# WD-Leong/CV-Lite-Object-Detection

Measured on AMD Instinct MI355X. Metric: training images/sec (whole node), FCOS-VOC 512x512 bs=16/GPU, higher is better.
Workload: dtype bf16; 1 GPU; FCOS ResNet-50-FPN train step (targets + fwd + loss + bwd + clip/SGD), 512x512, bs=16 per GPU; model=FCOS-ResNet50-FPN, global_batch=16, image_size=512, parallelism=dp1

## Files before the change

cv-lite-object-detection_amd/csrc/conv_common.h:

```cpp
#pragma once
#include "cvl_common.h"
#include "bn_acc.h"
#include <type_traits>
#include <vector>

typedef short s16x8 __attribute__((ext_vector_type(8)));
typedef short s16x4 __attribute__((ext_vector_type(4)));
typedef __bf16 bf16x8 __attribute__((ext_vector_type(8)));
typedef float f32x4 __attribute__((ext_vector_type(4)));

constexpr int kMaxSeg = CVL_CONV_MAX_SEG;

__device__ __forceinline__ short relu_bf16_bits(short v) { return v < 0 ? (short)0 : v; }

extern thread_local int g_cvl_conv_last_kernel;
extern thread_local int g_cvl_conv_last_ktile;

__device__ __forceinline__ int xcd_remap(int b, int nwg) {
  const int q = nwg / 8, r = nwg % 8, x = b % 8;
  return (x < r ? x * (q + 1) : r * (q + 1) + (x - r) * q) + b / 8;
}

template <int N>
__device__ __forceinline__ void wait_vm() {
  __builtin_amdgcn_s_waitcnt((N & 15) | ((N >> 4) << 14) | (7 << 4) | (15 << 8));
}

__device__ __forceinline__ s16x4 ds_tr16(unsigned addr) {
  s16x4 v;
  asm volatile("ds_read_b64_tr_b16 %0, %1" : "=v"(v) : "v"(addr));
  return v;
}
__device__ __forceinline__ void lgkm_wait() { asm volatile("s_waitcnt lgkmcnt(0)" ::: "memory"); }
__device__ __forceinline__ void tr_pin(s16x4& v) { asm volatile("" : "+v"(v)); }
__device__ __forceinline__ s16x8 tr_join(s16x4 l, s16x4 h) {
  return s16x8{l[0], l[1], l[2], l[3], h[0], h[1], h[2], h[3]};
}

__device__ __forceinline__ unsigned lds_addr(const void* p) {
  return (unsigned)(size_t)(const __attribute__((address_space(3))) void*)p;
}

struct ConvSeg {
  int Hr, Wr, Hs, Ws;
  long src_base, src_img, dst_base, dst_img;
  int m_start;
  int rows;
  const cvl_bf16* w;
  const float* bias;
};

struct ConvArgs {
  const cvl_bf16* src;
  void* dst;
  acc_u64* stats;
  int acc_slots;
  int nseg, B;
  ConvSeg seg[kMaxSeg];
  int Cin, KH, KW, stride, pad_t, pad_l;
  int K, Npad, n_store, ld_dst, dst_coff, dst_f32, relu_out, relu_in;
  float beta;
  int m_tiles, m_total;
  float* slab;
  int splits, ksteps_per_split;
  int dbg;
  int dst_up, dst_w;
  const cvl_bf16* bz;
  const float* bmr;
  const float* bga;
  const float* bbe;
  acc_u64* bsum;
  float bhi;
  const cvl_bf16* by;
  const uint8_t* bbits;
  unsigned long long* probe;
  const cvl_bf16* ymask;
};

uint64_t* cvl_probe_current(bool take);
void cvl_probe_enter_call();
void cvl_probe_leave_call();

__device__ __forceinline__ void probe_enter(unsigned long long* p) {
  if (blockIdx.x == 0 && threadIdx.x == 0) __hip_atomic_store(p, wall_clock64(), __ATOMIC_RELAXED, __HIP_MEMORY_SCOPE_AGENT);
}
__device__ __forceinline__ void probe_leave(unsigned long long* p) {
  __syncthreads();
  if (threadIdx.x == 0) {
    if (atomicAdd(p + 3, 1ull) == (unsigned long long)gridDim.x - 1) {
      const unsigned long long t = wall_clock64();
      const unsigned long long t0 = __hip_atomic_load(p, __ATOMIC_RELAXED, __HIP_MEMORY_SCOPE_AGENT);
      atomicAdd(p + 1, t - t0);
      atomicAdd(p + 2, 1ull);
      __hip_atomic_store(p + 3, 0ull, __ATOMIC_RELAXED, __HIP_MEMORY_SCOPE_AGENT);
    }
  }
}

int cvl_bn_acc_prepare(uint64_t* acc, long nstat, hipStream_t s);

int cvl_wgrad_reduce(const float* slab, float* dst0, float* dst1, long n4, int splits, int groups, float beta,
                     hipStream_t s);
int cvl_wgrad_defer_guard(const float* dst, hipStream_t s);
int cvl_wgrad_reduce_lanes(long elems4, int splits);

struct BnSumArgs {
  const cvl_bf16* z;
  const float* mr;
  const float* gamma;
  const float* beta;
  acc_u64* sums;
  float hi;
  const cvl_bf16* y;
  const uint8_t* bits;
};

enum { CVL_BSUM_NONE = 0, CVL_BSUM_Z = 1, CVL_BSUM_Y = 2, CVL_BSUM_BITS = 3 };
struct ConvCallOpts {
  bool bn_stats;
  int bsum;
  bool ymask;
  size_t workspace_bytes;
  bool res_relu;
};

enum { CVL_PRE_NONE = 0, CVL_PRE_ZERO_GAPS = 1, CVL_PRE_S2DG3_PACK = 2 };

struct ConvPlan {
  int kernel;
  int bn, bk;
  bool dgrad;
  bool sw;
  bool wres;
  bool prio, acc, stamps;
  int stages;
  int bsum;
  bool ymask;
  bool res_relu;
  int splits, ksteps_per_split;
  int grid;
  size_t workspace_bytes;
  int pre;
  size_t pack_bytes;
  int dbg;
  cvl_conv_desc desc;
  ConvArgs geo;
};

int conv_plan(const cvl_conv_desc* d, const ConvCallOpts& o, ConvPlan* p);
size_t conv_plan_workspace_bound(const cvl_conv_desc* d);
static inline void conv_plan_set_splits(ConvPlan* p, int nk, int want) {
  p->ksteps_per_split = (nk + want - 1) / want;
  p->splits = (nk + p->ksteps_per_split - 1) / p->ksteps_per_split;
}
static inline int conv_plan_ktile(const ConvPlan& p) { return p.kernel == CVL_CK_X32 || p.kernel == CVL_CK_P ? p.bk : 0; }

int launch_base(const ConvPlan& p, const ConvArgs& a, hipStream_t s);
int launch_l(const ConvPlan& p, const ConvArgs& a, hipStream_t s);
int launch_x(const ConvPlan& p, const ConvArgs& a, hipStream_t s);
int launch_h(const ConvPlan& p, const ConvArgs& a, hipStream_t s);
int launch_p(const ConvPlan& p, const ConvArgs& a, hipStream_t s);

bool cvl_conv_h_fits(const cvl_conv_desc* d, const ConvArgs& a, int* halo_px);
constexpr int kConvHWresCb = 2;
constexpr int kConvHStampWgs = 4096;
constexpr unsigned kConvBufRecords = 0x7fffffffu;

template <class F>
static inline void with_bool(bool b, F&& f) {
  if (b) f(std::true_type{});
  else f(std::false_type{});
}

constexpr int kWgSegM = 128;
constexpr int kWgXMaxGroups = 2;
constexpr int kWgXMaxProb = 16, kWgHMaxProb = 12;

struct WgLaunch {
  int kernel;
  int seg0, nseg, ngroups;
  int tile;
  int rows;
  bool pf;
  int tiles, co_tiles;
  int chunk, nsplit;
  int steps;
  int g_m0[kWgXMaxGroups], g_m1[kWgXMaxGroups];
  int cbase[kMaxSeg + 1];
  size_t slab_bytes;
};

struct WgradPlan {
  int nlaunch;
  WgLaunch l[kMaxSeg];
  size_t workspace_bytes;
};
int wgrad_plan(const cvl_conv_desc* d, int ngroups, WgradPlan* p);

static inline cvl_conv_desc wgrad_launch_desc(const cvl_conv_desc* d, const WgLaunch& l) {
  cvl_conv_desc s = *d;
  s.nseg = l.nseg;
  for (int i = 0; i < l.nseg; ++i) s.seg[i] = d->seg[l.seg0 + i];
  return s;
}

struct WgBatchLaunch {
  int kernel, tile;
  int n, idx[kWgXMaxProb];
  int chunk;
  int nsplit[kWgXMaxProb];
  size_t slab_off[kWgXMaxProb];
  size_t ws_off, ws_bytes;
  WgradPlan single;
};
struct WgradBatchPlan {
  std::vector<WgBatchLaunch> l;
  size_t workspace_bytes;
};
int wgrad_batch_plan(const cvl_conv_desc* const* d, int n, WgradBatchPlan* p);

bool wg_sn_fits(const cvl_conv_desc* d, int ngroups);
bool wg_h_fits(const cvl_conv_desc* d);
bool wg_x_fits(const cvl_conv_desc* d, int ngroups, const ConvArgs& a);
bool wg_x_batch_fits(const cvl_conv_desc* d, ConvArgs* a);
bool wg_l_fits(const cvl_conv_desc* d, const ConvArgs& a);

int launch_wg_sn(const WgLaunch& l, const cvl_conv_desc& d, const void* x, const void* dy, float* const* dw, float beta,
                 void* ws, hipStream_t s);
int launch_wg_h(const WgLaunch& l, const cvl_conv_desc& d, const void* x, const void* dy, float* const* dw, float beta,
                void* ws, hipStream_t s);
int launch_wg_x(const WgLaunch& l, const cvl_conv_desc& d, const void* x, const void* dy, float* const* dw, float beta,
                void* ws, hipStream_t s);
int launch_wg_l(const WgLaunch& l, const cvl_conv_desc& d, const void* x, const void* dy, float* const* dw, float beta,
                void* ws, hipStream_t s);
int launch_wg_s(const WgLaunch& l, const cvl_conv_desc& d, const void* x, const void* dy, float* const* dw, float beta,
                void* ws, hipStream_t s);
int launch_wg_x_batch(const WgBatchLaunch& b, const cvl_conv_desc* const* d, const void* const* x, const void* const* dy,
                      float* const* dw, float beta, char* ws, hipStream_t s);
int launch_wg_h_batch(const WgBatchLaunch& b, const cvl_conv_desc* const* d, const void* const* x, const void* const* dy,
                      float* const* dw, float beta, char* ws, hipStream_t s);
int wgrad_run(const WgradPlan& p, const cvl_conv_desc* d, const void* x, const void* dy, float* const* dw, float beta,
              void* ws, hipStream_t s);

size_t cvl_conv_wgrad_f32_workspace(const cvl_conv_desc* d, int ngroups);
int cvl_conv_wgrad_f32(const cvl_conv_desc* d, int ngroups, const void* x, const void* dy, float* const* dw,
                       float beta, void* workspace, size_t workspace_bytes, hipStream_t s);

__device__ __forceinline__ long conv_dst_row(const ConvArgs& a, const ConvSeg& S, int img, int q) {
  long r = q;
  if (a.dst_up != 1) {
    const int y = q / S.Wr, x = q - (q / S.Wr) * S.Wr;
    r = (long)y * a.dst_up * a.dst_w + (long)x * a.dst_up;
  }
  return S.dst_base + (long)img * S.dst_img + r;
}

static inline int cvl_conv_prepare(const cvl_conv_desc* d, int bm, ConvArgs* a) {
  CVL_CHECK_ARG(d);
  CVL_CHECK_ARG(d->nseg >= 1 && d->nseg <= kMaxSeg && d->B >= 1);
  CVL_CHECK_ARG(d->Cin > 0 && d->KH > 0 && d->KW > 0 && d->stride > 0);
  CVL_CHECK_ARG(d->mode == CVL_CONV_FWD || d->mode == CVL_CONV_DGRAD);
  CVL_CHECK_ARG(d->Npad > 0 && d->n_store > 0 && d->n_store <= d->Npad);
  CVL_CHECK_ARG(d->ld_dst >= d->dst_coff + d->n_store);
  a->slab = nullptr;
  a->splits = 1;
  a->ksteps_per_split = 0;
  a->dst_up = 1;
  a->dst_w = 0;
  a->dbg = 0;
  a->bz = nullptr; a->bmr = nullptr; a->bga = nullptr; a->bbe = nullptr; a->bsum = nullptr; a->bhi = 0.f;
  a->by = nullptr;
  a->bbits = nullptr;
  a->probe = nullptr;
  a->ymask = nullptr;
  a->acc_slots = cvl_bn_acc_slots();
  a->nseg = d->nseg;
  a->B = d->B;
  a->Cin = d->Cin; a->KH = d->KH; a->KW = d->KW; a->stride = d->stride;
  a->pad_t = d->pad_t; a->pad_l = d->pad_l;
  a->K = d->KH * d->KW * d->Cin;
  a->Npad = d->Npad; a->n_store = d->n_store; a->ld_dst = d->ld_dst; a->dst_coff = d->dst_coff;
  a->dst_f32 = d->dst_f32; a->relu_out = d->relu_out; a->relu_in = d->relu_in; a->beta = d->beta;
  int m = 0;
  for (int i = 0; i < kMaxSeg; ++i) {
    ConvSeg& s = a->seg[i];
    if (i >= d->nseg) {
      s = a->seg[0];
      s.m_start = 0x7fffffff;
      continue;
    }
    const cvl_conv_seg& q = d->seg[i];
    CVL_CHECK_ARG(q.Hr > 0 && q.Wr > 0 && q.Hs > 0 && q.Ws > 0 && q.w);
    s.Hr = q.Hr; s.Wr = q.Wr; s.Hs = q.Hs; s.Ws = q.Ws;
    s.src_base = q.src_base; s.src_img = q.src_img; s.dst_base = q.dst_base; s.dst_img = q.dst_img;
    s.w = reinterpret_cast<const cvl_bf16*>(q.w);
    s.bias = q.bias;
    s.m_start = m;
    s.rows = d->B * q.Hr * q.Wr;
    m += ((s.rows + bm - 1) / bm) * bm;
  }
  a->m_total = m;
  a->m_tiles = m / bm;
  return CVL_OK;
}
```

cv-lite-object-detection_amd/csrc/conv_dispatch.hip:

```cpp
#include "conv_common.h"

namespace {

constexpr int BM_BASE = 128, NT_BASE = 256;
constexpr int BM = 256;
constexpr int H_BN = 64, H_BK = 32;

int device_cus() {
  static const int n = cvl_device_cus();
  return n;
}

int pick_bn(int npad) { return npad % 128 == 0 ? 128 : (npad % 64 == 0 ? 64 : 32); }

int base_split_want(const ConvArgs& a) {
  if (a.nseg != 1) return 1;
  const int BN_ = pick_bn(a.Npad), BK_ = a.Cin % 64 == 0 ? 64 : 32;
  const int tiles = a.m_tiles * (a.Npad / BN_);
  const int nk = a.K / BK_;
  const int max_tiles = cvl_tune_int("CVL_KSPLIT_MAX_TILES", 192);
  const int target = cvl_tune_int("CVL_KSPLIT_TARGET", 384);
  const int min_nk = cvl_dispatch_int("ksplit_min_nk", 4);
  if (tiles >= max_tiles || nk < min_nk) return 1;
  int s = (target + tiles - 1) / tiles;
  const int per = cvl_tune_int("CVL_KSPLIT_MIN_PER", 2);
  if (s > nk / per) s = nk / per;
  return s < 1 ? 1 : s;
}

int h_split_want(const ConvArgs& a) {
  const int tiles = a.m_tiles * (a.Npad / H_BN);
  const int target = cvl_tune_int("CVL_CONV_H_SPLIT_TARGET", 256);
  if (tiles >= target) return 1;
  int splits = (target + tiles - 1) / tiles;
  if (splits > (a.Cin / H_BK) / 2) splits = (a.Cin / H_BK) / 2;
  return splits < 1 ? 1 : splits;
}

size_t slab_bytes(const ConvArgs& a, int splits) { return (size_t)splits * a.m_total * a.Npad * sizeof(float); }

bool s2dgrad_transform(const cvl_conv_desc* d, cvl_conv_desc* out, int* up, int* upw) {
  if (d->mode != CVL_CONV_DGRAD || d->KH != 1 || d->KW != 1 || d->stride < 2 || d->nseg != 1 ||
      d->pad_t != 0 || d->pad_l != 0 || d->relu_in || cvl_tune_flag("CVL_CONV_NO_S2DG"))
    return false;
  const cvl_conv_seg& q = d->seg[0];
  if ((q.Hs - 1) * d->stride >= q.Hr || (q.Ws - 1) * d->stride >= q.Wr) return false;
  *out = *d;
  out->mode = CVL_CONV_FWD;
  out->stride = 1;
  out->seg[0].Hr = q.Hs;
  out->seg[0].Wr = q.Ws;
  *up = d->stride;
  *upw = q.Wr;
  return true;
}

bool s2dgrad3_ok(const cvl_conv_desc* d) {
  if (!d || d->mode != CVL_CONV_DGRAD || d->KH != 3 || d->KW != 3 || d->stride != 2 || d->pad_t || d->pad_l ||
      d->nseg != 1 || d->relu_in || d->prec != CVL_PREC_BF16 || d->Cin % 32 || d->Npad % 32 ||
      cvl_dispatch_flag("no_s2dg3"))
    return false;
  const cvl_conv_seg& q = d->seg[0];
  return q.Hr == 2 * q.Hs && q.Wr == 2 * q.Ws && q.w &&
         (long)d->B * q.Hr * q.Wr >= cvl_dispatch_int("s2dg3_min_rows", 4096);
}

size_t s2dgrad3_pack_bytes(const cvl_conv_desc* d) {
  return ((size_t)4 * d->Npad * 4 * d->Cin * sizeof(cvl_bf16) + 255) / 256 * 256;
}

cvl_conv_desc s2dgrad3_desc(const cvl_conv_desc* d, const cvl_bf16* sub) {
  cvl_conv_desc dd = *d;
  const cvl_conv_seg q = d->seg[0];
  dd.mode = CVL_CONV_FWD;
  dd.KH = dd.KW = 2;
  dd.stride = 1;
  dd.pad_t = dd.pad_l = 1;
  dd.nseg = 4;
  for (int cls = 0; cls < 4; ++cls) {
    cvl_conv_seg& g = dd.seg[cls];
    g = q;
    g.Hr = q.Hs;
    g.Wr = q.Ws;
    g.w = sub + (size_t)cls * d->Npad * 4 * d->Cin;
    g.bias = nullptr;
    g.dst_base = q.dst_base + (long)(cls >> 1) * q.Wr + (cls & 1);
  }
  return dd;
}
const cvl_bf16* const kPackPlaceholder = reinterpret_cast<const cvl_bf16*>(16);

bool dst_chunks8(const cvl_conv_desc* d) { return d->n_store % 8 == 0 && d->ld_dst % 8 == 0 && d->dst_coff % 8 == 0; }

bool tiles_in_images(const ConvArgs& a, bool dense) {
  for (int i = 0; i < a.nseg; ++i) {
    const long hw = (long)a.seg[i].Hr * a.seg[i].Wr;
    if (hw % BM || (dense && a.seg[i].dst_img != hw)) return false;
  }
  return true;
}

bool buffer_bounds_ok(const ConvArgs& a) {
  for (int i = 0; i < a.nseg; ++i) {
    const ConvSeg& q = a.seg[i];
    const long src_bytes = (q.src_base + (long)a.B * q.src_img) * a.Cin * 2;
    if (src_bytes >= (long)kConvBufRecords - 65536) return false;
  }
  return (long)a.Npad * a.K * 2 < (long)kConvBufRecords;
}

bool x32_fits(const cvl_conv_desc* d, const ConvArgs& a) {
  const bool dg = d->mode == CVL_CONV_DGRAD;
  if (a.Npad % 256 || a.Cin % 32 || a.K / 32 < 1 || d->KH * d->KW > 32 || a.relu_in || (dg && d->stride != 1) ||
      a.dst_up != 1)
    return false;
  return buffer_bounds_ok(a);
}

bool plan_x(const cvl_conv_desc* d, const ConvArgs& a, const ConvCallOpts& o, ConvPlan* p) {
  if (cvl_dispatch_flag("no_x") || !x32_fits(d, a)) return false;
  p->kernel = CVL_CK_X32;
  p->bn = 256;
  p->bk = 32;
  p->grid = a.m_tiles * (a.Npad / 256);
  p->dbg = cvl_tune_int("CVL_X_ABLATE", 0);
  p->sw = !a.dst_f32 && !o.bn_stats && a.beta == 0.f && dst_chunks8(d) && !cvl_dispatch_flag("x_no_sw");
  p->ymask = p->sw && o.ymask && !a.relu_out && !cvl_dispatch_flag("no_relu_mask_fuse");
  return true;
}

bool p_fits(const cvl_conv_desc* d, const ConvArgs& a, const ConvCallOpts& o) {
  if (d->KH != 1 || d->KW != 1 || d->pad_t || d->pad_l || a.relu_in || a.nseg != 1 || a.K % 32) return false;
  const bool by = o.bsum == CVL_BSUM_Y || o.bsum == CVL_BSUM_BITS;
  if (o.bsum == CVL_BSUM_BITS && (a.ld_dst % 8 || a.dst_coff % 8)) return false;
  if (o.bsum && ((d->mode != CVL_CONV_DGRAD && a.dst_up == 1) || a.dst_f32 || (a.beta != 0.f) != by ||
                 (a.dst_up != 1 && !by) || o.bn_stats || (a.seg[0].Hr * a.seg[0].Wr) % BM ||
                 (a.dst_up == 1 && a.seg[0].dst_img != (long)a.seg[0].Hr * a.seg[0].Wr) || a.Npad % 64))
    return false;
  if (d->mode == CVL_CONV_DGRAD && d->stride != 1) return false;
  const ConvSeg& q = a.seg[0];
  if (d->stride == 1 && (q.Hs != q.Hr || q.Ws != q.Wr)) return false;
  if (a.dst_f32 ? (a.n_store % 4 || a.ld_dst % 4 || a.dst_coff % 4) : !dst_chunks8(d)) return false;
  if (o.bn_stats && (a.dst_f32 || (q.Hr * q.Wr) % BM)) return false;
  return buffer_bounds_ok(a);
}

bool plan_p(const cvl_conv_desc* d, const ConvArgs& a, const ConvCallOpts& o, ConvPlan* p) {
  if (cvl_dispatch_flag("no_p") || !p_fits(d, a, o)) return false;
  if (o.bsum && cvl_tune_flag("CVL_CONV_P_NO_BSUM")) return false;
  const bool wide = a.K <= 256 || (a.Npad >= 2 * a.K && cvl_dispatch_int("p_wide128", 1));
  const int bn = wide && a.Npad % 128 == 0 ? 128 : (a.Npad % 64 == 0 ? 64 : 0);
  const int fbn = cvl_dispatch_int("p_bn", 0);
  const int use = o.bsum ? 64 : (fbn && a.Npad % fbn == 0 ? fbn : bn);
  if (!use) return false;
  const int ntiles = a.m_tiles * (a.Npad / use);
  const int ntn = a.Npad / use;
  const int wgs = cvl_dispatch_int("p_wgs", 256);
  int grid = cvl_tune_int("CVL_CONV_P_WGS", wgs > 256 ? 256 : (wgs < 1 ? 1 : wgs));
  if (grid >= ntiles) grid = ntiles;
  else grid -= grid % ntn;
  if (grid < 1) return false;
  p->kernel = CVL_CK_P;
  p->bn = use;
  p->bk = a.K % 64 == 0 && use != 256 && cvl_dispatch_int("p_k64", 1) ? 64 : 32;
  p->grid = grid;
  p->dbg = cvl_tune_int("CVL_P_ABLATE", 0);
  p->bsum = o.bsum;
  p->acc = a.beta != 0.f && !cvl_tune_flag("CVL_P_NO_ACC");
  p->res_relu = o.res_relu && p->acc && use != 256 && !cvl_dispatch_flag("no_res_relu_fuse");
  return true;
}

bool plan_h(const cvl_conv_desc* d, const ConvArgs& a, const ConvCallOpts& o, size_t ws_bytes, ConvPlan* p) {
  int halo_px = 0;
  if (cvl_dispatch_flag("no_h") || !cvl_conv_h_fits(d, a, &halo_px)) return false;
  const bool stg3 = !cvl_dispatch_flag("h_no_3stage") && halo_px <= 512;
  const bool bs = o.bsum != CVL_BSUM_NONE;
  p->kernel = CVL_CK_H64;
  p->bk = H_BK;
  p->bsum = o.bsum;
  if (a.Npad == 32) {
    if (o.bn_stats || bs) return false;
    p->bn = 32;
    p->stages = stg3 ? 3 : 2;
    p->grid = a.m_tiles < device_cus() ? a.m_tiles : device_cus();
    return true;
  }
  const int tiles = a.m_tiles * (a.Npad / H_BN);
  const bool sw_ok = !d->dst_f32 && d->beta == 0.f && dst_chunks8(d) && !(o.bn_stats && bs) && tiles_in_images(a, bs);
  if (!cvl_dispatch_flag("h_no_n32") && a.Npad % H_BN == 0 && 2 * tiles <= device_cus() && sw_ok) {
    p->bn = 32;
    p->sw = true;
    p->stages = stg3 ? 3 : 2;
    p->grid = 2 * tiles;
    return true;
  }
  const int ncb = a.Cin / H_BK;
  int splits = 1;
  if (a.nseg == 1 && !bs && ws_bytes && d->n_store % 8 == 0 && d->dst_coff % 8 == 0 &&
      (d->dst_f32 || d->ld_dst % 8 == 0) && d->n_store / 8 <= 256) {
    splits = h_split_want(a);
    if (slab_bytes(a, splits) > ws_bytes) splits = 1;
  }
  if (splits > 1) conv_plan_set_splits(p, ncb, splits);
  const int per_cu = cvl_tune_int("CVL_CONV_H_WG_PER_CU", 1);
  p->grid = p->splits > 1 ? tiles : (tiles < device_cus() * per_cu ? tiles : device_cus() * per_cu);
  p->bn = H_BN;
  p->stages = 2;
  p->wres = p->splits <= 1 && a.Npad == H_BN && ncb <= kConvHWresCb && a.nseg == 1 && !cvl_dispatch_flag("h_no_wres");
  p->sw = p->splits <= 1 && sw_ok && !cvl_dispatch_flag("h_no_sw");
  p->stamps = cvl_tune_flag("CVL_H_STAMPS") && p->splits <= 1 && p->grid <= kConvHStampWgs;
  return true;
}

bool large_fits(const cvl_conv_desc* d, const ConvCallOpts& o) {
  if (d->Cin % 32 != 0 || d->relu_in) return false;
  return d->dst_f32 ? (d->n_store % 4 == 0 && !o.bn_stats) : dst_chunks8(d);
}

bool plan_large(const cvl_conv_desc* d, const ConvArgs& a, const ConvCallOpts& o, ConvPlan* p) {
  if (cvl_dispatch_flag("no_l")) return false;
  const bool bs = o.bsum != CVL_BSUM_NONE, by = o.bsum == CVL_BSUM_Y || o.bsum == CVL_BSUM_BITS;
  const bool scat = by && a.dst_up != 1 && d->KH == 1 && d->KW == 1 && d->mode == CVL_CONV_FWD;
  if (bs && !scat &&
      (d->mode != CVL_CONV_DGRAD || d->dst_f32 || (d->beta != 0.f && !by) || a.dst_up != 1 || o.bn_stats))
    return false;
  if (scat && (d->dst_f32 || o.bn_stats)) return false;
  if (by && (d->KH != 1 || d->KW != 1)) return false;
  if (d->Npad == 32 && d->KH == 3 && d->KW == 3 && d->mode == CVL_CONV_FWD && d->dst_f32 && !o.bn_stats &&
      !bs && a.dst_up == 1 && d->Cin % 32 == 0 && !d->relu_in && !cvl_dispatch_flag("no_h32"))
    return plan_h(d, a, o, 0, p);
  if (!large_fits(d, o)) return false;
  if (d->dst_f32 && (cvl_tune_flag("CVL_CONV_L_F32_N8") || cvl_tune_flag("CVL_CONV_L_NO_F32"))) return false;
  const bool l_cin = d->Cin % 64 == 0;
  const bool w256 = d->Npad % 256 == 0 && !cvl_dispatch_flag("no_256") &&
                    (d->mode == CVL_CONV_FWD || !cvl_tune_flag("CVL_CONV_NO_DGRAD_256"));
  const int bn = w256 ? 256 : (d->Npad % 128 == 0 ? 128 : (d->Npad % 64 == 0 ? 64 : 0));
  if (!bn) return false;
  if (l_cin && d->KH * d->KW * d->Cin < cvl_tune_int("CVL_CONV_L_MIN_K", 0) && !bs) return false;
  if (d->KH == 1 && d->KW == 1) {
    if (plan_p(d, a, o, p)) return true;
    if (by) return false;
  }
  const long min_tiles = cvl_dispatch_int("l_min_tiles", 128);
  int use_bn = bn;
  if (use_bn == 256 && (long)a.m_tiles * (a.Npad / 256) < cvl_dispatch_int("l256_min_tiles", 256)) use_bn = 128;
  const int w256_min_k = cvl_dispatch_int("w256_min_k", 512);
  if (use_bn == 256 && a.K < w256_min_k) use_bn = 128;
  const int fill = cvl_tune_int("CVL_CONV_L64_FILL", 256);
  const bool fill_pre = !cvl_tune_flag("CVL_CONV_L64_NO_FILL_PRE");
  const bool to64 = fill && use_bn == 128 && (long)a.m_tiles * (a.Npad / 128) < fill && a.Npad % 64 == 0 &&
                    !(bs && cvl_tune_flag("CVL_BSUM_NO_FILL"));
  if (!l_cin && d->Cin == 32 && bn == 256 && !bs && !o.bn_stats && cvl_dispatch_int("x_cin32", 1) &&
      plan_x(d, a, o, p))
    return true;
  const bool h_width = use_bn == 64 || to64 || !l_cin || cvl_tune_flag("CVL_CONV_H_ANY_N");
  if (h_width && use_bn != 256 && (!bs || ((a.seg[0].Hr * a.seg[0].Wr) % BM == 0 && !o.bn_stats)) &&
      (!bs || tiles_in_images(a, true)) && plan_h(d, a, o, o.workspace_bytes, p))
    return true;
  if (!l_cin) return false;
  if (fill_pre && to64) use_bn = 64;
  if ((long)a.m_tiles * (a.Npad / use_bn) < min_tiles) return false;
  if (to64) use_bn = 64;
  if (o.bn_stats)
    for (int i = 0; i < a.nseg; ++i)
      if ((a.seg[i].Hr * a.seg[i].Wr) % 4) return false;
  if (bs && (use_bn == 256 || !tiles_in_images(a, true))) return false;
  if (use_bn == 256 && plan_x(d, a, o, p)) return true;
  p->kernel = use_bn == 256 ? CVL_CK_L256 : (use_bn == 128 ? CVL_CK_L128 : CVL_CK_L64);
  p->bn = use_bn;
  p->bk = 64;
  p->grid = a.m_tiles * (a.Npad / use_bn);
  p->bsum = o.bsum;
  p->prio = !cvl_tune_flag("CVL_CONV_NO_PRIO");
  p->sw = !a.dst_f32 && a.beta == 0.f && !bs && a.dst_up == 1 && dst_chunks8(d) && !cvl_dispatch_flag("l_no_sw") &&
          (!o.bn_stats || tiles_in_images(a, false));
  return true;
}

void plan_base(const cvl_conv_desc* d, const ConvArgs& a, const ConvCallOpts& o, ConvPlan* p) {
  p->bn = pick_bn(a.Npad);
  p->bk = p->bn <= 64 && a.Cin % 128 == 0 && cvl_dispatch_int("base_bk128", 1) ? 128 : (a.Cin % 64 == 0 ? 64 : 32);
  const int sp = base_split_want(a);
  const bool split = sp > 1 && (d->n_store / 8 <= NT_BASE) && o.workspace_bytes >= slab_bytes(a, sp) &&
                     d->n_store % 8 == 0 && d->dst_coff % 8 == 0 && (d->dst_f32 || d->ld_dst % 8 == 0);
  if (split) conv_plan_set_splits(p, a.K / p->bk, sp);
  p->kernel = split ? CVL_CK_BASE_SPLITK : CVL_CK_BASE;
  p->grid = a.m_tiles * (a.Npad / p->bn);
}

bool bsum_offer_ok(const cvl_conv_desc* d, int form) {
  if (cvl_tune_flag("CVL_NO_BNSUM_FUSE") || d->prec != CVL_PREC_BF16 || d->mode != CVL_CONV_DGRAD || d->dst_f32 ||
      d->Cin % 32 || d->Npad % 32 || !dst_chunks8(d))
    return false;
  const long hw = (long)d->seg[0].Hr * d->seg[0].Wr;
  if (form == CVL_BSUM_Z)
    return d->beta == 0.f && hw >= cvl_tune_int("CVL_BNSUM_MIN_HW", 0);
  return !cvl_tune_flag("CVL_NO_BNSUM_RES") && d->beta != 0.f && d->KH == 1 && d->KW == 1 &&
         (d->stride == 1 || !cvl_dispatch_flag("no_bnsum_res_s2")) &&
         hw >= cvl_dispatch_int("bnsum_res_min_hw", 256);
}

}

int conv_plan(const cvl_conv_desc* d, const ConvCallOpts& o, ConvPlan* p) {
  CVL_CHECK_ARG(d && p && d->prec == CVL_PREC_BF16);
  *p = ConvPlan{};
  p->kernel = CVL_CK_NONE;
  p->splits = 1;
  size_t ws_bytes = o.workspace_bytes;
  int up = 1, upw = 0;
  if (o.bsum) {
    if (!d->nseg || !bsum_offer_ok(d, o.bsum)) return CVL_OK;
    const bool tr = s2dgrad_transform(d, &p->desc, &up, &upw);
    if (o.bsum == CVL_BSUM_Z ? tr : (d->stride != 1 && !tr)) return CVL_OK;
    if (!tr) p->desc = *d;
  } else if (s2dgrad3_ok(d) && ws_bytes >= s2dgrad3_pack_bytes(d)) {
    CVL_CHECK_ARG(!o.bn_stats);
    CVL_CHECK_ARG(d->dst_f32 || dst_chunks8(d));
    p->pre = CVL_PRE_S2DG3_PACK;
    p->pack_bytes = s2dgrad3_pack_bytes(d);
    p->desc = s2dgrad3_desc(d, kPackPlaceholder);
    up = 2;
    upw = d->seg[0].Wr;
    ws_bytes -= p->pack_bytes;
  } else if (s2dgrad_transform(d, &p->desc, &up, &upw)) {
    CVL_CHECK_ARG(!o.bn_stats);
    CVL_CHECK_ARG(d->dst_f32 || dst_chunks8(d));
    if (d->beta == 0.f) {
      const cvl_conv_seg& q = d->seg[0];
      const long line = (long)q.Wr * (d->dst_f32 ? d->n_store : d->n_store / 8);
      CVL_CHECK_ARG(line < (1l << 31) && (long)d->B * q.Hr < (1l << 31));
      p->pre = CVL_PRE_ZERO_GAPS;
    }
  } else {
    p->desc = *d;
  }
  d = &p->desc;
  p->dgrad = d->mode == CVL_CONV_DGRAD;
  ConvCallOpts oo = o;
  oo.workspace_bytes = ws_bytes;
  ConvArgs base;
  const int st = cvl_conv_prepare(d, BM_BASE, &base);
  if (st) return o.bsum ? CVL_OK : st;
  if (!o.bsum) {
    CVL_CHECK_ARG(d->Cin % 32 == 0 && d->Npad % 32 == 0);
    if (!d->dst_f32) CVL_CHECK_ARG(dst_chunks8(d));
    if (o.bn_stats) {
      for (int i = 0; i < base.nseg; ++i) {
        const int hw = base.seg[i].Hr * base.seg[i].Wr;
        CVL_CHECK_ARG(hw % BM_BASE == 0 || hw % 4 == 0);
      }
    }
  }
  if (cvl_conv_prepare(d, BM, &p->geo) == CVL_OK) {
    p->geo.dst_up = up;
    p->geo.dst_w = upw;
    ConvPlan q = *p;
    if (plan_large(d, p->geo, oo, &q)) *p = q;
  }
  if (p->kernel == CVL_CK_NONE) {
    if (o.bsum) return CVL_OK;
    p->geo = base;
    p->geo.dst_up = up;
    p->geo.dst_w = upw;
    plan_base(d, p->geo, oo, p);
  }
  p->workspace_bytes = p->pack_bytes + (p->splits > 1 ? slab_bytes(p->geo, p->splits) : 0);
  return CVL_OK;
}

size_t conv_plan_workspace_bound(const cvl_conv_desc* d) {
  if (s2dgrad3_ok(d)) {
    const cvl_conv_desc dd = s2dgrad3_desc(d, kPackPlaceholder);
    return s2dgrad3_pack_bytes(d) + conv_plan_workspace_bound(&dd);
  }
  cvl_conv_desc dd;
  int up = 1, upw = 0;
  if (s2dgrad_transform(d, &dd, &up, &upw)) d = &dd;
  ConvArgs a;
  if (cvl_conv_prepare(d, BM_BASE, &a)) return 0;
  const int sp = base_split_want(a);
  size_t n = sp > 1 ? slab_bytes(a, sp) : 16;
  ConvArgs a256;
  int halo_px = 0;
  if (cvl_conv_prepare(d, BM, &a256) == CVL_OK && a256.nseg == 1 && a256.Npad % H_BN == 0 &&
      cvl_conv_h_fits(d, a256, &halo_px)) {
    const int hs = h_split_want(a256);
    if (hs > 1 && slab_bytes(a256, hs) > n) n = slab_bytes(a256, hs);
  }
  return n;
}

extern "C" int cvl_conv_igemm_plan(const cvl_conv_desc* d, int with_bn_stats, size_t workspace_bytes, int32_t* kernel,
                                   int32_t* ktile) {
  CVL_CHECK_ARG(d && kernel && ktile);
  *kernel = CVL_CK_NONE;
  *ktile = 0;
  if (d->prec == CVL_PREC_F32) return CVL_OK;
  ConvPlan p;
  const int st = conv_plan(d, ConvCallOpts{with_bn_stats != 0, CVL_BSUM_NONE, false, workspace_bytes}, &p);
  if (st) return st;
  *kernel = p.kernel;
  *ktile = conv_plan_ktile(p);
  return CVL_OK;
}
```

cv-lite-object-detection_amd/csrc/conv_igemm.hip:

```cpp
#include "conv_common.h"

namespace {

constexpr int BM = 128;
constexpr int NT = 256;

template <int BK>
__device__ __forceinline__ int swz(int r) {
  return BK == 128 ? (r & 15) : (BK == 64 ? ((r >> 1) & 7) : ((r >> 2) & 3));
}

__device__ __forceinline__ s16x8 relu_bf16x8(s16x8 v) {
#pragma unroll
  for (int i = 0; i < 8; ++i) v[i] = v[i] < 0 ? (short)0 : v[i];
  return v;
}



template <int BN, int BK, bool DGRAD>
__global__ void __launch_bounds__(NT) conv_igemm_kernel(ConvArgs a) {
  constexpr int WM = BM / 2, WN = BN / 2;
  constexpr int TM = WM / 16, TN = WN / 16;
  constexpr int CPR = BK / 8;
  constexpr int RPP = NT / CPR;
  constexpr int AP = BM / RPP;
  constexpr int BROWS = BN < RPP ? BN : RPP;
  constexpr int BP = BN / BROWS;
  constexpr int LDS_AB = (BM + BN) * BK;
  constexpr int LDS_C = BM * (BN + 8);
  constexpr int LDS_EL = LDS_AB > LDS_C ? LDS_AB : LDS_C;
  __shared__ __attribute__((aligned(16))) cvl_bf16 lds[LDS_EL];
  cvl_bf16* As = lds;
  cvl_bf16* Bs = lds + BM * BK;

  const int tid = threadIdx.x;
  const int m_tile = blockIdx.x, n_tile = blockIdx.y;
  const int m0 = m_tile * BM, n0 = n_tile * BN;
  int sg = 0;
#pragma unroll
  for (int i = 1; i < kMaxSeg; ++i)
    if (i < a.nseg && m0 >= a.seg[i].m_start) sg = i;
  const ConvSeg& S = a.seg[sg];
  const int HWr = S.Hr * S.Wr;
  const int mloc0 = m0 - S.m_start;
  if (mloc0 >= S.rows) return;

  const int ch = tid % CPR, rr = tid / CPR;
  int a_img[AP], a_y[AP], a_x[AP];
  bool a_ok[AP];
#pragma unroll
  for (int p = 0; p < AP; ++p) {
    const int ml = mloc0 + p * RPP + rr;
    a_ok[p] = ml < S.rows;
    const int img = ml / HWr, q = ml - img * HWr;
    const int oy = q / S.Wr, ox = q - (q / S.Wr) * S.Wr;
    a_img[p] = img;
    if (DGRAD) { a_y[p] = oy + a.pad_t; a_x[p] = ox + a.pad_l; }
    else { a_y[p] = oy * a.stride - a.pad_t; a_x[p] = ox * a.stride - a.pad_l; }
  }
  const cvl_bf16* __restrict__ wsrc = S.w;
  const cvl_bf16* __restrict__ src = a.src;
  const int Cin = a.Cin;

  s16x8 ra[AP], rb[BP];
  auto load_tile = [&](int kt) {
    const int k0 = kt * BK;
    const int tap = k0 / Cin;
    const int c0 = k0 - tap * Cin + ch * 8;
    const int r = tap / a.KW, s = tap - (tap / a.KW) * a.KW;
#pragma unroll
    for (int p = 0; p < AP; ++p) {
      int iy, ix;
      bool ok = a_ok[p];
      if (DGRAD) {
        const int ty = a_y[p] - r, tx = a_x[p] - s;
        ok = ok && ty >= 0 && tx >= 0 && (ty % a.stride) == 0 && (tx % a.stride) == 0;
        iy = ty / a.stride; ix = tx / a.stride;
      } else {
        iy = a_y[p] + r; ix = a_x[p] + s;
      }
      ok = ok && iy >= 0 && ix >= 0 && iy < S.Hs && ix < S.Ws;
      if (ok) {
        const long row = S.src_base + (long)a_img[p] * S.src_img + (long)iy * S.Ws + ix;
        ra[p] = *reinterpret_cast<const s16x8*>(src + row * Cin + c0);
        if (a.relu_in) ra[p] = relu_bf16x8(ra[p]);
      } else {
        ra[p] = s16x8{0, 0, 0, 0, 0, 0, 0, 0};
      }
    }
#pragma unroll
    for (int p = 0; p < BP; ++p) {
      const int n = n0 + p * BROWS + tid / CPR;
      if (tid / CPR < BROWS)
        rb[p] = *reinterpret_cast<const s16x8*>(wsrc + (long)n * a.K + k0 + ch * 8);
    }
  };
  auto store_tile = [&]() {
#pragma unroll
    for (int p = 0; p < AP; ++p) {
      const int r = p * RPP + rr;
      *reinterpret_cast<s16x8*>(As + r * BK + ((ch ^ swz<BK>(r)) * 8)) = ra[p];
    }
#pragma unroll
    for (int p = 0; p < BP; ++p) {
      const int r = p * BROWS + tid / CPR;
      if (tid / CPR < BROWS) *reinterpret_cast<s16x8*>(Bs + r * BK + ((ch ^ swz<BK>(r)) * 8)) = rb[p];
    }
  };

  const int wave = tid >> 6, lane = tid & 63;
  const int wm = wave >> 1, wn = wave & 1;
  const int lr = lane & 15, lg = lane >> 4;
  f32x4 acc[TM][TN];
#pragma unroll
  for (int i = 0; i < TM; ++i)
#pragma unroll
    for (int j = 0; j < TN; ++j) acc[i][j] = f32x4{0.f, 0.f, 0.f, 0.f};

  int kt0 = 0, kt1 = a.K / BK;
  if (a.splits > 1) {
    kt0 = blockIdx.z * a.ksteps_per_split;
    kt1 = min(kt1, kt0 + a.ksteps_per_split);
  }
  const int nk = kt1;
  load_tile(kt0);
  for (int kt = kt0; kt < nk; ++kt) {
    const cvl_bf16* Ac = As;
    const cvl_bf16* Bc = Bs;
    __syncthreads();
    store_tile();
    __syncthreads();
    if (kt + 1 < nk) load_tile(kt + 1);
#pragma unroll
    for (int ks = 0; ks < BK / 32; ++ks) {
      const int chunk = ks * 4 + lg;
      s16x8 fa[TM], fb[TN];
#pragma unroll
      for (int i = 0; i < TM; ++i) {
        const int r = wm * WM + i * 16 + lr;
        fa[i] = *reinterpret_cast<const s16x8*>(Ac + r * BK + ((chunk ^ swz<BK>(r)) * 8));
      }
#pragma unroll
      for (int j = 0; j < TN; ++j) {
        const int r = wn * WN + j * 16 + lr;
        fb[j] = *reinterpret_cast<const s16x8*>(Bc + r * BK + ((chunk ^ swz<BK>(r)) * 8));
      }
#pragma unroll
      for (int i = 0; i < TM; ++i)
#pragma unroll
        for (int j = 0; j < TN; ++j)
          acc[i][j] = __builtin_amdgcn_mfma_f32_16x16x32_bf16(
              __builtin_bit_cast(bf16x8, fa[i]), __builtin_bit_cast(bf16x8, fb[j]), acc[i][j], 0, 0, 0);
    }
  }

  if (a.splits > 1) {
    float* slab = a.slab + (size_t)blockIdx.z * a.m_total * a.Npad;
#pragma unroll
    for (int i = 0; i < TM; ++i)
#pragma unroll
      for (int j = 0; j < TN; ++j)
#pragma unroll
        for (int e = 0; e < 4; ++e) {
          const int r = m0 + wm * WM + i * 16 + lg * 4 + e;
          const int c = n0 + wn * WN + j * 16 + lr;
          slab[(size_t)r * a.Npad + c] = acc[i][j][e];
        }
    return;
  }
  const float* bias = S.bias;
  float bcol[TN];
#pragma unroll
  for (int j = 0; j < TN; ++j) {
    const int n = n0 + wn * WN + j * 16 + lr;
    bcol[j] = (bias && n < a.n_store) ? bias[n] : 0.f;
  }
  const bool round_bf16 = !a.dst_f32;
#pragma unroll
  for (int i = 0; i < TM; ++i)
#pragma unroll
    for (int j = 0; j < TN; ++j)
#pragma unroll
      for (int e = 0; e < 4; ++e) {
        float v = acc[i][j][e] + bcol[j];
        if (a.relu_out) v = v > 0.f ? v : 0.f;
        if (round_bf16) v = bf16_to_f32(f32_to_bf16(v));
        acc[i][j][e] = v;
      }

  if (a.stats && (HWr % BM) != 0) {
#pragma unroll
    for (int i = 0; i < TM; ++i) {
      const int ml0 = mloc0 + wm * WM + i * 16 + lg * 4;
      if (ml0 >= S.rows) continue;
      const int img = ml0 / HWr;
#pragma unroll
      for (int j = 0; j < TN; ++j) {
        const int n = n0 + wn * WN + j * 16 + lr;
        if (n >= a.n_store) continue;
        float s1 = 0.f, s2 = 0.f;
#pragma unroll
        for (int e = 0; e < 4; ++e) { const float v = acc[i][j][e]; s1 += v; s2 += v * v; }
        acc_u64* st = a.stats + acc_idx((long)img * a.n_store + n, 0, a.acc_slots);
        acc_add(st, s1, a.acc_slots);
        acc_add(st + a.acc_slots, s2, a.acc_slots);
      }
    }
  } else if (a.stats) {
    const int img = mloc0 / HWr;
#pragma unroll
    for (int j = 0; j < TN; ++j) {
      float s1 = 0.f, s2 = 0.f;
#pragma unroll
      for (int i = 0; i < TM; ++i)
#pragma unroll
        for (int e = 0; e < 4; ++e) {
          const int ml = mloc0 + wm * WM + i * 16 + lg * 4 + e;
          const float v = ml < S.rows ? acc[i][j][e] : 0.f;
          s1 += v; s2 += v * v;
        }
      s1 += __shfl_xor(s1, 16, 64); s1 += __shfl_xor(s1, 32, 64);
      s2 += __shfl_xor(s2, 16, 64); s2 += __shfl_xor(s2, 32, 64);
      const int n = n0 + wn * WN + j * 16 + lr;
      if (lg == 0 && n < a.n_store) {
        acc_u64* st = a.stats + acc_idx((long)img * a.n_store + n, 0, a.acc_slots);
        acc_add(st, s1, a.acc_slots);
        acc_add(st + a.acc_slots, s2, a.acc_slots);
      }
    }
  }

  if (a.dst_f32) {
    float* dst = reinterpret_cast<float*>(a.dst);
#pragma unroll
    for (int i = 0; i < TM; ++i)
#pragma unroll
      for (int e = 0; e < 4; ++e) {
        const int ml = mloc0 + wm * WM + i * 16 + lg * 4 + e;
        if (ml >= S.rows) continue;
        const int img = ml / HWr, q = ml - img * HWr;
        const long drow = conv_dst_row(a, S, img, q);
#pragma unroll
        for (int j = 0; j < TN; ++j) {
          const int n = n0 + wn * WN + j * 16 + lr;
          if (n >= a.n_store) continue;
          float* pd = dst + drow * a.ld_dst + a.dst_coff + n;
          *pd = a.beta != 0.f ? acc[i][j][e] + a.beta * *pd : acc[i][j][e];
        }
      }
    return;
  }

  __syncthreads();
  constexpr int CP = BN + 8;
  cvl_bf16* Cs = lds;
#pragma unroll
  for (int i = 0; i < TM; ++i)
#pragma unroll
    for (int j = 0; j < TN; ++j)
#pragma unroll
      for (int e = 0; e < 4; ++e) {
        const int r = wm * WM + i * 16 + lg * 4 + e;
        const int c = wn * WN + j * 16 + lr;
        Cs[r * CP + c] = f32_to_bf16(acc[i][j][e]);
      }
  __syncthreads();
  constexpr int CCH = BN / 8;
  cvl_bf16* dst = reinterpret_cast<cvl_bf16*>(a.dst);
  for (int idx = tid; idx < BM * CCH; idx += NT) {
    const int r = idx / CCH, c8 = (idx - (idx / CCH) * CCH) * 8;
    const int ml = mloc0 + r;
    if (ml >= S.rows || n0 + c8 >= a.n_store) continue;
    const int img = ml / HWr, q = ml - img * HWr;
    const long drow = conv_dst_row(a, S, img, q);
    s16x8 v = *reinterpret_cast<const s16x8*>(Cs + r * CP + c8);
    s16x8* pd = reinterpret_cast<s16x8*>(dst + drow * a.ld_dst + a.dst_coff + n0 + c8);
    if (a.beta != 0.f) {
      const s16x8 o = *pd;
#pragma unroll
      for (int u = 0; u < 8; ++u)
        v[u] = (short)f32_to_bf16(bf16_to_f32((cvl_bf16)v[u]) + a.beta * bf16_to_f32((cvl_bf16)o[u]));
    }
    *pd = v;
  }
}

constexpr int FIN_RL = NT / 8;
__global__ void __launch_bounds__(NT) conv_splitk_finish(ConvArgs a, int rows_per_blk) {
  const ConvSeg& S = a.seg[0];
  const int HW = S.Hr * S.Wr;
  const int img = blockIdx.y;
  const int cgi = threadIdx.x & 7, rl = threadIdx.x >> 3;
  const int c0 = blockIdx.z * 64 + cgi * 8;
  const bool cok = c0 < a.n_store;
  const int q0 = blockIdx.x * rows_per_blk;
  const int q1 = min(q0 + rows_per_blk, HW);
  __shared__ float red[FIN_RL][8][17];
  float s1[8], s2[8], bb[8];
#pragma unroll
  for (int u = 0; u < 8; ++u) { s1[u] = 0.f; s2[u] = 0.f; bb[u] = (S.bias && cok) ? S.bias[c0 + u] : 0.f; }
  if (cok) {
    for (int q = q0 + rl; q < q1; q += FIN_RL) {
      const long ml = (long)img * HW + q;
      float v[8];
#pragma unroll
      for (int u = 0; u < 8; ++u) v[u] = bb[u];
      const f32x4* p = reinterpret_cast<const f32x4*>(a.slab + (size_t)ml * a.Npad + c0);
      const size_t zs = (size_t)a.m_total * a.Npad / 4;
      int z = 0;
      for (; z + 4 <= a.splits; z += 4) {
        f32x4 x[4][2];
#pragma unroll
        for (int t = 0; t < 4; ++t) { x[t][0] = p[(z + t) * zs]; x[t][1] = p[(z + t) * zs + 1]; }
#pragma unroll
        for (int t = 0; t < 4; ++t) {
          v[0] += x[t][0][0]; v[1] += x[t][0][1]; v[2] += x[t][0][2]; v[3] += x[t][0][3];
          v[4] += x[t][1][0]; v[5] += x[t][1][1]; v[6] += x[t][1][2]; v[7] += x[t][1][3];
        }
      }
      for (; z < a.splits; ++z) {
        const f32x4 x0 = p[z * zs], x1 = p[z * zs + 1];
        v[0] += x0[0]; v[1] += x0[1]; v[2] += x0[2]; v[3] += x0[3];
        v[4] += x1[0]; v[5] += x1[1]; v[6] += x1[2]; v[7] += x1[3];
      }
      const long drow = conv_dst_row(a, S, img, q);
      if (a.dst_f32) {
        float* pd = reinterpret_cast<float*>(a.dst) + drow * a.ld_dst + a.dst_coff + c0;
#pragma unroll
        for (int u = 0; u < 8; ++u) {
          float o = v[u];
          if (a.relu_out) o = o > 0.f ? o : 0.f;
          s1[u] += o; s2[u] += o * o;
          if (a.beta != 0.f) o += a.beta * pd[u];
          pd[u] = o;
        }
      } else {
        s16x8* pd = reinterpret_cast<s16x8*>(reinterpret_cast<cvl_bf16*>(a.dst) + drow * a.ld_dst + a.dst_coff + c0);
        s16x8 old;
        if (a.beta != 0.f) old = *pd;
        s16x8 o;
#pragma unroll
        for (int u = 0; u < 8; ++u) {
          float x = v[u];
          if (a.relu_out) x = x > 0.f ? x : 0.f;
          x = bf16_to_f32(f32_to_bf16(x));
          s1[u] += x; s2[u] += x * x;
          if (a.beta != 0.f) x += a.beta * bf16_to_f32((cvl_bf16)old[u]);
          o[u] = (short)f32_to_bf16(x);
        }
        *pd = o;
      }
    }
  }
  if (a.stats) {
#pragma unroll
    for (int u = 0; u < 8; ++u) { red[rl][cgi][u] = s1[u]; red[rl][cgi][8 + u] = s2[u]; }
    __syncthreads();
    if (threadIdx.x < 64) {
      const int cg2 = threadIdx.x >> 3, u = threadIdx.x & 7;
      const int c = blockIdx.z * 64 + cg2 * 8 + u;
      if (c < a.n_store) {
        double t1 = 0.0, t2 = 0.0;
        for (int k = 0; k < FIN_RL; ++k) { t1 += red[k][cg2][u]; t2 += red[k][cg2][8 + u]; }
        acc_u64* st = a.stats + acc_idx((long)img * a.n_store + c, 0, a.acc_slots);
        acc_add_f64(st, t1, a.acc_slots);
        acc_add_f64(st + a.acc_slots, t2, a.acc_slots);
      }
    }
  }
}

static int splitk_finish_launch(const ConvArgs& a, hipStream_t s) {
  const ConvSeg& S = a.seg[0];
  const int HW = S.Hr * S.Wr;
  const int nch = (a.n_store + 63) / 64;
  int parts = 512 / (a.B * nch);
  if (parts > HW / 16) parts = HW / 16;
  if (parts < 1) parts = 1;
  const int rpb = (HW + parts - 1) / parts;
  hipLaunchKernelGGL(conv_splitk_finish, dim3((HW + rpb - 1) / rpb, a.B, nch), dim3(NT), 0, s, a, rpb);
  return cvl_launch_status();
}

template <int BN, int BK>
void launch_bn_bk(const ConvPlan& p, const ConvArgs& a, hipStream_t s) {
  dim3 grid(a.m_tiles, a.Npad / BN, a.splits);
  with_bool(p.dgrad, [&](auto DG) {
    hipLaunchKernelGGL((conv_igemm_kernel<BN, BK, decltype(DG)::value>), grid, dim3(NT), 0, s, a);
  });
}

template <int BN>
void launch_bn(const ConvPlan& p, const ConvArgs& a, hipStream_t s) {
  if (BN <= 64 && p.bk == 128) launch_bn_bk<BN, 128>(p, a, s);
  else if (p.bk == 64) launch_bn_bk<BN, 64>(p, a, s);
  else launch_bn_bk<BN, 32>(p, a, s);
}

}

__global__ void s2dgrad3_pack_kernel(const cvl_bf16* __restrict__ wd, cvl_bf16* __restrict__ sub, int Npad, int Cin) {
  const int c8n = Cin / 8;
  const long total = 16L * Npad * c8n;
  for (long i = blockIdx.x * (long)NT + threadIdx.x; i < total; i += (long)gridDim.x * NT) {
    const int c8 = (int)(i % c8n);
    const long r1 = i / c8n;
    const int t = (int)(r1 & 3);
    const long r2 = r1 >> 2;
    const int n = (int)(r2 % Npad), cls = (int)(r2 / Npad);
    const int py = cls >> 1, px = cls & 1, rp = t >> 1, sp = t & 1;
    const int r = py ? (rp ? 1 : -1) : (rp ? 0 : 2);
    const int sx = px ? (sp ? 1 : -1) : (sp ? 0 : 2);
    s16x8 v = s16x8{0, 0, 0, 0, 0, 0, 0, 0};
    if (r >= 0 && sx >= 0) v = *reinterpret_cast<const s16x8*>(wd + (long)n * 9 * Cin + (r * 3 + sx) * Cin + c8 * 8);
    *reinterpret_cast<s16x8*>(sub + i * 8) = v;
  }
}

__global__ void zero_gaps_kernel(void* dst, int is_f32, long dst_base, long dst_img, int ld, int coff, int n,
                                 int B, int H, int W, int s) {
  const int n8 = is_f32 ? n : n / 8;
  for (int line = blockIdx.y; line < B * H; line += gridDim.y) {
    const int img = line / H, y = line - img * H;
    const bool full = y % s != 0;
    const long base = dst_base + (long)img * dst_img + (long)y * W;
    for (int i = blockIdx.x * blockDim.x + threadIdx.x; i < W * n8; i += gridDim.x * blockDim.x) {
      const int x = i / n8, c = i - x * n8;
      if (!full && x % s == 0) continue;
      const long row = base + x;
      if (is_f32) reinterpret_cast<float*>(dst)[row * ld + coff + c] = 0.f;
      else *reinterpret_cast<s16x8*>(reinterpret_cast<cvl_bf16*>(dst) + row * ld + coff + c * 8) = s16x8{0, 0, 0, 0, 0, 0, 0, 0};
    }
  }
}

namespace {

int pre_pass(const ConvPlan& p, const cvl_conv_desc* d, void* dst, void* workspace, hipStream_t s) {
  if (p.pre == CVL_PRE_S2DG3_PACK) {
    const long b = (16L * d->Npad * (d->Cin / 8) + NT - 1) / NT;
    hipLaunchKernelGGL(s2dgrad3_pack_kernel, dim3((int)(b > 4096 ? 4096 : (b < 1 ? 1 : b))), dim3(NT), 0, s,
                       reinterpret_cast<const cvl_bf16*>(d->seg[0].w), reinterpret_cast<cvl_bf16*>(workspace), d->Npad,
                       d->Cin);
  } else if (p.pre == CVL_PRE_ZERO_GAPS) {
    const cvl_conv_seg& q = d->seg[0];
    const long line = (long)q.Wr * (d->dst_f32 ? d->n_store : d->n_store / 8);
    const int bx = (int)((line + NT - 1) / NT);
    const int by = d->B * q.Hr < 65535 ? d->B * q.Hr : 65535;
    hipLaunchKernelGGL(zero_gaps_kernel, dim3(bx < 1 ? 1 : bx, by), dim3(NT), 0, s, dst, d->dst_f32, q.dst_base,
                       q.dst_img, d->ld_dst, d->dst_coff, d->n_store, d->B, q.Hr, q.Wr, d->stride);
  } else {
    return CVL_OK;
  }
  return cvl_launch_status();
}

struct ConvIo {
  const void* src;
  void* dst;
  acc_u64* stats;
  const BnSumArgs* bsum;
  const void* ymask;
  void* workspace;
};

void fill_args(const ConvPlan& p, const ConvIo& io, ConvArgs* a) {
  *a = p.geo;
  a->src = reinterpret_cast<const cvl_bf16*>(io.src);
  a->dst = io.dst;
  a->stats = io.stats;
  if (p.bsum) {
    const BnSumArgs& b = *io.bsum;
    a->bz = b.z; a->bmr = b.mr; a->bga = b.gamma; a->bbe = b.beta; a->bsum = b.sums; a->bhi = b.hi;
    a->by = b.y;
    a->bbits = b.bits;
  }
  if (p.ymask) a->ymask = reinterpret_cast<const cvl_bf16*>(io.ymask);
  if (p.kernel == CVL_CK_X32) a->probe = reinterpret_cast<unsigned long long*>(cvl_probe_current(true));
  a->dbg = p.dbg;
  a->splits = p.splits;
  a->ksteps_per_split = p.ksteps_per_split;
  char* ws = reinterpret_cast<char*>(io.workspace);
  if (p.splits > 1) a->slab = reinterpret_cast<float*>(ws + p.pack_bytes);
  if (p.pre == CVL_PRE_S2DG3_PACK)
    for (int i = 0; i < kMaxSeg; ++i)
      a->seg[i].w = reinterpret_cast<const cvl_bf16*>(ws) + (size_t)(i < a->nseg ? i : 0) * a->Npad * a->K;
}

}

thread_local int g_cvl_conv_last_kernel = CVL_CK_NONE;
thread_local int g_cvl_conv_last_ktile = 0;

extern "C" int cvl_conv_igemm_last_kernel(void) { return g_cvl_conv_last_kernel; }
extern "C" int cvl_conv_igemm_last_ktile(void) { return g_cvl_conv_last_ktile; }

int launch_base(const ConvPlan& p, const ConvArgs& a, hipStream_t s) {
  if (p.bn == 128) launch_bn<128>(p, a, s);
  else if (p.bn == 64) launch_bn<64>(p, a, s);
  else launch_bn<32>(p, a, s);
  return cvl_launch_status();
}

namespace {
int conv_run(const ConvPlan& p, const cvl_conv_desc* d, const ConvIo& io, hipStream_t s) {
  int st = pre_pass(p, d, io.dst, io.workspace, s);
  if (st) return st;
  ConvArgs a;
  fill_args(p, io, &a);
  switch (p.kernel) {
    case CVL_CK_P: st = launch_p(p, a, s); break;
    case CVL_CK_X32: st = launch_x(p, a, s); break;
    case CVL_CK_H64: st = launch_h(p, a, s); break;
    case CVL_CK_L64: case CVL_CK_L128: case CVL_CK_L256: st = launch_l(p, a, s); break;
    default: st = launch_base(p, a, s); break;
  }
  g_cvl_conv_last_kernel = p.kernel;
  g_cvl_conv_last_ktile = conv_plan_ktile(p);
  if (st || p.splits <= 1) return st;
  return splitk_finish_launch(a, s);
}
}

extern "C" const char* cvl_conv_kernel_name(int code) {
  switch (code) {
    case CVL_CK_BASE: return "conv_igemm_kernel (128-row)";
    case CVL_CK_BASE_SPLITK: return "conv_igemm_kernel (128-row, split-K)";
    case CVL_CK_L64: return "conv_igemm_l_kernel<64> (256x64)";
    case CVL_CK_L128: return "conv_igemm_l_kernel<128> (256x128)";
    case CVL_CK_L256: return "conv_igemm_l_kernel<256> (256x256)";
    case CVL_CK_X256: return "conv_igemm_x_kernel (256x256, 4 phases per 64-deep K-tile)";
    case CVL_CK_X32: return "conv_igemm_x32_kernel (256x256, 5-slot ring of 32-deep K-tiles)";
    case CVL_CK_X32H: return "conv_igemm_x32h_kernel (256x256, 3x3 halo tile in LDS, 6-slot weight ring)";
    case CVL_CK_WG_SN: return "conv_wgrad_sn_kernel (Npad 32, taps on the dY side, chunk slabs)";
    case CVL_CK_WG_S: return "conv_wgrad_kernel (128-wide k tile)";
    case CVL_CK_WG_L128: return "conv_wgrad_l_kernel<128> (128x256)";
    case CVL_CK_WG_L256: return "conv_wgrad_l_kernel<256> (256x256)";
    case CVL_CK_WG_X: return "conv_wgrad_x_kernel (256x256, 5-slot ring of 32-row steps, grouped)";
    case CVL_CK_WG_H: return "conv_wgrad_h_kernel (64 ci x 64 co x 9 taps, 128-row halo steps)";
    case CVL_CK_H64: return "conv_igemm_h_kernel (256x64, 3x3 halo + 9-tap weight stage per channel block)";
    case CVL_CK_P: return "conv_igemm_p_kernel (persistent 1x1, K-tile stream across tiles)";
    default: return "none";
  }
}

int cvl_conv_f32(const cvl_conv_desc* d, const void* src, void* dst, acc_u64* bn_stats, hipStream_t s);
int cvl_relu_backward(const void* dy, const void* y, void* dx, long n, float beta, cvl_stream_t stream);

extern "C" size_t cvl_conv_igemm_workspace_size(const cvl_conv_desc* d) {
  if (!d) return 0;
  if (d->prec == CVL_PREC_F32) return 16;
  return conv_plan_workspace_bound(d);
}

extern "C" int cvl_conv_igemm(const cvl_conv_desc* d, const void* src, void* dst, uint64_t* bn_stats_acc,
                              void* workspace, size_t workspace_bytes, cvl_stream_t stream) {
  CVL_CHECK_ARG(d);
  acc_u64* bn_stats = reinterpret_cast<acc_u64*>(bn_stats_acc);
  if (d->prec == CVL_PREC_F32) return cvl_conv_f32(d, src, dst, bn_stats, (hipStream_t)stream);
  ConvPlan p;
  const int st = conv_plan(d, ConvCallOpts{bn_stats != nullptr, CVL_BSUM_NONE, false, workspace ? workspace_bytes : 0}, &p);
  if (st) return st;
  CVL_CHECK_ARG(src && dst);
  cvl_probe_enter_call();
  const int rst = conv_run(p, d, ConvIo{src, dst, bn_stats, nullptr, nullptr, workspace}, (hipStream_t)stream);
  cvl_probe_leave_call();
  return rst;
}

extern "C" int cvl_conv_igemm_relu_mask(const cvl_conv_desc* d, const void* src, void* dst, const void* y,
                                        void* workspace, size_t workspace_bytes, cvl_stream_t stream) {
  CVL_CHECK_ARG(d && src && dst && y && d->mode == CVL_CONV_DGRAD && d->prec == CVL_PREC_BF16 && !d->dst_f32 &&
                d->beta == 0.f && !d->relu_out);
  ConvPlan p;
  int st = conv_plan(d, ConvCallOpts{false, CVL_BSUM_NONE, true, workspace ? workspace_bytes : 0}, &p);
  if (st) return st;
  if (!p.ymask) CVL_CHECK_ARG(d->ld_dst == d->n_store && d->dst_coff == 0);
  cvl_probe_enter_call();
  st = conv_run(p, d, ConvIo{src, dst, nullptr, nullptr, y, workspace}, (hipStream_t)stream);
  cvl_probe_leave_call();
  if (st || p.ymask) return st;
  long rows = 0;
  for (int i = 0; i < d->nseg; ++i) {
    const long e = d->seg[i].dst_base + (long)d->B * (d->seg[i].dst_img ? d->seg[i].dst_img : (long)d->seg[i].Hr * d->seg[i].Wr);
    rows = e > rows ? e : rows;
  }
  return cvl_relu_backward(dst, y, dst, rows * d->n_store, 0.f, stream);
}

namespace {
int res_relu_plan(const cvl_conv_desc* d, size_t ws, ConvPlan* p) {
  CVL_CHECK_ARG(d && d->mode == CVL_CONV_FWD && d->prec == CVL_PREC_BF16 && !d->dst_f32 && d->beta == 1.f &&
                !d->relu_out);
  const int st = conv_plan(d, ConvCallOpts{false, CVL_BSUM_NONE, false, ws, true}, p);
  if (st) return st;
  if (!p->res_relu) CVL_CHECK_ARG(d->ld_dst == d->n_store && d->dst_coff == 0);
  return CVL_OK;
}
}

extern "C" int cvl_conv_igemm_res_relu(const cvl_conv_desc* d, const void* src, void* dst, void* workspace,
                                       size_t workspace_bytes, cvl_stream_t stream) {
  CVL_CHECK_ARG(src && dst);
  ConvPlan p;
  int st = res_relu_plan(d, workspace ? workspace_bytes : 0, &p);
  if (st) return st;
  cvl_probe_enter_call();
  st = conv_run(p, d, ConvIo{src, dst, nullptr, nullptr, nullptr, workspace}, (hipStream_t)stream);
  cvl_probe_leave_call();
  if (st || p.res_relu) return st;
  long lo = d->seg[0].dst_base, hi = 0;
  for (int i = 0; i < d->nseg; ++i) {
    const long b = d->seg[i].dst_base;
    const long e = b + (long)d->B * (d->seg[i].dst_img ? d->seg[i].dst_img : (long)d->seg[i].Hr * d->seg[i].Wr);
    lo = b < lo ? b : lo;
    hi = e > hi ? e : hi;
  }
  return cvl_relu_(reinterpret_cast<cvl_bf16*>(dst) + lo * d->n_store, (hi - lo) * d->n_store, stream);
}

extern "C" int cvl_conv_igemm_res_relu_plan(const cvl_conv_desc* d, size_t workspace_bytes, int32_t* kernel,
                                            int32_t* fused) {
  CVL_CHECK_ARG(kernel && fused);
  *kernel = CVL_CK_NONE;
  *fused = 0;
  ConvPlan p;
  const int st = res_relu_plan(d, workspace_bytes, &p);
  if (st) return st;
  *kernel = p.kernel;
  *fused = p.res_relu ? 1 : 0;
  return CVL_OK;
}

namespace {
int dgrad_bnsum_plan_form(const cvl_conv_desc* d, int offer, size_t ws, int32_t* form) {
  *form = CVL_BSUM_NONE;
  if (d->prec == CVL_PREC_F32) return CVL_OK;
  for (int f = offer; f != CVL_BSUM_NONE; f = f == CVL_BSUM_BITS ? CVL_BSUM_Y : CVL_BSUM_NONE) {
    ConvPlan p;
    const int st = conv_plan(d, ConvCallOpts{false, f, false, ws}, &p);
    if (st) return st;
    if (p.kernel != CVL_CK_NONE) { *form = f; break; }
  }
  return CVL_OK;
}

int dgrad_bnsum_call(const cvl_conv_desc* d, const void* src, void* dst, int form, const BnSumArgs& b, int32_t* fused,
                     void* workspace, size_t workspace_bytes, cvl_stream_t stream) {
  *fused = 0;
  if (d->prec == CVL_PREC_F32) return cvl_conv_f32(d, src, dst, nullptr, (hipStream_t)stream);
  const size_t ws = workspace ? workspace_bytes : 0;
  ConvPlan p;
  int st = conv_plan(d, ConvCallOpts{false, form, false, ws}, &p);
  if (st) return st;
  const bool fuse = p.kernel != CVL_CK_NONE && src && dst;
  if (!fuse && (st = conv_plan(d, ConvCallOpts{false, CVL_BSUM_NONE, false, ws}, &p))) return st;
  CVL_CHECK_ARG(src && dst);
  if (!fuse) cvl_probe_enter_call();
  st = conv_run(p, d, ConvIo{src, dst, nullptr, &b, nullptr, workspace}, (hipStream_t)stream);
  if (!fuse) cvl_probe_leave_call();
  *fused = fuse && st == CVL_OK ? 1 : 0;
  return st;
}
}

extern "C" int cvl_conv_igemm_dgrad_bnsum(const cvl_conv_desc* d, const void* src, void* dst, const void* z,
                                          const float* mean_rstd, const float* gamma, const float* beta, float act_hi,
                                          uint64_t* sums, int32_t* fused, void* workspace, size_t workspace_bytes,
                                          cvl_stream_t stream) {
  CVL_CHECK_ARG(d && fused && z && mean_rstd && gamma && beta && sums);
  const BnSumArgs b{reinterpret_cast<const cvl_bf16*>(z), mean_rstd, gamma, beta, reinterpret_cast<acc_u64*>(sums),
                    act_hi, nullptr, nullptr};
  return dgrad_bnsum_call(d, src, dst, CVL_BSUM_Z, b, fused, workspace, workspace_bytes, stream);
}

extern "C" int cvl_conv_igemm_dgrad_bnsum_res(const cvl_conv_desc* d, const void* src, void* dst, const void* y,
                                              const void* z, const float* mean_rstd, const float* gamma,
                                              const float* beta, uint64_t* sums, int32_t* fused, void* workspace,
                                              size_t workspace_bytes, cvl_stream_t stream) {
  CVL_CHECK_ARG(d && fused && y && z && mean_rstd && gamma && beta && sums);
  const BnSumArgs b{reinterpret_cast<const cvl_bf16*>(z), mean_rstd, gamma, beta, reinterpret_cast<acc_u64*>(sums),
                    INFINITY, reinterpret_cast<const cvl_bf16*>(y), nullptr};
  return dgrad_bnsum_call(d, src, dst, CVL_BSUM_Y, b, fused, workspace, workspace_bytes, stream);
}

extern "C" int cvl_conv_igemm_dgrad_bnsum_res_bits(const cvl_conv_desc* d, const void* src, void* dst, const void* y,
                                                   const uint8_t* relu_bits, const void* z, const float* mean_rstd,
                                                   const float* gamma, const float* beta, uint64_t* sums,
                                                   int32_t* fused, int32_t* form, void* workspace,
                                                   size_t workspace_bytes, cvl_stream_t stream) {
  CVL_CHECK_ARG(d && fused && y && relu_bits && z && mean_rstd && gamma && beta && sums);
  const BnSumArgs b{reinterpret_cast<const cvl_bf16*>(z), mean_rstd, gamma, beta, reinterpret_cast<acc_u64*>(sums),
                    INFINITY, reinterpret_cast<const cvl_bf16*>(y), relu_bits};
  int32_t tmp = 0, *pf = form ? form : &tmp;
  *pf = 0;
  int st = dgrad_bnsum_plan_form(d, CVL_BSUM_BITS, workspace ? workspace_bytes : 0, pf);
  if (st) return st;
  st = dgrad_bnsum_call(d, src, dst, *pf ? *pf : CVL_BSUM_Y, b, fused, workspace, workspace_bytes, stream);
  if (st || !*fused) *pf = 0;
  return st;
}

extern "C" int cvl_conv_igemm_plan_bnsum(const cvl_conv_desc* d, int offer, size_t workspace_bytes, int32_t* form,
                                         int32_t* kernel, int32_t* ktile) {
  CVL_CHECK_ARG(d && form && kernel && ktile && offer >= CVL_BSUM_Z && offer <= CVL_BSUM_BITS);
  *form = 0;
  *kernel = CVL_CK_NONE;
  *ktile = 0;
  if (d->prec == CVL_PREC_F32) return CVL_OK;
  int st = dgrad_bnsum_plan_form(d, offer, workspace_bytes, form);
  if (st) return st;
  ConvPlan p;
  if ((st = conv_plan(d, ConvCallOpts{false, *form, false, workspace_bytes}, &p))) return st;
  *kernel = p.kernel;
  *ktile = conv_plan_ktile(p);
  return CVL_OK;
}

extern "C" int cvl_conv_igemm_plan_grid(const cvl_conv_desc* d, int with_bn_stats, int bsum_offer, size_t workspace_bytes,
                                        int32_t* kernel, int32_t* ktile, int32_t* grid, int32_t* ntile) {
  CVL_CHECK_ARG(d && kernel && ktile && grid && ntile && bsum_offer >= CVL_BSUM_NONE && bsum_offer <= CVL_BSUM_BITS);
  *kernel = CVL_CK_NONE;
  *ktile = *grid = *ntile = 0;
  if (d->prec == CVL_PREC_F32) return CVL_OK;
  int32_t form = CVL_BSUM_NONE;
  int st = bsum_offer ? dgrad_bnsum_plan_form(d, bsum_offer, workspace_bytes, &form) : CVL_OK;
  if (st) return st;
  ConvPlan p;
  if ((st = conv_plan(d, ConvCallOpts{with_bn_stats != 0 && !form, form, false, workspace_bytes}, &p))) return st;
  *kernel = p.kernel;
  *ktile = conv_plan_ktile(p);
  *grid = p.grid;
  *ntile = p.bn;
  return CVL_OK;
}
```

cv-lite-object-detection_amd/csrc/conv_igemm_h.hip:

```cpp
#include "conv_common.h"
#include "conv_epilogue.h"

namespace {

constexpr int BM = 256, BN = 64, NT = 512, BK = 32;
constexpr int WGM = 4, WM = 64, TM = 4;
constexpr int HPX = 640;
constexpr int HPW = HPX / 16 / 8;
constexpr int HALO_EL = HPX * BK;
constexpr int WRES_CB = 2;
constexpr unsigned kRecords = 0x7fffffffu;
constexpr unsigned kOOB = 0x80000000u;

__device__ __forceinline__ int swz4(int r) { return (r >> 1) & 3; }

typedef __bf16 bf16x2 __attribute__((ext_vector_type(2)));
typedef float f32x2 __attribute__((ext_vector_type(2)));
typedef unsigned u32x4 __attribute__((ext_vector_type(4)));

__device__ __forceinline__ void dma16(__amdgpu_buffer_rsrc_t r, const cvl_bf16* lds_dst, unsigned voff) {
  __builtin_amdgcn_raw_ptr_buffer_load_lds(r, (__attribute__((address_space(3))) void*)lds_dst, 16, (int)voff, 0,
                                           0, 0);
}

struct HGeo {
  int whole, mx, my, th, pitch, rows;
};
__host__ __device__ inline HGeo h_geo(int H, int W) {
  HGeo g;
  const int HW = H * W;
  g.whole = HW < BM;
  if (g.whole) {
    const int n = BM / HW;
    int lg = 0;
    while ((1 << (lg + 1)) <= n) ++lg;
    g.mx = 1 << ((lg + 1) / 2);
    g.my = n / g.mx;
    g.th = H;
  } else {
    g.mx = g.my = 1;
    g.th = BM / W;
  }
  g.pitch = (g.mx * (W + 1) + 1 + 7) & ~7;
  g.rows = g.my * (g.th + 1) + 1;
  return g;
}

struct HaloPieces {
  int rel[HPW];
  int yrow[HPW];
  unsigned valid;
};

__device__ __forceinline__ HaloPieces halo_pieces(const HGeo& G, int H, int W, int wave, int lane) {
  HaloPieces P;
  P.valid = 0;
  const int hpx = G.rows * G.pitch;
#pragma unroll
  for (int j = 0; j < HPW; ++j) {
    const int hp = 16 * (wave + 8 * j) + (lane >> 2);
    const int hy = hp / G.pitch, hx = hp - hy * G.pitch;
    bool ok;
    if (!G.whole) {
      const int gx = hx - 1;
      ok = gx >= 0 && gx < W;
      P.rel[j] = (hy - 1) * W + gx;
      P.yrow[j] = hy - 1;
    } else {
      const int ix = (hx - 1) / (W + 1), iy = (hy - 1) / (H + 1);
      const int gx = hx - 1 - ix * (W + 1), gy = hy - 1 - iy * (H + 1);
      ok = hx >= 1 && hy >= 1 && gx < W && gy < H && ix < G.mx && iy < G.my;
      P.rel[j] = gy * W + gx;
      P.yrow[j] = iy * G.mx + ix;
    }
    if (ok && hp < hpx) P.valid |= 1u << j;
  }
  return P;
}

#ifdef CVL_MEASURE
constexpr int kHStampWgs = 4096;
#else
constexpr int kHStampWgs = 1;
#endif
__device__ unsigned long long g_h_stamps[kHStampWgs * 8];

template <bool DGRAD, bool BSUM, bool WRES = false, bool ST = false, bool SW = false, int BNT = 64, int NSTG = 2>
__global__ void __launch_bounds__(NT) conv_igemm_h_kernel(ConvArgs a) {
  constexpr int BN = BNT, TN = BN / 32, WN = BN / 2;
  static_assert(NSTG == 2 || (NSTG == 3 && BNT == 32 && !WRES), "three stages: 32-wide tiles only");
  constexpr int HPXk = NSTG == 3 ? 512 : HPX;
  constexpr int HPWk = HPXk / 16 / 8;
  constexpr int HALO_ELk = HPXk * BK;
  constexpr int WPC = 9 * BN * BK * 2 / 1024;
  constexpr int WJ = WPC / 8, WR = WPC % 8;
  constexpr int PPT = BN / 16;
  constexpr int WT_EL = 9 * BN * BK;
  constexpr int STAGE_EL = HALO_ELk + WT_EL;
  constexpr int LDS_C = BM * (BN + 8) + WGM * BN * 2 * 2;
  constexpr int LDS_EL = NSTG * STAGE_EL > LDS_C ? NSTG * STAGE_EL : LDS_C;
  constexpr int LDS_WRES_EL = 2 * HALO_EL + WRES_CB * WT_EL;
  static_assert(HALO_ELk >= LDS_C && HPWk + WJ <= 9 && BN % 32 == 0, "H64 stage layout");
  constexpr int MAIN_EL = WRES ? LDS_WRES_EL : LDS_EL;
  __shared__ __attribute__((aligned(16))) cvl_bf16 lds[MAIN_EL + (SW ? WGM * BN * 2 * 2 : 0)];
  float* const red = reinterpret_cast<float*>(lds + MAIN_EL);
  constexpr int SST = WRES ? HALO_EL : STAGE_EL;
  const int pw_blk = HPWk + WJ + ((WR && (int)(threadIdx.x >> 6) < WR) ? 1 : 0);
  cvl_bf16* const wres = lds + 2 * HALO_EL;
  const int tid = threadIdx.x;
  const int wave = __builtin_amdgcn_readfirstlane(tid >> 6), lane = tid & 63;
  unsigned long long* const stamp = (ST && tid == 0 && blockIdx.x < kHStampWgs && blockIdx.z == 0)
                                        ? g_h_stamps + blockIdx.x * 8 : nullptr;
  unsigned long long t_tap = 0, t_wait = 0, t_epi = 0, n_tile = 0, c0 = 0, w0 = 0, w1 = 0;
  unsigned long long te[4] = {0, 0, 0, 0};
  if (ST && stamp) w0 = wall_clock64();
  const int ntn = a.Npad / BN;
  const int ntiles = a.m_tiles * ntn;
  const int G_ = gridDim.x;
  const int wl = xcd_remap(blockIdx.x, G_);
  const int t_lo = (int)((long)wl * ntiles / G_), t_hi = (int)((long)(wl + 1) * ntiles / G_);

  const int Cin = a.Cin, Kdim = a.K;
  const int ncb_all = Cin / BK;
  int cb0 = 0, cb1 = ncb_all;
  if (a.splits > 1) {
    cb0 = blockIdx.z * a.ksteps_per_split;
    cb1 = min(ncb_all, cb0 + a.ksteps_per_split);
  }
  auto tile_seg = [&](int L, int* sg, int* mloc0, int* n0) {
    const int m0 = (L / ntn) * BM;
    *n0 = (L % ntn) * BN;
    int q = 0;
#pragma unroll
    for (int i = 1; i < kMaxSeg; ++i)
      if (i < a.nseg && m0 >= a.seg[i].m_start) q = i;
    *sg = q;
    *mloc0 = m0 - a.seg[q].m_start;
    return *mloc0 < a.seg[q].rows;
  };
  auto next_tile = [&](int L) {
    int sg, ml, n0;
    while (L < t_hi && !tile_seg(L, &sg, &ml, &n0)) ++L;
    return L;
  };

  const int hch = lane & 3;
  int i_L = next_tile(t_lo), i_cb = cb0, i_sg = -1;
  unsigned hoff[HPW], woff[WJ + (WR ? 1 : 0)];
  HaloPieces HP;
  HP.valid = 0;
  auto cursor_tile = [&]() {
    int sg, mloc0, n0;
    tile_seg(i_L, &sg, &mloc0, &n0);
    const ConvSeg& S = a.seg[sg];
    const int W = S.Wr, H = S.Hr, HWr = H * W;
    const HGeo G = h_geo(H, W);
    if (sg != i_sg) {
      HP = halo_pieces(G, H, W, wave, lane);
      i_sg = sg;
    }
    const int img0 = mloc0 / HWr;
    const int y0 = G.whole ? 0 : (mloc0 - img0 * HWr) / W;
    const long base = S.src_base + (long)img0 * S.src_img + (long)y0 * W;
#pragma unroll
    for (int j = 0; j < HPW; ++j) {
      const int hp = 16 * (wave + 8 * j) + (lane >> 2);
      bool ok = (HP.valid >> j) & 1u;
      long pix;
      if (!G.whole) {
        ok = ok && (unsigned)(y0 + HP.yrow[j]) < (unsigned)H && img0 < a.B;
        pix = base + HP.rel[j];
      } else {
        const int img = img0 + HP.yrow[j];
        ok = ok && img < a.B;
        pix = S.src_base + (long)img * S.src_img + HP.rel[j];
      }
      hoff[j] = ok ? (unsigned)(pix * Cin * 2) + (unsigned)((hch ^ swz4(hp)) * 16) : kOOB;
    }
#pragma unroll
    for (int j = 0; j < WJ + (WR ? 1 : 0); ++j) {
      const int w = (wave + 8 * j) % WPC, tap = w / PPT;
      const int row = (w % PPT) * 16 + (lane >> 2);
      woff[j] = (unsigned)(((n0 + row) * Kdim + tap * Cin) * 2) + (unsigned)((hch ^ swz4(row)) * 16);
    }
  };
  if (i_L >= t_hi) return;
  cursor_tile();
  const __amdgpu_buffer_rsrc_t rsA = __builtin_amdgcn_make_buffer_rsrc((void*)a.src, (short)0, (int)kRecords, 0x00020000);
  __amdgpu_buffer_rsrc_t rsB = __builtin_amdgcn_make_buffer_rsrc((void*)a.seg[i_sg].w, (short)0, (int)kRecords, 0x00020000);
  auto advance = [&]() {
    if (++i_cb < cb1) return;
    i_cb = cb0;
    i_L = next_tile(i_L + 1);
    if (i_L < t_hi) {
      cursor_tile();
      rsB = __builtin_amdgcn_make_buffer_rsrc((void*)a.seg[i_sg].w, (short)0, (int)kRecords, 0x00020000);
    }
  };

  const int wm = wave >> 1, wn = wave & 1;
  const int lr = lane & 15, lg = lane >> 4;
  unsigned bfr[TN];
#pragma unroll
  for (int j = 0; j < TN; ++j) {
    const int rr = wn * WN + j * 16 + lr;
    bfr[j] = (unsigned)(rr * BK * 2 + ((lg ^ swz4(rr)) * 16));
  }

  constexpr int CPL = TN == 2 ? 8 : 4;
  const int lgo = TN == 2 ? ((lg & 1) ? 16 : 0) + ((lg & 2) ? 8 : 0) : 4 * lg;
  float ss1[SW ? TN : 1][4], ss2[SW ? TN : 1][4];
  float bs1[8], bs2[8], pm[8], prs[8], pga[8], pbe[8];
  int k_img = -1, k_n0 = 0;
  if constexpr (SW) {
#pragma unroll
    for (int j = 0; j < TN; ++j)
#pragma unroll
      for (int e = 0; e < 4; ++e) { ss1[j][e] = 0.f; ss2[j][e] = 0.f; }
#pragma unroll
    for (int u = 0; u < 8; ++u) { bs1[u] = 0.f; bs2[u] = 0.f; }
  }
  auto row16_sum = [](float v) {
    v += __int_as_float(__builtin_amdgcn_mov_dpp(__float_as_int(v), 0xB1, 0xF, 0xF, false));
    v += __int_as_float(__builtin_amdgcn_mov_dpp(__float_as_int(v), 0x4E, 0xF, 0xF, false));
    v += __int_as_float(__builtin_amdgcn_mov_dpp(__float_as_int(v), 0x141, 0xF, 0xF, false));
    v += __int_as_float(__builtin_amdgcn_mov_dpp(__float_as_int(v), 0x140, 0xF, 0xF, false));
    return v;
  };
  auto sw_flush = [&]() {
    if constexpr (SW) {
      if (k_img < 0) return;
      if (BSUM) {
#pragma unroll
        for (int u = 0; u < CPL; ++u) {
          const float t1 = row16_sum(bs1[u]), t2 = row16_sum(bs2[u]);
          bs1[u] = 0.f;
          bs2[u] = 0.f;
          if (lr == 0) {
            const int c = wn * WN + lgo + u;
            red[(wm * BN + c) * 2] = t1;
            red[(wm * BN + c) * 2 + 1] = t2;
          }
        }
      } else {
#pragma unroll
        for (int j = 0; j < TN; ++j)
#pragma unroll
          for (int e = 0; e < 4; ++e) {
            const float t1 = row16_sum(ss1[j][e]), t2 = row16_sum(ss2[j][e]);
            ss1[j][e] = 0.f;
            ss2[j][e] = 0.f;
            if (lr == 0) {
              const int c = wn * WN + j * 16 + 4 * lg + e;
              red[(wm * BN + c) * 2] = t1;
              red[(wm * BN + c) * 2 + 1] = t2;
            }
          }
      }
      __syncthreads();
      if (tid < BN && k_n0 + tid < a.n_store) {
        float t1 = 0.f, t2 = 0.f;
#pragma unroll
        for (int w = 0; w < WGM; ++w) { t1 += red[(w * BN + tid) * 2]; t2 += red[(w * BN + tid) * 2 + 1]; }
        acc_u64* st = (BSUM ? a.bsum : a.stats) + acc_idx((long)k_img * a.n_store + k_n0 + tid, 0, a.acc_slots);
        acc_add(st, t1, a.acc_slots);
        acc_add(st + a.acc_slots, t2, a.acc_slots);
      }
      __syncthreads();
    }
  };

  {
    cvl_bf16* st = lds;
    const unsigned cbo = (unsigned)(i_cb * BK * 2);
#pragma unroll
    for (int j = 0; j < HPWk; ++j) dma16(rsA, st + (wave + 8 * j) * 16 * BK, hoff[j] + cbo);
    if (WRES) {
#pragma unroll
      for (int j = 0; j < WJ; ++j) dma16(rsB, wres + (wave + 8 * j) * 16 * BK, woff[j]);
      if (WR && wave < WR) dma16(rsB, wres + (wave + 8 * WJ) * 16 * BK, woff[WJ]);
    } else {
#pragma unroll
      for (int j = 0; j < WJ; ++j) dma16(rsB, st + HALO_ELk + (wave + 8 * j) * 16 * BK, woff[j] + cbo);
      if (WR && wave < WR) dma16(rsB, st + HALO_ELk + (wave + 8 * WJ) * 16 * BK, woff[WJ] + cbo);
    }
    advance();
    if constexpr (NSTG == 3) {
      const bool m1 = i_L < t_hi;
      cvl_bf16* s1 = lds + SST;
      const unsigned cb1o = (unsigned)(i_cb * BK * 2);
#pragma unroll
      for (int j = 0; j < HPWk; ++j) dma16(rsA, s1 + (wave + 8 * j) * 16 * BK, m1 ? hoff[j] + cb1o : kOOB);
#pragma unroll
      for (int j = 0; j < WJ; ++j) dma16(rsB, s1 + HALO_ELk + (wave + 8 * j) * 16 * BK, m1 ? woff[j] + cb1o : kOOB);
      if (WR && wave < WR) dma16(rsB, s1 + HALO_ELk + (wave + 8 * WJ) * 16 * BK, m1 ? woff[WJ] + cb1o : kOOB);
      if (m1) advance();
    }
  }
  if constexpr (NSTG == 3) {
    if (pw_blk == HPWk + WJ + 1) wait_vm<HPWk + WJ + 1>();
    else wait_vm<HPWk + WJ>();
  } else {
    wait_vm<0>();
  }
  __builtin_amdgcn_s_barrier();
  asm volatile("" ::: "memory");
  if (ST && stamp) w1 = wall_clock64();
  if (WRES) {
    for (int cbw = 1; cbw < ncb_all; ++cbw) {
      const unsigned wo = (unsigned)(cbw * BK * 2);
#pragma unroll
      for (int j = 0; j < WJ; ++j) dma16(rsB, wres + cbw * WT_EL + (wave + 8 * j) * 16 * BK, woff[j] + wo);
      if (WR && wave < WR) dma16(rsB, wres + cbw * WT_EL + (wave + 8 * WJ) * 16 * BK, woff[WJ] + wo);
    }
  }

  int gb = 0;
  int c_cb = 0;
  int c_sg = -1;
  unsigned afr[TM][3];
  int HWr = 1, prow = 0;
  for (int L = next_tile(t_lo); L < t_hi; L = next_tile(L + 1)) {
    int sg, mloc0, n0;
    tile_seg(L, &sg, &mloc0, &n0);
    const ConvSeg& S = a.seg[sg];
    if (sg != c_sg) {
      c_sg = sg;
      const int W = S.Wr, H = S.Hr;
      HWr = H * W;
      const HGeo G = h_geo(H, W);
      prow = G.pitch * BK * 2;
#pragma unroll
      for (int i = 0; i < TM; ++i) {
        const int r = wm * WM + i * 16 + lr;
        const int ii = r / HWr, q = r - ii * HWr;
        const int yy = q / W, xx = q - yy * W;
        const int hy = 1 + (G.whole ? (ii / G.mx) * (H + 1) : 0) + yy;
        const int hx = 1 + (G.whole ? (ii % G.mx) * (W + 1) : 0) + xx;
        const int pc = hy * G.pitch + hx;
#pragma unroll
        for (int d = 0; d < 3; ++d) {
          const int pp = pc + d - 1;
          afr[i][d] = (unsigned)(pp * BK * 2 + ((lg ^ swz4(pp)) * 16));
        }
      }
    }
    s16x8 zpre[BnSumPre<BN, NT>::N];
    BnSumPar bpar;
    float bcol[TN];
    float bq[SW ? TN : 1][4];
    s16x8 zq[SW && BSUM ? TM : 1];
    if constexpr (SW) {
      const int img = mloc0 / HWr;
      if ((a.stats || BSUM) && (img != k_img || n0 != k_n0)) {
        sw_flush();
        k_img = img;
        k_n0 = n0;
        if (BSUM) {
#pragma unroll
          for (int u = 0; u < CPL; ++u) {
            const int c = min(n0 + wn * WN + lgo + u, a.n_store - 1);
            const long bc = (long)img * a.n_store + c;
            pm[u] = a.bmr[bc * 2];
            prs[u] = a.bmr[bc * 2 + 1];
            pga[u] = a.bga[c];
            pbe[u] = a.bbe[c];
          }
        }
      }
#pragma unroll
      for (int j = 0; j < TN; ++j)
#pragma unroll
        for (int e = 0; e < 4; ++e) {
          const int n = n0 + wn * WN + j * 16 + 4 * lg + e;
          bq[j][e] = (S.bias && n < a.n_store) ? S.bias[n] : 0.f;
        }
      if (BSUM) {
#pragma unroll
        for (int i = 0; i < TM; ++i) {
          const long row = S.dst_base + mloc0 + wm * WM + i * 16 + lr;
          const cvl_bf16* zp = a.bz + row * a.ld_dst + a.dst_coff + n0 + wn * WN + lgo;
          if constexpr (TN == 2) {
            zq[i] = *reinterpret_cast<const s16x8*>(zp);
          } else {
            const s16x4 z4 = *reinterpret_cast<const s16x4*>(zp);
            zq[i] = s16x8{z4[0], z4[1], z4[2], z4[3], 0, 0, 0, 0};
          }
        }
      }
    } else {
      if constexpr (BSUM) bnsum_prefetch<BN, NT>(a, S, tid, n0, mloc0, zpre, bpar);
      epi_bias<BN, WGM, TN>(a, S, n0, wn, lane, bcol);
    }
    f32x4 acc[TM][TN];
#pragma unroll
    for (int i = 0; i < TM; ++i)
#pragma unroll
      for (int j = 0; j < TN; ++j) acc[i][j] = f32x4{0.f, 0.f, 0.f, 0.f};

    s16x8 fa[2][TM], fb[2][TN];
    auto read_tap = [&](int buf, const char* Hc, int t) {
      const int r = t / 3, sx = t - 3 * (t / 3);
      const int d = DGRAD ? 2 - sx : sx;
      const char* Hr = Hc + (DGRAD ? 1 - r : r - 1) * prow;
      const char* Wt = WRES ? reinterpret_cast<const char*>(wres + c_cb * WT_EL) + t * BN * BK * 2
                            : Hc + HALO_ELk * 2 + t * BN * BK * 2;
#pragma unroll
      for (int i = 0; i < TM; ++i) fa[buf][i] = *reinterpret_cast<const s16x8*>(Hr + afr[i][d]);
#pragma unroll
      for (int j = 0; j < TN; ++j) fb[buf][j] = *reinterpret_cast<const s16x8*>(Wt + bfr[j]);
    };
    auto mma_tap = [&](int buf) {
#pragma unroll
      for (int i = 0; i < TM; ++i)
#pragma unroll
        for (int j = 0; j < TN; ++j)
          acc[i][j] = SW ? __builtin_amdgcn_mfma_f32_16x16x32_bf16(__builtin_bit_cast(bf16x8, fb[buf][j]),
                                                                    __builtin_bit_cast(bf16x8, fa[buf][i]), acc[i][j], 0, 0, 0)
                         : __builtin_amdgcn_mfma_f32_16x16x32_bf16(__builtin_bit_cast(bf16x8, fa[buf][i]),
                                                                    __builtin_bit_cast(bf16x8, fb[buf][j]), acc[i][j], 0, 0, 0);
    };
    for (int cb = cb0; cb < cb1; ++cb) {
      const char* Hc = reinterpret_cast<const char*>(lds + (gb % NSTG) * SST);
      c_cb = cb;
      const bool more = i_L < t_hi;
      cvl_bf16* nh = lds + ((gb + NSTG - 1) % NSTG) * SST;
      const unsigned cbo = (unsigned)(i_cb * BK * 2);
      if (ST && stamp) c0 = __builtin_amdgcn_s_memtime();
      read_tap(0, Hc, 0);
#pragma unroll
      for (int t = 0; t < 9; ++t) {
        const bool iss = NSTG == 3 || more;
        if (iss && t < HPWk) dma16(rsA, nh + (wave + 8 * t) * 16 * BK, more ? hoff[t] + cbo : kOOB);
        if (!WRES && iss && t >= HPWk && t < HPWk + WJ)
          dma16(rsB, nh + HALO_ELk + (wave + 8 * (t - HPWk)) * 16 * BK, more ? woff[t - HPWk] + cbo : kOOB);
        if (!WRES && WR && t == 8 && iss && wave < WR) dma16(rsB, nh + HALO_ELk + (wave + 8 * WJ) * 16 * BK, more ? woff[WJ] + cbo : kOOB);
        if (t < 8) read_tap((t + 1) & 1, Hc, t + 1);
        mma_tap(t & 1);
      }
      if (more) advance();
      unsigned long long c1 = 0;
      if (ST && stamp) {
        c1 = __builtin_amdgcn_s_memtime();
        t_tap += c1 - c0;
      }
      if constexpr (NSTG == 3) {
        if (pw_blk == HPWk + WJ + 1) wait_vm<HPWk + WJ + 1>();
        else wait_vm<HPWk + WJ>();
      } else {
        wait_vm<0>();
      }
      __builtin_amdgcn_s_barrier();
      asm volatile("" ::: "memory");
      if (ST && stamp) t_wait += __builtin_amdgcn_s_memtime() - c1;
      ++gb;
    }
    if (a.splits > 1) {
      const int m0 = mloc0 + S.m_start;
      float* slab = a.slab + (size_t)blockIdx.z * a.m_total * a.Npad;
#pragma unroll
      for (int i = 0; i < TM; ++i)
#pragma unroll
        for (int j = 0; j < TN; ++j)
#pragma unroll
          for (int e = 0; e < 4; ++e) {
            const int rr = m0 + wm * WM + i * 16 + lg * 4 + e;
            const int c = n0 + wn * WN + j * 16 + lr;
            slab[(size_t)rr * a.Npad + c] = acc[i][j][e];
          }
      continue;
    }
    if constexpr (SW) {
      if (ST && stamp) c0 = __builtin_amdgcn_s_memtime();
      const bool dense = S.dst_img == (long)HWr;
      const int n = n0 + wn * WN + lgo;
#pragma unroll
      for (int i = 0; i < TM; ++i) {
        const int ml = mloc0 + wm * WM + i * 16 + lr;
        long drow;
        if (dense) {
          drow = S.dst_base + ml;
        } else {
          const int img = ml / HWr, q = ml - img * HWr;
          drow = conv_dst_row(a, S, img, q);
        }
        unsigned pk[2][2];
#pragma unroll
        for (int jj = 0; jj < TN; ++jj)
#pragma unroll
          for (int h = 0; h < 2; ++h) {
            float v0 = acc[i][jj][2 * h] + bq[jj][2 * h];
            float v1 = acc[i][jj][2 * h + 1] + bq[jj][2 * h + 1];
            if (a.relu_out) { v0 = fmaxf(v0, 0.f); v1 = fmaxf(v1, 0.f); }
            const unsigned u = __builtin_bit_cast(unsigned, __builtin_convertvector((f32x2){v0, v1}, bf16x2));
            pk[jj][h] = u;
            if (!BSUM && a.stats) {
              const float r0 = __uint_as_float(u << 16), r1 = __uint_as_float(u & 0xffff0000u);
              ss1[jj][2 * h] += r0;
              ss2[jj][2 * h] = __builtin_fmaf(r0, r0, ss2[jj][2 * h]);
              ss1[jj][2 * h + 1] += r1;
              ss2[jj][2 * h + 1] = __builtin_fmaf(r1, r1, ss2[jj][2 * h + 1]);
            }
          }
        if constexpr (TN == 2) {
#pragma unroll
          for (int h = 0; h < 2; ++h) {
            const auto sw = __builtin_amdgcn_permlane16_swap(pk[0][h], pk[1][h], false, false);
            pk[0][h] = sw[0];
            pk[1][h] = sw[1];
          }
        } else {
          pk[1][0] = pk[1][1] = 0u;
        }
        if (n >= a.n_store) continue;
        const s16x8 o = __builtin_bit_cast(s16x8, (u32x4){pk[0][0], pk[0][1], pk[1][0], pk[1][1]});
        if (BSUM) {
#pragma unroll
          for (int u = 0; u < CPL; ++u) {
            const float zf = bf16_to_f32((cvl_bf16)zq[i][u]);
            const float xh = (zf - pm[u]) * prs[u];
            const float af = __builtin_fmaf(pga[u], xh, pbe[u]);
            const float g = (af > 0.f && af < a.bhi) ? bf16_to_f32((cvl_bf16)o[u]) : 0.f;
            bs1[u] += g;
            bs2[u] = __builtin_fmaf(g, xh, bs2[u]);
          }
        }
        cvl_bf16* op = reinterpret_cast<cvl_bf16*>(a.dst) + drow * a.ld_dst + a.dst_coff + n;
        if constexpr (TN == 2) {
          *reinterpret_cast<s16x8*>(op) = o;
        } else {
          *reinterpret_cast<s16x4*>(op) = s16x4{o[0], o[1], o[2], o[3]};
        }
      }
      if (ST && stamp) {
        t_epi += __builtin_amdgcn_s_memtime() - c0;
        ++n_tile;
      }
      continue;
    }
    if (ST && stamp) {
      c0 = __builtin_amdgcn_s_memtime();
    }
    conv_l_epilogue<BN, WGM, TM, TN, NT, BSUM>(a, S, acc, lds + ((gb + NSTG - 1) % NSTG) * SST, tid, wm, wn, n0, mloc0,
                                                HWr, zpre, bpar, bcol, (ST && stamp) ? te : nullptr);
    __builtin_amdgcn_s_barrier();
    asm volatile("" ::: "memory");
    if (ST && stamp) {
      t_epi += __builtin_amdgcn_s_memtime() - c0;
      ++n_tile;
    }
  }
  sw_flush();
  wait_vm<0>();
  if (ST && stamp) {
    stamp[0] = w0;
    stamp[1] = w1;
    stamp[2] = (te[0] & 0xffff) | ((te[1] & 0xffff) << 16) | ((te[2] & 0xffff) << 32) | ((te[3] & 0xffff) << 48);
    stamp[3] = wall_clock64();
    stamp[4] = t_tap;
    stamp[5] = t_wait;
    stamp[6] = t_epi;
    stamp[7] = n_tile;
  }
}

static_assert(WRES_CB == kConvHWresCb && HPX >= 512, "conv_dispatch.hip plans with these");

template <bool DG, bool BS, bool ST>
void h_launch64(const ConvPlan& p, const ConvArgs& a, hipStream_t s) {
  const dim3 grid(p.grid, 1, p.splits);
  with_bool(p.wres, [&](auto WR) {
    with_bool(p.sw, [&](auto SW) {
      hipLaunchKernelGGL((conv_igemm_h_kernel<DG, BS, decltype(WR)::value, ST, decltype(SW)::value>), grid, dim3(NT), 0,
                         s, a);
    });
  });
}

template <bool DG, bool BS, bool SW>
void h_launch32(const ConvPlan& p, const ConvArgs& a, hipStream_t s) {
  if (p.stages == 3) hipLaunchKernelGGL((conv_igemm_h_kernel<DG, BS, false, false, SW, 32, 3>), dim3(p.grid), dim3(NT), 0, s, a);
  else hipLaunchKernelGGL((conv_igemm_h_kernel<DG, BS, false, false, SW, 32>), dim3(p.grid), dim3(NT), 0, s, a);
}

template <bool ST>
void h_launch(const ConvPlan& p, const ConvArgs& a, hipStream_t s) {
  if (p.bn == 32 && !p.sw) h_launch32<false, false, false>(p, a, s);
  else if (p.bn == 32 && p.dgrad && p.bsum) h_launch32<true, true, true>(p, a, s);
  else if (p.bn == 32 && p.dgrad) h_launch32<true, false, true>(p, a, s);
  else if (p.bn == 32) h_launch32<false, false, true>(p, a, s);
  else if (p.dgrad && p.bsum) h_launch64<true, true, ST>(p, a, s);
  else if (p.dgrad) h_launch64<true, false, ST>(p, a, s);
  else h_launch64<false, false, ST>(p, a, s);
}

}

#ifdef CVL_MEASURE
int g_h_stamp_grid = 0;

extern "C" int cvl_debug_h_stamps(uint64_t* host, int max_wgs) {
  if (max_wgs < 0) return g_h_stamp_grid = 0;
  const int n = g_h_stamp_grid < max_wgs ? g_h_stamp_grid : max_wgs;
  if (n <= 0 || !host) return g_h_stamp_grid;
  if (hipDeviceSynchronize() != hipSuccess) return CVL_EHIP;
  if (hipMemcpyFromSymbol(host, HIP_SYMBOL(g_h_stamps), (size_t)n * 64, 0, hipMemcpyDeviceToHost) != hipSuccess)
    return CVL_EHIP;
  return g_h_stamp_grid;
}
#endif

bool cvl_conv_h_fits(const cvl_conv_desc* d, const ConvArgs& a, int* halo_px) {
  *halo_px = 0;
  if (d->KH != 3 || d->KW != 3 || d->stride != 1 || d->pad_t != 1 || d->pad_l != 1 || a.Cin % BK ||
      (a.Npad % BN && a.Npad != 32) || a.relu_in || a.dst_up != 1)
    return false;
  if (a.Npad == 32 && (d->mode != CVL_CONV_FWD || !d->dst_f32)) return false;
  for (int i = 0; i < a.nseg; ++i) {
    const ConvSeg& q = a.seg[i];
    if (q.Hr != q.Hs || q.Wr != q.Ws) return false;
    const int W = q.Wr, HW = q.Hr * q.Wr;
    if (HW >= BM ? (BM % W || HW % BM) : (BM % HW)) return false;
    const HGeo g = h_geo(q.Hr, W);
    if (g.mx * g.my * (g.whole ? HW : BM) != BM || g.rows * g.pitch > HPX) return false;
    if (g.rows * g.pitch > *halo_px) *halo_px = g.rows * g.pitch;
    const long src_bytes = (q.src_base + (long)a.B * q.src_img) * a.Cin * 2;
    if (src_bytes >= (long)kRecords - 65536) return false;
  }
  return (long)a.Npad * a.K * 2 < (long)kRecords;
}

int launch_h(const ConvPlan& p, const ConvArgs& a, hipStream_t s) {
#ifdef CVL_MEASURE
  if (p.stamps) {
    g_h_stamp_grid = p.grid;
    h_launch<true>(p, a, s);
  } else
#endif
  {
    h_launch<false>(p, a, s);
  }
  return cvl_launch_status();
}
```

cv-lite-object-detection_amd/csrc/conv_igemm_x.hip:

```cpp
#include "conv_common.h"
#include "conv_epilogue.h"

namespace {

constexpr int BM = 256, BN = 256, NT = 512;
constexpr int WGM = 2, WM = 128, WN = 64, TM = 8, TN = 4;
constexpr int LDS_C = BM * (BN + 8);
constexpr unsigned kRecords = 0x7fffffffu;
constexpr unsigned kOOB = 0x80000000u;

__device__ __forceinline__ void dma16(__amdgpu_buffer_rsrc_t r, const cvl_bf16* lds_dst, unsigned voff) {
  __builtin_amdgcn_raw_ptr_buffer_load_lds(r, (__attribute__((address_space(3))) void*)lds_dst, 16, (int)voff, 0,
                                           0, 0);
}

constexpr int BK32 = 32;
constexpr int SLOT = 2 * 256 * BK32;
constexpr int NSLOT = 5;
constexpr int LDS32_EL = NSLOT * SLOT > LDS_C ? NSLOT * SLOT : LDS_C;

__device__ __forceinline__ int swz4(int r) { return (r >> 1) & 3; }

typedef __bf16 bf16x2 __attribute__((ext_vector_type(2)));
typedef float f32x2 __attribute__((ext_vector_type(2)));
typedef unsigned u32x4 __attribute__((ext_vector_type(4)));

template <bool DGRAD, bool DBG, bool SW>
__device__ __forceinline__ void x32_body(const ConvArgs& a) {
  const int dbg = DBG ? a.dbg : 0;
  __shared__ __attribute__((aligned(16))) cvl_bf16 lds[LDS32_EL];
  unsigned long long* stamp = (DBG && (dbg & 256) && threadIdx.x == 0)
                                  ? reinterpret_cast<unsigned long long*>(a.dst) + (size_t)blockIdx.x * 4 : nullptr;
  if (stamp) stamp[0] = wall_clock64();

  const int tid = threadIdx.x;
  const int wave = __builtin_amdgcn_readfirstlane(tid >> 6), lane = tid & 63;
  const int ntn = a.Npad / BN;
  const int L = xcd_remap(blockIdx.x, gridDim.x);
  const int m_tile = L / ntn, n_tile = L % ntn;
  const int m0 = m_tile * BM, n0 = n_tile * BN;
  int sg = 0;
#pragma unroll
  for (int i = 1; i < kMaxSeg; ++i)
    if (i < a.nseg && m0 >= a.seg[i].m_start) sg = i;
  const ConvSeg& S = a.seg[sg];
  const int HWr = S.Hr * S.Wr;
  const int mloc0 = m0 - S.m_start;
  if (mloc0 >= S.rows) return;

  const int Cin = a.Cin, KW = a.KW, T = a.KH * a.KW, Ws = S.Ws, Hs = S.Hs;
  const int Kdim = a.K;
  const int nk = Kdim / BK32;
  const int x16 = wave * 16 + (lane >> 2), ch = lane & 3;
  const unsigned chs = (unsigned)((ch ^ swz4(x16)) * 16);
  unsigned aoff[2], amask[2];
#pragma unroll
  for (int p = 0; p < 2; ++p) {
    const int ml = mloc0 + p * 128 + x16;
    const int img = ml / HWr, q = ml - img * HWr;
    const int oy = q / S.Wr, ox = q - (q / S.Wr) * S.Wr;
    const int y0 = DGRAD ? oy + a.pad_t : oy * a.stride - a.pad_t;
    const int x0 = DGRAD ? ox + a.pad_l : ox * a.stride - a.pad_l;
    const long pix = S.src_base + (long)img * S.src_img + (long)y0 * Ws + x0;
    aoff[p] = (unsigned)(pix * Cin * 2) + chs;
    unsigned cm = 0, m = 0;
    for (int s = 0; s < KW; ++s) {
      const int ix = DGRAD ? x0 - s : x0 + s;
      if (ix >= 0 && ix < Ws) cm |= 1u << s;
    }
    for (int r = 0; r < a.KH; ++r) {
      const int iy = DGRAD ? y0 - r : y0 + r;
      if (iy >= 0 && iy < Hs) m |= cm << (r * KW);
    }
    amask[p] = ml < S.rows ? m : 0u;
  }
  const unsigned boff0 = (unsigned)((n0 + x16) * Kdim * 2) + chs;
  const __amdgpu_buffer_rsrc_t rsA = __builtin_amdgcn_make_buffer_rsrc((void*)a.src, (short)0, (int)kRecords, 0x00020000);
  const __amdgpu_buffer_rsrc_t rsB = __builtin_amdgcn_make_buffer_rsrc((void*)S.w, (short)0, (int)kRecords, 0x00020000);

  const int dsgn = DGRAD ? -1 : 1;
  int kc = 0, ctap = 0, cr = 0, cs = 0, ccb = 0, cslot = 0;
  unsigned cak = 0, cbk = 0;
  auto issue_piece = [&](int q) {
    if (dbg & 32) return;
    const bool live = kc < nk;
    cvl_bf16* Ab = lds + cslot * SLOT;
    cvl_bf16* Bb = Ab + 256 * BK32;
    if (q < 2) {
      const bool v = live && ((amask[q] >> ctap) & 1u) && !(dbg & 1);
      dma16(rsA, Ab + (q * 128 + wave * 16) * BK32, v ? aoff[q] + cak : kOOB);
    } else {
      const int p = q - 2;
      dma16(rsB, Bb + (p * 128 + wave * 16) * BK32,
            live && !(dbg & 2) ? boff0 + (unsigned)(p * 128 * Kdim * 2) + cbk : kOOB);
    }
  };
  auto advance = [&]() {
    ++kc;
    cslot = cslot == NSLOT - 1 ? 0 : cslot + 1;
    ++ctap;
    if (++cs == KW) { cs = 0; ++cr; }
    if (ctap == T) { ctap = 0; cr = 0; cs = 0; ++ccb; }
    cak = (unsigned)(dsgn * (cr * Ws + cs) * Cin * 2 + ccb * 64);
    cbk = (unsigned)((ctap * Cin + ccb * 32) * 2);
  };
  auto issue = [&]() {
#pragma unroll
    for (int q = 0; q < 4; ++q) issue_piece(q);
    advance();
  };

  const int wm = wave >> 2, wn = wave & 3;
  const int lr = lane & 15, lg = lane >> 4;
  float bq[SW ? TN : 1][4];
  if constexpr (SW) {
#pragma unroll
    for (int j = 0; j < TN; ++j)
#pragma unroll
      for (int e = 0; e < 4; ++e) {
        const int n = n0 + wn * WN + j * 16 + 4 * lg + e;
        bq[j][e] = (S.bias && n < a.n_store) ? S.bias[n] : 0.f;
      }
  }
  f32x4 acc[TM][TN];
#pragma unroll
  for (int i = 0; i < TM; ++i)
#pragma unroll
    for (int j = 0; j < TN; ++j) acc[i][j] = f32x4{0.f, 0.f, 0.f, 0.f};
  auto bar = [&]() {
    if (!(dbg & 512)) __builtin_amdgcn_s_barrier();
    asm volatile("" ::: "memory");
  };

  issue();
  issue();
  issue();
  wait_vm<8>();
  __builtin_amdgcn_s_barrier();
  asm volatile("" ::: "memory");
  if (wm == 1) bar();
  unsigned long long clk0 = 0;
  if (stamp) { stamp[1] = wall_clock64(); clk0 = __builtin_amdgcn_s_memtime(); }

  int rslot = 0;
  for (int kt = 0; kt < nk; ++kt) {
    if (!(dbg & 16)) wait_vm<4>();
    issue();
    const cvl_bf16* Ac = lds + rslot * SLOT;
    const cvl_bf16* Bc = Ac + 256 * BK32;
    s16x8 fa[TM], fb[TN];
    if (dbg & 64) {
#pragma unroll
      for (int i = 0; i < TM; ++i) fa[i] = s16x8{(short)lr, 0, 0, 0, 0, 0, 0, (short)kt};
#pragma unroll
      for (int j = 0; j < TN; ++j) fb[j] = s16x8{(short)j, 0, 0, 0, 0, 0, 0, (short)lg};
    } else {
#pragma unroll
      for (int i = 0; i < TM; ++i) {
        const int r = wm * WM + i * 16 + lr;
        fa[i] = *reinterpret_cast<const s16x8*>(Ac + r * BK32 + ((lg ^ swz4(r)) * 8));
      }
#pragma unroll
      for (int j = 0; j < TN; ++j) {
        const int r = wn * WN + j * 16 + lr;
        fb[j] = *reinterpret_cast<const s16x8*>(Bc + r * BK32 + ((lg ^ swz4(r)) * 8));
      }
    }
    bar();
    asm volatile("s_waitcnt lgkmcnt(0)" ::: "memory");
    __builtin_amdgcn_sched_barrier(0);
    __builtin_amdgcn_s_setprio(1);
    if (dbg & 4) {
      asm volatile("" ::"v"(fa[0]), "v"(fb[0]), "v"(fa[TM - 1]), "v"(fb[TN - 1]));
    } else {
#pragma unroll
      for (int i = 0; i < TM; ++i) {
#pragma unroll
        for (int j = 0; j < TN; ++j)
          acc[i][j] = SW ? __builtin_amdgcn_mfma_f32_16x16x32_bf16(__builtin_bit_cast(bf16x8, fb[j]),
                                                                    __builtin_bit_cast(bf16x8, fa[i]), acc[i][j], 0, 0, 0)
                         : __builtin_amdgcn_mfma_f32_16x16x32_bf16(__builtin_bit_cast(bf16x8, fa[i]),
                                                                    __builtin_bit_cast(bf16x8, fb[j]), acc[i][j], 0, 0, 0);
      }
    }
    __builtin_amdgcn_s_setprio(0);
    __builtin_amdgcn_sched_barrier(0);
    bar();
    rslot = rslot == NSLOT - 1 ? 0 : rslot + 1;
  }
  if (wm == 0) bar();
  wait_vm<0>();
  if (stamp) { stamp[2] = wall_clock64(); stamp[3] = __builtin_amdgcn_s_memtime() - clk0; }
  if (dbg & 8) {
    if (acc[0][0][0] == 12345.f) reinterpret_cast<float*>(a.dst)[1] = 1.f;
    return;
  }
  if constexpr (SW) {
    const int lgo = ((lg & 1) ? 16 : 0) + ((lg & 2) ? 8 : 0);
    const bool dense = S.dst_img == (long)HWr;
#pragma unroll
    for (int i = 0; i < TM; ++i) {
      const int ml = mloc0 + wm * WM + i * 16 + lr;
      if (ml >= S.rows) continue;
      long drow;
      if (dense) {
        drow = S.dst_base + ml;
      } else {
        const int img = ml / HWr, q = ml - img * HWr;
        drow = conv_dst_row(a, S, img, q);
      }
      s16x8 ym[TN / 2];
      if (a.ymask) {
#pragma unroll
        for (int jp = 0; jp < TN / 2; ++jp) {
          const int n = min(n0 + wn * WN + jp * 32 + lgo, a.n_store - 8);
          ym[jp] = *reinterpret_cast<const s16x8*>(a.ymask + drow * a.ld_dst + a.dst_coff + n);
        }
      }
#pragma unroll
      for (int jp = 0; jp < TN / 2; ++jp) {
        unsigned pk[2][2];
#pragma unroll
        for (int jj = 0; jj < 2; ++jj)
#pragma unroll
          for (int h = 0; h < 2; ++h) {
            float v0 = acc[i][2 * jp + jj][2 * h] + bq[2 * jp + jj][2 * h];
            float v1 = acc[i][2 * jp + jj][2 * h + 1] + bq[2 * jp + jj][2 * h + 1];
            if (a.relu_out) { v0 = fmaxf(v0, 0.f); v1 = fmaxf(v1, 0.f); }
            pk[jj][h] = __builtin_bit_cast(unsigned, __builtin_convertvector((f32x2){v0, v1}, bf16x2));
          }
#pragma unroll
        for (int h = 0; h < 2; ++h) {
          const auto sw = __builtin_amdgcn_permlane16_swap(pk[0][h], pk[1][h], false, false);
          pk[0][h] = sw[0];
          pk[1][h] = sw[1];
        }
        const int n = n0 + wn * WN + jp * 32 + lgo;
        if (n >= a.n_store) continue;
        s16x8 o = __builtin_bit_cast(s16x8, (u32x4){pk[0][0], pk[0][1], pk[1][0], pk[1][1]});
        if (a.ymask) {
#pragma unroll
          for (int u = 0; u < 8; ++u) o[u] = bf16_to_f32((cvl_bf16)ym[jp][u]) > 0.f ? o[u] : (short)0;
        }
        *reinterpret_cast<s16x8*>(reinterpret_cast<cvl_bf16*>(a.dst) + drow * a.ld_dst + a.dst_coff + n) = o;
      }
    }
    return;
  }
  const s16x8 znone[1] = {s16x8{0, 0, 0, 0, 0, 0, 0, 0}};
  conv_l_epilogue<BN, WGM, TM, TN, NT>(a, S, acc, lds, tid, wm, wn, n0, mloc0, HWr, znone, BnSumPar{});
}

template <bool DGRAD, bool DBG = false, bool SW = false>
__global__ void __launch_bounds__(NT) conv_igemm_x32_kernel(ConvArgs a) {
  if (a.probe) probe_enter(a.probe);
  x32_body<DGRAD, DBG, SW>(a);
  if (a.probe) probe_leave(a.probe);
}

}

int launch_x(const ConvPlan& p, const ConvArgs& a, hipStream_t s) {
  const dim3 grid(p.grid);
  with_bool(p.dgrad, [&](auto DG) {
    with_bool(p.sw, [&](auto SW) {
#ifdef CVL_MEASURE
      if (p.dbg)
        hipLaunchKernelGGL((conv_igemm_x32_kernel<decltype(DG)::value, true, decltype(SW)::value>), grid, dim3(NT), 0, s, a);
      else
#endif
        hipLaunchKernelGGL((conv_igemm_x32_kernel<decltype(DG)::value, false, decltype(SW)::value>), grid, dim3(NT), 0, s, a);
    });
  });
  return cvl_launch_status();
}
```

cv-lite-object-detection_amd/cvlite/_lib.py:

```python
import ctypes
import os

import torch

_HERE = os.path.dirname(os.path.abspath(__file__))
LIB_PATH = os.environ.get("CVL_LIB") or os.path.join(_HERE, "libcvlite_hip.so")


def dispatch(key, default=0):
    for tok in os.environ.get("CVL_DISPATCH", "").split(","):
        k, _, v = tok.strip().partition("=")
        if k == key:
            return int(v) if v else 1
    return default

c_int, c_float, c_size_t, c_void_p = ctypes.c_int, ctypes.c_float, ctypes.c_size_t, ctypes.c_void_p
P = c_void_p

SIGNATURES = {
    "cvl_version": (c_int, []),
    "cvl_fcos_assign": (c_int, [P, P, P, c_int, c_int, c_int, c_int, c_int, P, P, P, P, P]),
    "cvl_fcos_loss_workspace_size": (c_size_t, [c_int, c_int]),
    "cvl_fcos_loss": (c_int, [P, c_int, P, c_int, P, c_int, c_int, c_int, c_int, c_float, P,
                              P, c_int, c_int, P, c_int, c_int, P, c_size_t, P]),
    "cvl_fcos_loss_ex": (c_int, [P, c_int, P, c_int, P, c_int, c_int, c_int, c_int, c_float, c_float, c_float,
                                 c_float, P, P, c_int, c_int, P, c_int, c_int, P, c_size_t, P]),
    "cvl_fcos_paper_assign": (c_int, [P, P, P, c_int, c_int, c_int, c_int, c_int, P, P, c_float, P, P, P]),
    "cvl_fcos_target_norm_workspace_size": (c_size_t, [c_int, c_int]),
    "cvl_fcos_target_norm": (c_int, [P, c_int, c_int, c_int, P, P, c_size_t, P]),
    "cvl_fcos_paper_loss": (c_int, [P, c_int, P, c_int, P, P, c_int, c_int, c_int, c_float, c_float, c_float, P,
                                    P, c_int, c_int, P, c_int, c_int, P, c_size_t, P]),
    "cvl_fcos_atss_workspace_size": (c_size_t, [c_int, c_int]),
    "cvl_fcos_atss_assign": (c_int, [P, P, P, c_int, c_int, c_int, c_int, c_int, P, c_int, c_float, P, P, P, P, P,
                                     P, c_size_t, P]),
    "cvl_retina_atss_workspace_size": (c_size_t, [c_int, c_int, c_int]),
    "cvl_retina_atss_assign": (c_int, [P, P, P, c_int, c_int, c_int, c_int, P, c_int, P, c_int, P, P, P, P, P, P,
                                       c_size_t, P]),
    "cvl_retina_atss_loss_workspace_size": (c_size_t, [c_int, c_int, c_int]),
    "cvl_retina_atss_loss": (c_int, [P, c_int, P, c_int, P, P, P, c_int, c_int, c_int, c_int, c_float, c_float,
                                     c_float, P, P, c_int, c_int, P, c_int, c_int, P, c_size_t, P]),
    "cvl_fcos_gfl_norm_workspace_size": (c_size_t, [c_int, c_int]),
    "cvl_fcos_gfl_norm": (c_int, [P, c_int, P, c_int, c_int, c_int, P, P, c_size_t, P]),
    "cvl_fcos_gfl_loss_workspace_size": (c_size_t, [c_int, c_int]),
    "cvl_fcos_gfl_loss": (c_int, [P, c_int, P, c_int, P, P, c_int, c_int, c_int, c_int, c_float, c_float, c_float,
                                  c_float, P, P, c_int, c_int, P, c_int, c_int, P, c_size_t, P]),
    "cvl_fcos_gfl_decode": (c_int, [P, c_int, c_int, c_int, P, c_int, P]),
    "cvl_centernet_gauss_assign": (c_int, [P, P, P, c_int, c_int, c_int, c_int, c_int, c_int, c_float, P, P]),
    "cvl_centernet_gauss_norm": (c_int, [P, c_int, c_int, c_int, P, P]),
    "cvl_centernet_gauss_loss_workspace_size": (c_size_t, [c_int, c_int]),
    "cvl_centernet_gauss_loss": (c_int, [P, c_int, P, P, c_int, c_int, c_int, c_float, c_float, c_float, c_float,
                                         P, P, c_int, P, P]),
    "cvl_fcos_decode": (c_int, [P, c_int, c_int, c_int, ctypes.c_double, P, P]),
    "cvl_fcos_v1_decode": (c_int, [P, c_int, c_int, c_int, c_float, c_float, P, P]),
    "cvl_conv_igemm_workspace_size": (c_size_t, [P]),
    "cvl_conv_igemm": (c_int, [P, P, P, P, P, c_size_t, P]),
    "cvl_conv_igemm_relu_mask": (c_int, [P, P, P, P, P, c_size_t, P]),
    "cvl_conv_igemm_res_relu": (c_int, [P, P, P, P, c_size_t, P]),
    "cvl_conv_igemm_res_relu_plan": (c_int, [P, c_size_t, P, P]),
    "cvl_pack_conv_weights_scaled_multi": (c_int, [P, P, c_int, P]),
    "cvl_relu_": (c_int, [P, ctypes.c_long, P]),
    "cvl_conv_igemm_last_kernel": (c_int, []),
    "cvl_conv_igemm_last_ktile": (c_int, []),
    "cvl_conv_igemm_plan": (c_int, [P, c_int, c_size_t, P, P]),
    "cvl_conv_igemm_plan_grid": (c_int, [P, c_int, c_int, c_size_t, P, P, P, P]),
    "cvl_conv_kernel_name": (ctypes.c_char_p, [c_int]),
    "cvl_conv_igemm_plan_bnsum": (c_int, [P, c_int, c_size_t, P, P, P]),
    "cvl_conv_igemm_dgrad_bnsum_res_bits": (c_int, [P, P, P, P, P, P, P, P, P, P, P, P, P, ctypes.c_size_t, P]),
    "cvl_bn_finalize_apply_bits": (c_int, [P, P, P, P, P, P, P, P, P, P, c_int, c_int, c_int, c_int, c_float,
                                           c_float, P]),
    "cvl_bn_finalize_apply_bnres_bits": (c_int, [P, P, P, P, P, P, P, P, P, P, P, P, P, P, c_float, c_float, P, P,
                                                 c_int, c_int, c_int, c_int, c_float, c_float, P]),
    "cvl_bn_backward_bits": (c_int, [P, P, P, P, P, P, c_size_t, P, P, P, P, c_float, P, c_int, c_int, c_int, P]),
    "cvl_bn_backward_res_sums_bits": (c_int, [P, P, P, P, P, P, P, P, P, P, c_float, P, c_int, c_int, c_int, P]),
    "cvl_bn_backward_res_sums_sc_bits": (c_int, [P, P, P, P, P, P, P, P, P, P, c_float, P, P, P, P, c_size_t, P,
                                                 c_int, c_int, c_int, P]),
    "cvl_bn_backward_sc_bits": (c_int, [P, P, P, P, P, P, c_size_t, P, P, P, P, c_float, P, P, P, P, c_int, c_int,
                                        c_int, P]),
    "cvl_centernet_peak_decode_workspace_size": (ctypes.c_size_t, [c_int, c_int, c_int, c_int]),
    "cvl_centernet_peak_decode": (c_int, [P, c_int, c_int, c_int, c_int, c_int, c_float, c_float, c_int, P, P, P,
                                          ctypes.c_size_t, P]),
    "cvl_conv_igemm_dgrad_bnsum": (c_int, [P, P, P, P, P, P, P, c_float, P, P, P, ctypes.c_size_t, P]),
    "cvl_bn_backward_relu_sums": (c_int, [P, P, P, P, P, P, P, P, P, c_float, P, c_float, c_int, c_int, c_int, P]),
    "cvl_conv_igemm_dgrad_bnsum_res": (c_int, [P, P, P, P, P, P, P, P, P, P, P, ctypes.c_size_t, P]),
    "cvl_bn_backward_res_sums": (c_int, [P, P, P, P, P, P, P, P, P, P, c_float, P, c_int, c_int, c_int, P]),
    "cvl_bn_backward_res_sums_sc_workspace_size": (c_size_t, [c_int, c_int, c_int]),
    "cvl_bn_backward_res_sums_sc": (c_int, [P, P, P, P, P, P, P, P, P, P, c_float, P, P, P, P, c_size_t, P, c_int,
                                            c_int, c_int, P]),
    "cvl_bn_backward_sums": (c_int, [P, P, P, P, P, P, P, P, c_float, P, c_int, c_int, c_int, P]),
    "cvl_bn_backward_sc_workspace_size": (c_size_t, [c_int, c_int, c_int]),
    "cvl_bn_backward_sc": (c_int, [P, P, P, P, P, P, c_size_t, P, P, P, P, c_float, P, P, P, P, c_int, c_int, c_int, P]),
    "cvl_probe_arm": (c_int, [P]),
    "cvl_probe_clock_hz": (ctypes.c_double, []),
    "cvl_conv_wgrad_workspace_size": (c_size_t, [P]),
    "cvl_conv_wgrad": (c_int, [P, P, P, P, c_float, P, c_size_t, P]),
    "cvl_conv_wgrad_grouped_workspace_size": (c_size_t, [P, c_int]),
    "cvl_conv_wgrad_grouped": (c_int, [P, c_int, P, P, P, c_float, P, c_size_t, P]),
    "cvl_conv_wgrad_batch_workspace_size": (c_size_t, [P, c_int]),
    "cvl_conv_wgrad_batch": (c_int, [P, c_int, P, P, P, c_float, P, c_size_t, P]),
    "cvl_conv_wgrad_plan": (c_int, [P, c_int, P, P, P, P]),
    "cvl_conv_wgrad_batch_plan": (c_int, [P, c_int, P, P, P]),
    "cvl_pack_conv_weights": (c_int, [P, c_int, c_int, c_int, c_int, c_int, c_int, P, c_int, c_int, P, P]),
    "cvl_pack_conv_weights_multi": (c_int, [P, P, c_int, P]),
    "cvl_im2col": (c_int, [P, c_int, c_int, c_int, c_int, c_int, c_int, c_int, c_int, c_int, c_int,
                           c_int, c_int, P, P]),
    "cvl_bn_finalize": (c_int, [P, P, P, P, c_int, c_int, c_int, c_float, c_float, P]),
    "cvl_bn_acc_decode": (c_int, [P, P, ctypes.c_int64, P]),
    "cvl_bn_set_exact": (c_int, [c_int]),
    "cvl_bn_acc_slots": (c_int, []),
    "cvl_stem_conv7x7s2": (c_int, [P, c_int, c_int, c_int, P, P, P, P, P]),
    "cvl_stem_wgrad_workspace_size": (c_size_t, [c_int, c_int, c_int]),
    "cvl_stem_wgrad": (c_int, [P, c_int, c_int, c_int, P, P, c_float, P, c_size_t, P]),
    "cvl_bn_apply": (c_int, [P, P, P, P, P, P, c_int, c_int, c_int, c_int, P]),
    "cvl_bn_finalize_apply": (c_int, [P, P, P, P, P, P, P, P, P, c_int, c_int, c_int, c_int, c_float, c_float, P]),
    "cvl_bn_finalize_apply_bnres": (c_int, [P, P, P, P, P, P, P, P, P, P, P, P, P, P, c_float, c_float, P, c_int,
                                            c_int, c_int, c_int, c_float, c_float, P]),
    "cvl_bn_backward_workspace_size": (c_size_t, [c_int, c_int, c_int]),
    "cvl_bn_backward": (c_int, [P, P, P, P, P, P, c_size_t, P, P, P, P, c_float, P, c_int, c_int, c_int, P]),
    "cvl_bn_backward_relu": (c_int, [P, P, P, P, P, P, c_size_t, P, P, P, c_float, P, c_int, c_int, c_int, P]),
    "cvl_maxpool3x3s2": (c_int, [P, P, P, c_int, c_int, c_int, c_int, P]),
    "cvl_bn_relu_maxpool3x3s2": (c_int, [P, P, P, P, P, P, c_int, c_int, c_int, c_int, P]),
    "cvl_maxpool3x3s2_backward": (c_int, [P, P, P, c_int, c_int, c_int, c_int, P]),
    "cvl_maxpool3x3s2_backward_bn_relu_workspace_size": (c_size_t, [c_int, c_int, c_int, c_int]),
    "cvl_maxpool3x3s2_backward_bn_relu": (c_int, [P, P, P, P, P, P, P, c_size_t, P, P, P, P, c_float, P, c_int, c_int,
                                                  c_int, c_int, P]),
    "cvl_upsample2x_add": (c_int, [P, P, P, c_int, c_int, c_int, c_int, P]),
    "cvl_upsample2x_backward": (c_int, [P, P, c_int, c_int, c_int, c_int, c_float, P]),
    "cvl_relu_backward": (c_int, [P, P, P, ctypes.c_long, c_float, P]),
    "cvl_add": (c_int, [P, P, P, ctypes.c_long, P]),
    "cvl_bias_grad_workspace_size": (c_size_t, [c_int, c_int, c_int]),
    "cvl_bias_grad_multi_workspace_size": (c_size_t, [P, c_int]),
    "cvl_bias_grad_multi": (c_int, [P, c_int, P, c_size_t, P]),
    "cvl_bias_grad": (c_int, [P, c_int, c_int, c_int, ctypes.c_int64, ctypes.c_int64, c_int, c_int, P, c_size_t,
                              P, c_float, P]),
    "cvl_wgrad_defer": (c_int, [c_int, P]),
    "cvl_wgrad_flush": (c_int, [P]),
    "cvl_sgd_clip_update": (c_int, [P, P, P, ctypes.c_int64, P, c_float, c_float, c_float, P, P]),
    "cvl_lr_schedule": (c_int, [P, P, ctypes.c_double, ctypes.c_double, ctypes.c_double, c_int, P]),
    "cvl_lr_schedule_capped": (c_int, [P, P, ctypes.c_double, ctypes.c_double, ctypes.c_double, c_int, c_int, P]),
    "cvl_l2_params_reg": (c_int, [P, P, P, c_int, P, P, P]),
    "cvl_select_first_nonzero": (c_int, [P, c_int, c_int, P, P, P]),
    "cvl_gather_rows": (c_int, [P, ctypes.c_int64, P, c_int, P, P]),
    "cvl_retina_assign": (c_int, [P, P, P, c_int, c_int, c_int, c_int, P, c_int, P, c_float, P, P, P]),
    "cvl_centernet_assign": (c_int, [P, P, P, c_int, c_int, c_int, c_int, c_int, c_int, P, P]),
    "cvl_center_dist": (c_int, [P, P, c_int, ctypes.c_double, ctypes.c_double, ctypes.c_double, P, P]),
    "cvl_centernet_splat": (c_int, [P, P, P, c_int, c_int, c_int, c_int, c_int, c_int, c_float, P, P]),
    "cvl_det_loss_workspace_size": (c_size_t, [c_int, c_int]),
    "cvl_det_loss": (c_int, [P, c_int, P, c_int, P, c_int, c_int, c_int, c_float, c_float, P, P, P, P, P]),
    "cvl_retina_loss_workspace_size": (c_size_t, [c_int, c_int, c_int]),
    "cvl_retina_loss": (c_int, [P, c_int, P, c_int, P, c_int, P, c_int, c_int, P, c_float, P, P, c_int, P, c_int,
                                P, P]),
    "cvl_bn_stats_workspace_size": (c_size_t, [c_int, c_int, c_int]),
    "cvl_bn_stats": (c_int, [P, c_int, c_int, c_int, P, P, c_size_t, P]),
    "cvl_bn_finalize_grouped": (c_int, [P, P, P, P, c_int, c_int, c_int, c_int, c_float, c_float, P]),
    "cvl_bn_backward_grouped_workspace_size": (c_size_t, [c_int, c_int, c_int]),
    "cvl_bn_backward_grouped": (c_int, [P, P, P, P, P, P, c_size_t, P, c_float, P, P, c_int, c_int, c_int, c_int, P]),
    "cvl_maxpool2x2": (c_int, [P, P, P, c_int, c_int, c_int, c_int, P]),
    "cvl_maxpool2x2_backward": (c_int, [P, P, P, c_int, c_int, c_int, c_int, P]),
    "cvl_upsample_bilinear2x_add": (c_int, [P, P, P, c_int, c_int, c_int, c_int, P]),
    "cvl_upsample_bilinear2x_backward": (c_int, [P, P, c_int, c_int, c_int, c_int, c_float, P]),
    "cvl_upsample_bilinear2x_sum": (c_int, [P, P, P, c_int, c_int, c_int, c_int, P]),
    "cvl_bn_backward_relu6": (c_int, [P, P, P, P, P, P, c_size_t, P, P, P, c_float, P, c_int, c_int, c_int, P]),
    "cvl_depthwise_fwd": (c_int, [P, P, P, c_int, c_int, c_int, c_int, c_int, c_int, c_int, c_int, c_int, c_int, P]),
    "cvl_depthwise_dgrad": (c_int, [P, P, P, c_int, c_int, c_int, c_int, c_int, c_int, c_int, c_int, c_int, c_int,
                                    c_float, P]),
    "cvl_depthwise_wgrad_workspace_size": (c_size_t, [c_int, c_int, c_int, c_int, c_int]),
    "cvl_depthwise_wgrad": (c_int, [P, P, P, c_float, c_int, c_int, c_int, c_int, c_int, c_int, c_int, c_int, c_int,
                                    c_int, P, c_size_t, P]),
    "cvl_gconv3x3_packed_bytes": (c_size_t, [c_int]),
    "cvl_gconv3x3_pack": (c_int, [P, c_int, c_int, P, P, P]),
    "cvl_gconv3x3_fwd": (c_int, [P, P, P, P, c_int, c_int, c_int, c_int, c_int, c_int, c_int, c_int, P]),
    "cvl_gconv3x3_dgrad": (c_int, [P, P, P, c_int, c_int, c_int, c_int, c_int, c_int, c_int, c_int, c_float, P]),
    "cvl_gconv3x3_wgrad_workspace_size": (c_size_t, [c_int, c_int, c_int, c_int, c_int, c_int]),
    "cvl_gconv3x3_wgrad": (c_int, [P, P, P, c_float, c_int, c_int, c_int, c_int, c_int, c_int, c_int, c_int, P,
                                   c_size_t, P]),
    "cvl_gconv3x3_plan": (c_int, [c_int, c_int, c_int, c_int, c_int, c_int, c_int, P, P, P, P, P, P]),
    "cvl_bn_data_stats_workspace_size": (c_size_t, [c_int]),
    "cvl_bn_data_stats": (c_int, [P, c_int, c_int, c_int, c_float, c_float, P, P, P, P, c_size_t, P]),
    "cvl_bn_data_apply": (c_int, [P, P, P, P, c_int, c_int, c_int, P]),
    "cvl_reshape_concat": (c_int, [P, c_int, c_int, c_int, P, c_int, P]),
    "cvl_reshape_concat_backward": (c_int, [P, c_int, c_int, c_int, P, c_int, P]),
    "cvl_bias_scalar_fold_periodic": (c_int, [P, P, P, c_int, c_int, c_int, P]),
    "cvl_bias_scalar_unfold_periodic": (c_int, [P, P, P, c_int, c_int, c_int, P]),
    "cvl_hourglass_v2_assign": (c_int, [P, P, c_int, c_int, c_int, c_int, c_int, P, P]),
    "cvl_centernet_s8_assign": (c_int, [P, P, P, c_int, c_int, c_int, c_int, c_int, P, c_int, c_int, P, P]),
    "cvl_centernet_s8_loss_workspace_size": (c_size_t, [c_int, c_int, c_int]),
    "cvl_centernet_s8_loss": (c_int, [P, c_int, P, c_int, P, c_int, c_int, c_int, c_int, c_float, c_float, P, P, c_int,
                                      P, c_int, P, P]),
    "cvl_hourglass_v2_loss_workspace_size": (c_size_t, [c_int, c_int]),
    "cvl_hourglass_v2_loss": (c_int, [P, c_int, P, c_int, c_int, c_int, c_int, c_float, c_float, P, P, c_int, P, P]),
    "cvl_sep_fold_multi": (c_int, [P, P, c_int, P]),
    "cvl_sep_unfold_multi": (c_int, [P, P, c_int, P]),
    "cvl_bias_scalar_fold": (c_int, [P, P, P, c_int, c_int, P]),
    "cvl_bias_scalar_unfold": (c_int, [P, P, P, c_int, c_int, P]),
    "cvl_centernet_loss": (c_int, [P, c_int, P, c_int, c_int, c_int, c_float, c_float, P, P, c_int, P, P]),
    "cvl_adam_clip_update": (c_int, [P, P, P, P, ctypes.c_int64, P, P, c_float, c_float, c_float, c_float, c_float,
                                     P, P]),
    "cvl_centernet_decode": (c_int, [P, c_int, c_int, c_int, c_int, ctypes.c_double, c_float, ctypes.c_double,
                                     ctypes.c_double, ctypes.c_double, ctypes.c_double, P, P, P]),
    "cvl_centernet_scale_decode": (c_int, [P, c_int, c_int, c_int, c_int, c_int, c_int, c_int, c_int, P, c_float,
                                           c_float, ctypes.c_double, ctypes.c_double, ctypes.c_double,
                                           ctypes.c_double, P, P, P]),
    "cvl_nms_workspace_size": (c_size_t, [c_int, c_int]),
    "cvl_nms": (c_int, [P, c_int, P, c_int, ctypes.c_double, P, P, P, P]),
    "cvl_soft_nms_workspace_size": (c_size_t, [c_int, c_int]),
    "cvl_soft_nms": (c_int, [P, c_int, P, c_int, ctypes.c_double, P, P, P, P, P]),
    "cvl_retina_corners": (c_int, [P, c_int, c_int, c_int, c_float, c_float, c_int, P, P]),
    "cvl_retina_decode_workspace_size": (c_size_t, [c_int, P, c_int]),
    "cvl_retina_decode": (c_int, [P, c_int, P, c_int, c_int, P, P, P, c_int, c_int, c_float, P, P, P, c_size_t,
                                  P]),
    "cvl_retina_nms_workspace_size": (c_size_t, [c_int, c_int]),
    "cvl_retina_nms": (c_int, [P, c_int, P, c_int, c_int, c_float, P, P, P, P]),
    "cvl_fcos_center_assign": (c_int, [P, P, P, c_int, c_int, c_int, c_int, c_int, P, P, c_int, P, P, P]),
    "cvl_fcos_center_v1_assign": (c_int, [P, P, P, c_int, c_int, c_int, c_int, c_int, P, P, P, P, P]),
    "cvl_resize_pad_normalize": (c_int, [P, c_int, c_int, c_int, c_int, c_int, c_int, c_int, c_int, c_int, P, P]),
    "cvl_image_augment_workspace_size": (c_size_t, [c_int, c_int]),
    "cvl_image_augment": (c_int, [P, P, P, P, P, P, c_int, c_int, c_int, c_int, P, c_size_t, P]),
    "cvl_fcos_detect_workspace_size": (c_size_t, [c_int, c_int, c_int, c_int]),
    "cvl_fcos_detect": (c_int, [P, c_int, P, c_int, c_int, P, P, c_int, c_int, c_float, c_float, c_int, c_int, P, P,
                                P, P, P, c_size_t, P]),
    "cvl_eval_match": (c_int, [P, P, P, P, P, P, P, P, P, c_int, c_int, c_int, c_int, P, c_int, c_int, c_int, P, P, P,
                               P, P, ctypes.c_int64, P, P]),
    "cvl_eval_ap": (c_int, [P, P, P, P, ctypes.c_int64, c_int, c_int, c_int, P, P, P]),
    "cvl_eval_match_areas": (c_int, [P, P, P, P, P, P, P, P, P, c_int, c_int, c_int, c_int, P, c_int, c_int, c_int,
                                     P, c_int, P, P, P, P, P, P, P, P, ctypes.c_int64, P, P]),
    "cvl_eval_ap_views": (c_int, [P, P, P, P, P, ctypes.c_int64, c_int, c_int, c_int, P, c_int, P, P, P]),
    "cvl_jpeg_info": (c_int, [P, c_size_t, P]),
    "cvl_jpeg_entropy_decode": (c_int, [P, c_size_t, P, c_size_t, P]),
    "cvl_jpeg_batch_sizes": (c_int, [P, c_int, P, P]),
    "cvl_jpeg_decode_batch": (c_int, [P, P, c_int, P, P, c_size_t, P, c_size_t, P, P]),
    "cvl_bn_apply_f32": (c_int, [P, P, P, P, P, P, c_int, c_int, c_int, c_int, P]),
    "cvl_bn_finalize_apply_f32": (c_int, [P, P, P, P, P, P, P, P, P, c_int, c_int, c_int, c_int, c_float, c_float,
                                          P]),
    "cvl_bn_backward_f32_workspace_size": (c_size_t, [c_int, c_int]),
    "cvl_bn_backward_f32": (c_int, [P, P, P, P, P, P, P, c_size_t, P, P, P, P, c_float, P, c_float, c_int, c_int,
                                    c_int, P]),
    "cvl_maxpool3x3s2_f32": (c_int, [P, P, P, c_int, c_int, c_int, c_int, P]),
    "cvl_maxpool3x3s2_backward_f32": (c_int, [P, P, P, c_int, c_int, c_int, c_int, P]),
    "cvl_upsample2x_add_f32": (c_int, [P, P, P, c_int, c_int, c_int, c_int, P]),
    "cvl_upsample2x_backward_f32": (c_int, [P, P, c_int, c_int, c_int, c_int, c_float, P]),
    "cvl_relu_backward_f32": (c_int, [P, P, P, ctypes.c_long, c_float, P]),
    "cvl_add_f32": (c_int, [P, P, P, ctypes.c_long, P]),
    "cvl_bias_grad_multi_f32": (c_int, [P, c_int, P]),
    "cvl_retina_loss_f32": (c_int, [P, c_int, P, c_int, P, c_int, P, c_int, c_int, P, c_float, P, P, c_int, P, c_int,
                                    P, P]),
}


class CvlError(RuntimeError):
    pass


_lib = None


NEWER = {"cvl_conv_igemm_last_ktile", "cvl_conv_igemm_plan", "cvl_conv_igemm_plan_bnsum", "cvl_conv_igemm_plan_grid",
         "cvl_conv_igemm_dgrad_bnsum_res_bits", "cvl_bn_finalize_apply_bits", "cvl_bn_finalize_apply_bnres_bits",
         "cvl_bn_backward_bits", "cvl_bn_backward_res_sums_bits", "cvl_bn_backward_res_sums_sc_bits",
         "cvl_bn_backward_sc_bits", "cvl_conv_wgrad_plan", "cvl_conv_wgrad_batch_plan", "cvl_conv_igemm_res_relu",
         "cvl_conv_igemm_res_relu_plan", "cvl_pack_conv_weights_scaled_multi", "cvl_relu_", "cvl_eval_match_areas",
         "cvl_eval_ap_views", "cvl_fcos_atss_workspace_size", "cvl_fcos_atss_assign", "cvl_gconv3x3_plan",
         "cvl_fcos_gfl_norm_workspace_size", "cvl_fcos_gfl_norm", "cvl_fcos_gfl_loss_workspace_size",
         "cvl_fcos_gfl_loss", "cvl_fcos_gfl_decode", "cvl_retina_atss_workspace_size", "cvl_retina_atss_assign",
         "cvl_retina_atss_loss_workspace_size", "cvl_retina_atss_loss", "cvl_centernet_gauss_assign",
         "cvl_centernet_gauss_norm", "cvl_centernet_gauss_loss_workspace_size", "cvl_centernet_gauss_loss"}


def load():
    global _lib
    if _lib is None:
        if not os.path.exists(LIB_PATH):
            raise CvlError("cvlite native library not built (%s): run __graft_entry__.build() or "
                           "make -C cv-lite-object-detection_amd/csrc" % LIB_PATH)
        lib = ctypes.CDLL(LIB_PATH)
        for name, (res, args) in SIGNATURES.items():
            if name in NEWER and os.environ.get("CVL_LIB") and not hasattr(lib, name):
                continue
            fn = getattr(lib, name)
            fn.restype = res
            fn.argtypes = args
        _lib = lib
        if os.environ.get("CVL_BN_EXACT", "0") == "1":
            lib.cvl_bn_set_exact(1)
    return _lib


def call(name, *args):
    st = getattr(load(), name)(*args)
    if st != 0:
        if st >= 1000:
            raise CvlError("%s failed: hipError %d" % (name, st - 1000))
        raise CvlError("%s: invalid argument (status %d)" % (name, st))
    return True


def ptr(t):
    return None if t is None else c_void_p(t.data_ptr())


def stream():
    return c_void_p(torch.cuda.current_stream().cuda_stream)


def require_cuda(*tensors):
    if not torch.cuda.is_available():
        raise CvlError("cvlite ops need an MI355X GPU (no CPU fallback)")
    for t in tensors:
        if t is not None and not t.is_cuda:
            raise CvlError("cvlite ops take device tensors")
        if t is not None and not t.is_contiguous():
            raise CvlError("cvlite ops take contiguous tensors")
```

include/cvlite.h:

```cpp
#ifndef CVLITE_H_
#define CVLITE_H_

#include <stddef.h>
#include <stdint.h>

#ifdef __cplusplus
extern "C" {
#endif

typedef void* cvl_stream_t;

enum { CVL_OK = 0, CVL_EINVAL = 1, CVL_EHIP = 1000 };

int cvl_version(void);

int cvl_fcos_assign(const float* boxes, const int32_t* nbox, const float* img_dim, int B, int n_max,
                    int pad_h, int pad_w, int num_classes, const int32_t* strides ,
                    const float* size_bounds , float* targets, int32_t* num_targets,
                    cvl_stream_t stream);

size_t cvl_fcos_loss_workspace_size(int B, int P);
int cvl_fcos_loss(const float* reg_pred, int ld_reg, const float* cls_pred, int ld_cls,
                  const float* targets, int B, int P, int num_classes, int reg_type,
                  float grad_scale, float* losses, void* d_reg, int ld_dreg, int dreg_dtype,
                  void* d_cls, int ld_dcls, int dcls_dtype, void* workspace, size_t workspace_bytes,
                  cvl_stream_t stream);
int cvl_fcos_loss_ex(const float* reg_pred, int ld_reg, const float* cls_pred, int ld_cls,
                     const float* targets, int B, int P, int num_classes, int reg_type,
                     float grad_scale, float alpha, float gamma, float delta, float* losses, void* d_reg,
                     int ld_dreg, int dreg_dtype, void* d_cls, int ld_dcls, int dcls_dtype, void* workspace,
                     size_t workspace_bytes, cvl_stream_t stream);

int cvl_fcos_decode(const float* pred, int ld, int S0, int S1, double stride, double* out,
                    cvl_stream_t stream);
int cvl_fcos_v1_decode(const float* pred, int ld, int S0, int S1, float box_sc, float stride, double* out,
                       cvl_stream_t stream);


int cvl_fcos_center_assign(const float* boxes, const int32_t* nbox, const float* img_dim, int B, int n_max,
                           int pad_h, int pad_w, int num_classes, const int32_t* strides, const float* b_dim,
                           int center_only, float* targets, int32_t* num_targets, cvl_stream_t stream);
int cvl_fcos_center_v1_assign(const float* boxes, const int32_t* nbox, const float* img_dim, int B, int n_max,
                              int pad_h, int pad_w, int num_classes, const int32_t* strides, const float* b_dim,
                              float* targets, int32_t* num_targets, cvl_stream_t stream);

int cvl_fcos_paper_assign(const float* boxes, const int32_t* nbox, const float* img_dim, int B, int n_max,
                          int pad_h, int pad_w, int num_classes, const int32_t* strides ,
                          const float* size_bounds , float center_radius, float* targets,
                          int32_t* num_targets, cvl_stream_t stream);
size_t cvl_fcos_target_norm_workspace_size(int B, int P);
int cvl_fcos_target_norm(const float* targets, int B, int P, int num_classes, float* norm, void* workspace,
                         size_t workspace_bytes, cvl_stream_t stream);
int cvl_fcos_paper_loss(const float* reg_pred, int ld_reg, const float* cls_pred, int ld_cls,
                        const float* targets, const float* norm, int B, int P, int num_classes,
                        float grad_scale, float alpha, float gamma, float* losses, void* d_reg, int ld_dreg,
                        int dreg_dtype, void* d_cls, int ld_dcls, int dcls_dtype, void* workspace,
                        size_t workspace_bytes, cvl_stream_t stream);

size_t cvl_fcos_atss_workspace_size(int B, int P);
int cvl_fcos_atss_assign(const float* boxes, const int32_t* nbox, const float* img_dim, int B, int n_max,
                         int pad_h, int pad_w, int num_classes, const int32_t* strides , int topk,
                         float anchor_scale, float* targets, int32_t* num_targets, int32_t* cand_cells,
                         float* cand_iou, double* cand_thr, void* workspace, size_t workspace_bytes,
                         cvl_stream_t stream);

size_t cvl_retina_atss_workspace_size(int B, int P, int n_anchors);
int cvl_retina_atss_assign(const float* boxes, const int32_t* nbox, const float* img_dim, int B, int n_max, int pad,
                           int num_classes, const float* anchor_dims, int n_anchors,
                           const int32_t* strides , int topk, float* targets, int32_t* num_targets,
                           int32_t* cand_idx, float* cand_iou, double* cand_thr, void* workspace,
                           size_t workspace_bytes, cvl_stream_t stream);
size_t cvl_retina_atss_loss_workspace_size(int B, int P, int n_anchors);
int cvl_retina_atss_loss(const float* reg_pred, int ld_reg, const float* cls_pred, int ld_cls, const float* targets,
                         const int32_t* num_targets, const float* img_weight, int B, int P, int n_anchors,
                         int num_classes, float grad_scale, float alpha, float gamma, float* losses, void* d_reg,
                         int ld_dreg, int dreg_dtype, void* d_cls, int ld_dcls, int dcls_dtype, void* workspace,
                         size_t workspace_bytes, cvl_stream_t stream);

size_t cvl_fcos_gfl_norm_workspace_size(int B, int P);
int cvl_fcos_gfl_norm(const float* cls_pred, int ld_cls, const float* targets, int B, int P, int num_classes,
                      float* norm, void* workspace, size_t workspace_bytes, cvl_stream_t stream);
size_t cvl_fcos_gfl_loss_workspace_size(int B, int P);
int cvl_fcos_gfl_loss(const float* reg_pred, int ld_reg, const float* cls_pred, int ld_cls,
                      const float* targets, const float* norm, int B, int P, int num_classes, int reg_max,
                      float grad_scale, float beta, float w_box, float w_dfl, float* losses, void* d_reg,
                      int ld_dreg, int dreg_dtype, void* d_cls, int ld_dcls, int dcls_dtype, void* workspace,
                      size_t workspace_bytes, cvl_stream_t stream);
int cvl_fcos_gfl_decode(const float* reg_pred, int ld_reg, int rows, int reg_max, float* out, int ld_out,
                        cvl_stream_t stream);

int cvl_centernet_gauss_assign(const float* boxes, const int32_t* nbox, const float* img_dim, int B, int n_max,
                               int pad_h, int pad_w, int num_classes, int stride, float min_overlap,
                               float* targets, cvl_stream_t stream);
int cvl_centernet_gauss_norm(const float* targets, int B, int P, int num_classes, int32_t* npos,
                             cvl_stream_t stream);
size_t cvl_centernet_gauss_loss_workspace_size(int B, int P);
int cvl_centernet_gauss_loss(const float* pred, int ld_pred, const float* targets, const int32_t* npos, int B,
                             int P, int num_classes, float alpha, float beta, float cls_scale, float reg_scale,
                             float* losses, void* d_pred, int ld_d, void* workspace, cvl_stream_t stream);

#define CVL_BN_ACC_SLOTS 8
int cvl_bn_set_exact(int on);
int cvl_bn_acc_slots(void);
int cvl_bn_acc_decode(const uint64_t* acc, double* out, int64_t n, cvl_stream_t stream);
#define CVL_CONV_MAX_SEG 10
enum { CVL_CONV_FWD = 0, CVL_CONV_DGRAD = 1 };

typedef struct {
  int Hr, Wr;
  int Hs, Ws;
  int64_t src_base, src_img;
  int64_t dst_base, dst_img;
  const void* w;
  const float* bias;
} cvl_conv_seg;

typedef struct {
  int mode;
  int B;
  int Cin;
  int KH, KW, stride, pad_t, pad_l;
  int Npad;
  int n_store;
  int ld_dst, dst_coff;
  int dst_f32;
  int relu_out;
  int relu_in;
  float beta;
  int nseg;
  cvl_conv_seg seg[CVL_CONV_MAX_SEG];
  int prec;
} cvl_conv_desc;
enum { CVL_PREC_BF16 = 0, CVL_PREC_F32 = 1 };

size_t cvl_conv_igemm_workspace_size(const cvl_conv_desc* d);
int cvl_conv_igemm(const cvl_conv_desc* d, const void* src, void* dst, uint64_t* bn_stats,
                   void* workspace, size_t workspace_bytes, cvl_stream_t stream);
int cvl_conv_igemm_relu_mask(const cvl_conv_desc* d, const void* src, void* dst, const void* y, void* workspace,
                             size_t workspace_bytes, cvl_stream_t stream);
int cvl_conv_igemm_res_relu(const cvl_conv_desc* d, const void* src, void* dst, void* workspace,
                            size_t workspace_bytes, cvl_stream_t stream);
int cvl_conv_igemm_res_relu_plan(const cvl_conv_desc* d, size_t workspace_bytes, int32_t* kernel, int32_t* fused);

enum { CVL_CK_NONE = 0, CVL_CK_BASE = 1, CVL_CK_BASE_SPLITK = 2, CVL_CK_L64 = 3, CVL_CK_L128 = 4,
       CVL_CK_L256 = 5, CVL_CK_X256 = 6, CVL_CK_X32 = 7,
       CVL_CK_WG_S = 8, CVL_CK_WG_L128 = 9, CVL_CK_WG_L256 = 10, CVL_CK_WG_X = 11, CVL_CK_X32H = 12, CVL_CK_WG_SN = 13,
       CVL_CK_H64 = 14, CVL_CK_WG_H = 15, CVL_CK_P = 16 };
int cvl_conv_igemm_last_kernel(void);
int cvl_conv_igemm_last_ktile(void);
int cvl_conv_igemm_plan(const cvl_conv_desc* d, int with_bn_stats, size_t workspace_bytes, int32_t* kernel,
                        int32_t* ktile);
int cvl_conv_igemm_plan_grid(const cvl_conv_desc* d, int with_bn_stats, int bsum_offer, size_t workspace_bytes,
                             int32_t* kernel, int32_t* ktile, int32_t* grid, int32_t* ntile);
const char* cvl_conv_kernel_name(int code);

int cvl_probe_arm(uint64_t* slot);
double cvl_probe_clock_hz(void);

size_t cvl_conv_wgrad_workspace_size(const cvl_conv_desc* d);
int cvl_conv_wgrad(const cvl_conv_desc* d, const void* x, const void* dy, float* dw, float beta,
                   void* workspace, size_t workspace_bytes, cvl_stream_t stream);

int cvl_wgrad_defer(int on, cvl_stream_t stream);
int cvl_wgrad_flush(cvl_stream_t stream);
size_t cvl_conv_wgrad_grouped_workspace_size(const cvl_conv_desc* d, int ngroups);
int cvl_conv_wgrad_grouped(const cvl_conv_desc* d, int ngroups, const void* x, const void* dy, float* const* dw,
                           float beta, void* workspace, size_t workspace_bytes, cvl_stream_t stream);

size_t cvl_conv_wgrad_batch_workspace_size(const cvl_conv_desc* const* d, int n);
int cvl_conv_wgrad_batch(const cvl_conv_desc* const* d, int n, const void* const* x, const void* const* dy,
                         float* const* dw, float beta, void* workspace, size_t workspace_bytes, cvl_stream_t stream);

int cvl_conv_wgrad_plan(const cvl_conv_desc* d, int ngroups, int32_t* kernel, int32_t* tile, int32_t* nsplit,
                        size_t* workspace);
int cvl_conv_wgrad_batch_plan(const cvl_conv_desc* const* d, int n, int32_t* kernel_of, int32_t* launch_of,
                              int32_t* nsplit_of);

int cvl_pack_conv_weights(const float* w_hwio, int KH, int KW, int Cin, int Cout, int Cin_k, int Npad,
                          void* w_fwd, int Cin_pad, int Cout_pad, void* w_dgrad, cvl_stream_t stream);

typedef struct {
  const float* w;
  void* w_fwd;
  void* w_dgrad;
  int KHW, Cin, Cout, Cin_k, Npad, Cin_pad, Cout_pad;
  int f32_out;
} cvl_pack_item;
int cvl_pack_conv_weights_multi(const cvl_pack_item* items, const int32_t* tiles, int ntiles,
                                cvl_stream_t stream);
typedef struct {
  const float* w;
  const float* scale;
  void* w_fwd;
  int KHW, Cin, Cout, Cin_k, Npad;
} cvl_pack_scaled_item;
int cvl_pack_conv_weights_scaled_multi(const cvl_pack_scaled_item* items, const int32_t* tiles, int ntiles,
                                       cvl_stream_t stream);

int cvl_stem_conv7x7s2(const float* img, int B, int H, int W, const void* w_packed, const float* bias, void* z,
                       uint64_t* bn_stats, cvl_stream_t stream);
size_t cvl_stem_wgrad_workspace_size(int B, int H, int W);
int cvl_stem_wgrad(const float* img, int B, int H, int W, const void* dz, float* dw, float beta, void* workspace,
                   size_t workspace_bytes, cvl_stream_t stream);

int cvl_im2col(const float* x, int B, int H, int W, int C, int KH, int KW, int stride, int pad_t,
               int pad_l, int Ho, int Wo, int Kp, void* out, cvl_stream_t stream);

int cvl_bn_finalize(uint64_t* stats, float* mean_rstd, float* run_mean, float* run_var, int B,
                    int C, int HW, float eps, float momentum, cvl_stream_t stream);
int cvl_bn_apply(const void* z, const float* mean_rstd, const float* gamma, const float* beta,
                 const void* residual, void* y, int B, int HW, int C, int relu, cvl_stream_t stream);
int cvl_bn_finalize_apply(uint64_t* stats, float* mean_rstd, float* run_mean, float* run_var,
                          const void* z, const float* gamma, const float* beta, const void* residual, void* y,
                          int B, int HW, int C, int relu, float eps, float momentum, cvl_stream_t stream);
int cvl_bn_finalize_apply_bnres(uint64_t* stats, float* mean_rstd, float* run_mean, float* run_var,
                                const void* z, const float* gamma, const float* beta, uint64_t* res_stats,
                                float* res_mean_rstd, float* res_run_mean, float* res_run_var,
                                const void* res_z, const float* res_gamma, const float* res_beta,
                                float res_eps, float res_momentum, void* y, int B, int HW, int C, int relu,
                                float eps, float momentum, cvl_stream_t stream);
size_t cvl_bn_backward_workspace_size(int B, int HW, int C);
int cvl_bn_backward(const void* dy, const void* y_relu, const void* z, const float* mean_rstd,
                    const float* gamma, void* workspace, size_t workspace_bytes, void* dz, void* g_out,
                    float* dgamma, float* dbeta, float beta_acc, float* conv_dbias, int B, int HW, int C,
                    cvl_stream_t stream);
int cvl_bn_backward_relu(const void* dy, const void* z, const float* mean_rstd, const float* gamma,
                         const float* beta, void* workspace, size_t workspace_bytes, void* dz, float* dgamma,
                         float* dbeta, float beta_acc, float* conv_dbias, int B, int HW, int C,
                         cvl_stream_t stream);
int cvl_conv_igemm_dgrad_bnsum(const cvl_conv_desc* d, const void* src, void* dst, const void* z,
                               const float* mean_rstd, const float* gamma, const float* beta, float act_hi,
                               uint64_t* sums, int32_t* fused, void* workspace, size_t workspace_bytes,
                               cvl_stream_t stream);
int cvl_bn_backward_relu_sums(const void* dy, const void* z, const float* mean_rstd, const float* gamma,
                              const float* beta, uint64_t* sums, void* dz, float* dgamma, float* dbeta,
                              float beta_acc, float* conv_dbias, float act_hi, int B, int HW, int C,
                              cvl_stream_t stream);
int cvl_conv_igemm_dgrad_bnsum_res(const cvl_conv_desc* d, const void* src, void* dst, const void* y, const void* z,
                                   const float* mean_rstd, const float* gamma, const float* beta, uint64_t* sums,
                                   int32_t* fused, void* workspace, size_t workspace_bytes, cvl_stream_t stream);
int cvl_bn_backward_res_sums(const void* dy, const void* y, const void* z, const float* mean_rstd, const float* gamma,
                             uint64_t* sums, void* dz, void* g_out, float* dgamma, float* dbeta, float beta_acc,
                             float* conv_dbias, int B, int HW, int C, cvl_stream_t stream);
size_t cvl_bn_backward_res_sums_sc_workspace_size(int B, int HW, int C);
int cvl_bn_backward_res_sums_sc(const void* dy, const void* y, const void* z, const float* mean_rstd,
                                const float* gamma, uint64_t* sums, void* dz, void* g_out, float* dgamma,
                                float* dbeta, float beta_acc, float* conv_dbias, const void* z_sc,
                                const float* mean_rstd_sc, void* workspace, size_t workspace_bytes,
                                uint64_t* sc_sums, int B, int HW, int C, cvl_stream_t stream);
size_t cvl_bn_backward_sc_workspace_size(int B, int HW, int C);
int cvl_bn_backward_sc(const void* dy, const void* y, const void* z, const float* mean_rstd, const float* gamma,
                       void* workspace, size_t workspace_bytes, void* dz, void* g_out, float* dgamma, float* dbeta,
                       float beta_acc, float* conv_dbias, const void* z_sc, const float* mean_rstd_sc,
                       uint64_t* sc_sums, int B, int HW, int C, cvl_stream_t stream);
int cvl_bn_backward_sums(const void* dy, const void* z, const float* mean_rstd, const float* gamma,
                         const uint64_t* sums, void* dz, float* dgamma, float* dbeta, float beta_acc,
                         float* conv_dbias, int B, int HW, int C, cvl_stream_t stream);

int cvl_bn_finalize_apply_bits(uint64_t* stats, float* mean_rstd, float* run_mean, float* run_var, const void* z,
                               const float* gamma, const float* beta, const void* residual, void* y,
                               uint8_t* relu_bits, int B, int HW, int C, int relu, float eps, float momentum,
                               cvl_stream_t stream);
int cvl_bn_finalize_apply_bnres_bits(uint64_t* stats, float* mean_rstd, float* run_mean, float* run_var,
                                     const void* z, const float* gamma, const float* beta, uint64_t* res_stats,
                                     float* res_mean_rstd, float* res_run_mean, float* res_run_var,
                                     const void* res_z, const float* res_gamma, const float* res_beta,
                                     float res_eps, float res_momentum, void* y, uint8_t* relu_bits, int B, int HW,
                                     int C, int relu, float eps, float momentum, cvl_stream_t stream);
int cvl_bn_backward_bits(const void* dy, const uint8_t* relu_bits, const void* z, const float* mean_rstd,
                         const float* gamma, void* workspace, size_t workspace_bytes, void* dz, void* g_out,
                         float* dgamma, float* dbeta, float beta_acc, float* conv_dbias, int B, int HW, int C,
                         cvl_stream_t stream);
int cvl_bn_backward_res_sums_bits(const void* dy, const uint8_t* relu_bits, const void* z, const float* mean_rstd,
                                  const float* gamma, uint64_t* sums, void* dz, void* g_out, float* dgamma,
                                  float* dbeta, float beta_acc, float* conv_dbias, int B, int HW, int C,
                                  cvl_stream_t stream);
int cvl_bn_backward_res_sums_sc_bits(const void* dy, const uint8_t* relu_bits, const void* z, const float* mean_rstd,
                                     const float* gamma, uint64_t* sums, void* dz, void* g_out, float* dgamma,
                                     float* dbeta, float beta_acc, float* conv_dbias, const void* z_sc,
                                     const float* mean_rstd_sc, void* workspace, size_t workspace_bytes,
                                     uint64_t* sc_sums, int B, int HW, int C, cvl_stream_t stream);
int cvl_bn_backward_sc_bits(const void* dy, const uint8_t* relu_bits, const void* z, const float* mean_rstd,
                            const float* gamma, void* workspace, size_t workspace_bytes, void* dz, void* g_out,
                            float* dgamma, float* dbeta, float beta_acc, float* conv_dbias, const void* z_sc,
                            const float* mean_rstd_sc, uint64_t* sc_sums, int B, int HW, int C, cvl_stream_t stream);
int cvl_conv_igemm_dgrad_bnsum_res_bits(const cvl_conv_desc* d, const void* src, void* dst, const void* y,
                                        const uint8_t* relu_bits, const void* z, const float* mean_rstd,
                                        const float* gamma, const float* beta, uint64_t* sums, int32_t* fused,
                                        int32_t* form, void* workspace, size_t workspace_bytes, cvl_stream_t stream);
int cvl_conv_igemm_plan_bnsum(const cvl_conv_desc* d, int offer, size_t workspace_bytes, int32_t* form,
                              int32_t* kernel, int32_t* ktile);

int cvl_bn_backward_relu6(const void* dy, const void* z, const float* mean_rstd, const float* gamma,
                          const float* beta, void* workspace, size_t workspace_bytes, void* dz, float* dgamma,
                          float* dbeta, float beta_acc, float* conv_dbias, int B, int HW, int C, cvl_stream_t stream);

int cvl_bn_relu_maxpool3x3s2(const void* z, const float* mean_rstd, const float* gamma, const float* beta, void* y,
                             uint8_t* argmax, int B, int H, int W, int C, cvl_stream_t stream);
int cvl_maxpool3x3s2(const void* x, void* y, uint8_t* argmax, int B, int H, int W, int C,
                     cvl_stream_t stream);
int cvl_maxpool3x3s2_backward(const void* dy, const uint8_t* argmax, void* dx, int B, int H, int W,
                              int C, cvl_stream_t stream);
size_t cvl_maxpool3x3s2_backward_bn_relu_workspace_size(int B, int H, int W, int C);
int cvl_maxpool3x3s2_backward_bn_relu(const void* dp, const uint8_t* argmax, const void* z, const float* mean_rstd,
                                      const float* gamma, const float* beta, void* workspace,
                                      size_t workspace_bytes, void* dy, void* dz, float* dgamma, float* dbeta,
                                      float beta_acc, float* conv_dbias, int B, int H, int W, int C,
                                      cvl_stream_t stream);
int cvl_upsample2x_add(const void* a, const void* b, void* out, int B, int H, int W, int C,
                       cvl_stream_t stream);
int cvl_upsample2x_backward(const void* dout, void* db, int B, int H, int W, int C, float beta,
                            cvl_stream_t stream);
int cvl_relu_backward(const void* dy, const void* y, void* dx, long n, float beta, cvl_stream_t stream);
int cvl_relu_(void* x, long n, cvl_stream_t stream);
int cvl_add(const void* a, const void* b, void* out, long n, cvl_stream_t stream);
size_t cvl_bias_grad_workspace_size(int ncol, int HW, int B);
int cvl_bias_grad(const void* dy, int ld, int coff, int ncol, int64_t base, int64_t img_stride, int HW,
                  int B, void* workspace, size_t workspace_bytes, float* db, float beta, cvl_stream_t stream);
#define CVL_BIAS_MAX_ITEMS 16
typedef struct {
  const void* dy;
  float* db;
  int64_t base, img_stride;
  int ld, coff, ncol, HW, B;
  float beta;
} cvl_bias_item;
size_t cvl_bias_grad_multi_workspace_size(const cvl_bias_item* items, int n);
int cvl_bias_grad_multi(const cvl_bias_item* items, int n, void* workspace, size_t workspace_bytes,
                        cvl_stream_t stream);

int cvl_bn_apply_f32(const float* z, const float* mean_rstd, const float* gamma, const float* beta,
                     const float* residual, float* y, int B, int HW, int C, int relu, cvl_stream_t stream);
int cvl_bn_finalize_apply_f32(uint64_t* stats, float* mean_rstd, float* run_mean, float* run_var,
                              const float* z, const float* gamma, const float* beta, const float* residual,
                              float* y, int B, int HW, int C, int relu, float eps, float momentum,
                              cvl_stream_t stream);
size_t cvl_bn_backward_f32_workspace_size(int B, int C);
int cvl_bn_backward_f32(const float* dy, const float* y_relu, const float* z, const float* mean_rstd,
                        const float* gamma, const float* bn_beta, void* workspace, size_t workspace_bytes,
                        float* dz, float* g_out, float* dgamma, float* dbeta, float beta_acc,
                        float* conv_dbias, float act_hi, int B, int HW, int C, cvl_stream_t stream);
int cvl_maxpool3x3s2_f32(const float* x, float* y, uint8_t* argmax, int B, int H, int W, int C,
                         cvl_stream_t stream);
int cvl_maxpool3x3s2_backward_f32(const float* dy, const uint8_t* argmax, float* dx, int B, int H, int W,
                                  int C, cvl_stream_t stream);
int cvl_upsample2x_add_f32(const float* a, const float* b, float* out, int B, int H, int W, int C,
                           cvl_stream_t stream);
int cvl_upsample2x_backward_f32(const float* dout, float* db, int B, int H, int W, int C, float beta,
                                cvl_stream_t stream);
int cvl_relu_backward_f32(const float* dy, const float* y, float* dx, long n, float beta, cvl_stream_t stream);
int cvl_add_f32(const float* a, const float* b, float* out, long n, cvl_stream_t stream);
int cvl_bias_grad_multi_f32(const cvl_bias_item* items, int n, cvl_stream_t stream);
int cvl_retina_loss_f32(const float* reg_pred, int ld_reg, const float* cls_pred, int ld_cls, const float* targets,
                        int B, const int32_t* level_cells, int n_anchors, int num_classes, const float* img_weight,
                        float grad_scale, float* losses, float* d_reg, int ld_dreg, float* d_cls, int ld_dcls,
                        void* workspace, cvl_stream_t stream);

#define CVL_SUMSQ_WS 1025
int cvl_sgd_clip_update(float* w, const float* g, float* v, int64_t n, const float* lr_dev,
                        float momentum, float inv_bs, float clip, double* sumsq_ws, cvl_stream_t stream);
int cvl_lr_schedule(int32_t* step, float* lr, double init_lr, double min_lr, double decay_rate,
                    int decay_step, cvl_stream_t stream);
int cvl_lr_schedule_capped(int32_t* step, float* lr, double init_lr, double min_lr, double decay_rate,
                           int decay_step, int max_decays, cvl_stream_t stream);

int cvl_l2_params_reg(const float* flat, const int64_t* offsets, const int64_t* sizes, int n_tensors,
                      float* terms, float* out, cvl_stream_t stream);

int cvl_select_first_nonzero(const int32_t* counts, int n, int k, int32_t* idx, float* weight,
                             cvl_stream_t stream);
int cvl_gather_rows(const void* src, int64_t row_bytes, const int32_t* idx, int n, void* dst, cvl_stream_t stream);

int cvl_retina_assign(const float* boxes, const int32_t* nbox, const float* img_dim, int B, int n_max,
                      int pad, int num_classes, const float* anchor_dims, int n_anchors,
                      const int32_t* strides , float iou_thresh, float* targets,
                      int32_t* num_targets, cvl_stream_t stream);

int cvl_centernet_assign(const float* boxes, const int32_t* nbox, const float* img_dim, int B, int n_max,
                         int pad_h, int pad_w, int num_classes, int stride, float* targets,
                         cvl_stream_t stream);

int cvl_centernet_splat(const float* boxes, const int32_t* nbox, const float* img_dim, int B, int n_max,
                        int pad_h, int pad_w, int num_classes, int stride, float sigma, float* targets,
                        cvl_stream_t stream);
int cvl_center_dist(const double* grid_x, const double* grid_y, int n, double mu_x, double mu_y, double spread,
                    double* out, cvl_stream_t stream);

size_t cvl_det_loss_workspace_size(int B, int P);
int cvl_det_loss(const float* reg_pred, int ld_reg, const float* cls_pred, int ld_cls, const float* targets,
                 int B, int P, int num_classes, float grad_scale_cls, float grad_scale_reg, float* losses,
                 float* d_reg, float* d_cls, void* workspace, cvl_stream_t stream);

size_t cvl_retina_loss_workspace_size(int B, int P, int n_anchors);
int cvl_retina_loss(const float* reg_pred, int ld_reg, const float* cls_pred, int ld_cls, const float* targets,
                    int B, const int32_t* level_cells , int n_anchors, int num_classes,
                    const float* img_weight, float grad_scale, float* losses, void* d_reg, int ld_dreg,
                    void* d_cls, int ld_dcls, void* workspace, cvl_stream_t stream);

size_t cvl_nms_workspace_size(int n, int ncls);
int cvl_nms(const double* boxes, int n, const double* classes, int ncls, double iou_threshold,
            int32_t* keep, int32_t* nkeep, void* workspace, cvl_stream_t stream);
size_t cvl_soft_nms_workspace_size(int n, int ncls);
int cvl_soft_nms(const double* boxes, int n, const double* classes, int ncls, double sigma, int32_t* keep,
                 double* keep_score, int32_t* nkeep, void* workspace, cvl_stream_t stream);


size_t cvl_bn_stats_workspace_size(int B, int HW, int C);
int cvl_bn_stats(const void* x, int B, int HW, int C, uint64_t* stats, void* workspace, size_t workspace_bytes,
                 cvl_stream_t stream);
int cvl_bn_finalize_grouped(const uint64_t* stats, float* mean_rstd, float* run_mean, float* run_var, int B, int C,
                            int HW, int group, float eps, float momentum, cvl_stream_t stream);
size_t cvl_bn_backward_grouped_workspace_size(int B, int HW, int C);
int cvl_bn_backward_grouped(const void* dy, const void* y_relu, const void* z, const float* mean_rstd,
                            const float* gamma, void* workspace, size_t workspace_bytes, void* dz, float dz_beta,
                            float* dgamma, float* dbeta, int B, int HW, int C, int group, cvl_stream_t stream);

int cvl_maxpool2x2(const void* x, void* y, uint8_t* argmax, int B, int H, int W, int C, cvl_stream_t stream);
int cvl_maxpool2x2_backward(const void* dy, const uint8_t* argmax, void* dx, int B, int H, int W, int C,
                            cvl_stream_t stream);

int cvl_upsample_bilinear2x_add(const void* prev, const void* other, void* out, int B, int h, int w, int C,
                                cvl_stream_t stream);
int cvl_upsample_bilinear2x_backward(const void* dout, void* dprev, int B, int h, int w, int C, float beta,
                                     cvl_stream_t stream);

int cvl_depthwise_fwd(const void* x, const float* w, void* y, int B, int H, int W, int C, int k, int stride,
                      int pad_t, int pad_l, int Ho, int Wo, cvl_stream_t stream);
int cvl_depthwise_dgrad(const void* dy, const float* w, void* dx, int B, int H, int W, int C, int k, int stride,
                        int pad_t, int pad_l, int Ho, int Wo, float beta, cvl_stream_t stream);
size_t cvl_depthwise_wgrad_workspace_size(int B, int Ho, int Wo, int C, int k);
int cvl_depthwise_wgrad(const void* x, const void* dy, float* dw, float beta, int B, int H, int W, int C, int k,
                        int stride, int pad_t, int pad_l, int Ho, int Wo, void* workspace, size_t workspace_bytes,
                        cvl_stream_t stream);

size_t cvl_gconv3x3_packed_bytes(int C);
int cvl_gconv3x3_pack(const float* w, int C, int Cg, void* w_fwd, void* w_dgrad, cvl_stream_t stream);
int cvl_gconv3x3_fwd(const void* x, const void* w_fwd, void* y, uint64_t* bn_stats, int B, int H, int W, int C, int Cg,
                     int stride, int Ho, int Wo, cvl_stream_t stream);
int cvl_gconv3x3_dgrad(const void* dy, const void* w_dgrad, void* dx, int B, int H, int W, int C, int Cg, int stride,
                       int Ho, int Wo, float beta, cvl_stream_t stream);
size_t cvl_gconv3x3_wgrad_workspace_size(int B, int H, int W, int C, int Cg, int stride);
int cvl_gconv3x3_wgrad(const void* x, const void* dy, float* dw, float beta, int B, int H, int W, int C, int Cg,
                       int stride, int Ho, int Wo, void* workspace, size_t workspace_bytes, cvl_stream_t stream);
int cvl_gconv3x3_plan(int kind, int B, int H, int W, int C, int Cg, int stride, int* tpw, int* ychunks, int* tiles_x,
                      int* tiles_y, int* tpc, int* nchunk);

size_t cvl_bn_data_stats_workspace_size(int B);
int cvl_bn_data_stats(const float* img, int B, int H, int W, float eps, float momentum, float* mean_rstd,
                      float* run_mean, float* run_var, void* workspace, size_t workspace_bytes, cvl_stream_t stream);
int cvl_bn_data_apply(const float* img, const float* mean_rstd, const float* beta, float* out, int B, int H, int W,
                      cvl_stream_t stream);

int cvl_upsample_bilinear2x_sum(const void* a, const void* b, void* out, int B, int h, int w, int C,
                                cvl_stream_t stream);
#define CVL_RC_MAX_ITEMS 16
typedef struct {
  const void* src;
  void* dsrc;
  int c, c_ld, hw;
  float beta;
} cvl_rc_item;
int cvl_reshape_concat(const cvl_rc_item* items, int n_items, int B, int S2, void* dst, int ld_dst,
                       cvl_stream_t stream);
int cvl_reshape_concat_backward(const cvl_rc_item* items, int n_items, int B, int S2, const void* d_dst,
                                int ld_dst, cvl_stream_t stream);
int cvl_bias_scalar_fold_periodic(const float* bias, const float* scalar, float* b_eff, int n, int period, int c0,
                                  cvl_stream_t stream);
int cvl_bias_scalar_unfold_periodic(const float* g_eff, float* g_bias, float* g_scalar, int n, int period, int c0,
                                    cvl_stream_t stream);
int cvl_hourglass_v2_assign(const float* boxes, const int32_t* nbox, int B, int n_max, int raw_dims, int img_dims,
                            int num_classes, float* targets, cvl_stream_t stream);
int cvl_centernet_s8_assign(const float* boxes, const int32_t* nbox, const float* img_dim, int B, int n_max,
                            int pad_h, int pad_w, int num_classes, const float* box_scales, int n_scales, int stride,
                            float* targets, cvl_stream_t stream);
size_t cvl_centernet_s8_loss_workspace_size(int B, int P, int n_scales);
int cvl_centernet_s8_loss(const float* reg_pred, int ld_reg, const float* cls_pred, int ld_cls, const float* targets,
                          int B, int P, int n_scales, int num_classes, float cls_scale, float reg_scale, float* losses,
                          void* d_reg, int ld_dreg, void* d_cls, int ld_dcls, void* workspace, cvl_stream_t stream);
size_t cvl_hourglass_v2_loss_workspace_size(int B, int P);
int cvl_hourglass_v2_loss(const float* pred, int ld_pred, const float* targets, int B, int P, int num_classes,
                          int loss_type, float cls_scale, float reg_scale, float* losses, void* d_pred, int ld_d,
                          void* workspace, cvl_stream_t stream);

typedef struct {
  const float* dw;
  const float* pw;
  float* weff;
  const float* gweff;
  float* gdw;
  float* gpw;
  int taps, cin, cout;
  int cin_ld, cout_ld;
  int pad_;
} cvl_sep_item;
int cvl_sep_fold_multi(const cvl_sep_item* items, const int32_t* rows, int nrows, cvl_stream_t stream);
int cvl_sep_unfold_multi(const cvl_sep_item* items, const int32_t* rows, int nrows, cvl_stream_t stream);

int cvl_bias_scalar_fold(const float* bias, const float* scalar, float* b_eff, int n, int c0, cvl_stream_t stream);
int cvl_bias_scalar_unfold(const float* g_eff, float* g_bias, float* g_scalar, int n, int c0, cvl_stream_t stream);

int cvl_centernet_loss(const float* pred, int ld_pred, const float* targets, int B, int P, int num_classes,
                       float cls_scale, float reg_scale, float* losses, void* d_pred, int ld_d, void* workspace,
                       cvl_stream_t stream);

int cvl_centernet_decode(const float* pred, int ld, int H, int W, int num_classes, double stride, float thresh,
                         double w_ratio, double h_ratio, double img_width, double img_height, double* rows,
                         int32_t* count, cvl_stream_t stream);

int cvl_centernet_scale_decode(const float* pred, int ld, int H, int W, int n_scales, int ch_per_scale, int cls0,
                               int num_classes, int box_mode, const double* box_scales ,
                               float stride, float thresh, double w_ratio, double h_ratio, double img_width,
                               double img_height, double* rows, int32_t* count, cvl_stream_t stream);

size_t cvl_centernet_peak_decode_workspace_size(int B, int H, int W, int num_classes);
int cvl_centernet_peak_decode(const float* pred, int ld, int B, int H, int W, int num_classes, float stride,
                              float thresh, int K, double* dets, int32_t* count, void* workspace,
                              size_t workspace_bytes, cvl_stream_t stream);

int cvl_adam_clip_update(float* w, const float* g, float* m, float* v, int64_t n, const float* lr_dev,
                         int32_t* iterations, float beta1, float beta2, float eps, float inv_bs, float clip,
                         double* sumsq_ws, cvl_stream_t stream);


int cvl_retina_corners(const float* xy, int ld, int H, int W, float anchor_h, float anchor_w, int stride,
                       float* out, cvl_stream_t stream);

size_t cvl_retina_decode_workspace_size(int B, const int32_t* level_hw, int n_anchors);
int cvl_retina_decode(const float* reg_pred, int ld_reg, const float* cls_pred, int ld_cls, int B,
                      const int32_t* level_hw, const int32_t* strides, const float* anchor_dims, int n_anchors,
                      int num_classes, float cls_thresh, float* dets, int32_t* count, void* workspace,
                      size_t workspace_bytes, cvl_stream_t stream);

size_t cvl_retina_nms_workspace_size(int B, int n_cap);
int cvl_retina_nms(const float* dets, int rows_per_img, const int32_t* count, int B, int n_cap, float iou_thresh,
                   int32_t* keep, int32_t* nkeep, void* workspace, cvl_stream_t stream);

size_t cvl_fcos_detect_workspace_size(int B, int P, int num_classes, int max_per_class);
int cvl_fcos_detect(const float* reg_pred, int ld_reg, const float* cls_pred, int ld_cls, int B,
                    const int32_t* level_hw, const int32_t* strides, int num_classes, int center, float iou_thresh,
                    float score_thresh, int max_per_class, int max_total, float* out_boxes, float* out_scores,
                    float* out_classes, int32_t* valid, void* workspace, size_t workspace_bytes,
                    cvl_stream_t stream);

#define CVL_EVAL_MAX_T 1024
#define CVL_EVAL_MAX_G 1024
#define CVL_EVAL_MAX_THRESHOLDS 16
#define CVL_EVAL_MAX_CLASSES 65535
#define CVL_EVAL_MAX_B 65535
#define CVL_EVAL_AP_CHUNK 1024
enum { CVL_EVAL_VOC = 0, CVL_EVAL_COCO = 1 };
enum { CVL_EVAL_AP_VOC07 = 0, CVL_EVAL_AP_VOC12 = 1, CVL_EVAL_AP_COCO = 2 };

int cvl_eval_match(const float* boxes, const float* scores, const float* classes, const int32_t* valid,
                   const float* gt_boxes, const int32_t* gt_labels, const uint8_t* gt_flags,
                   const int32_t* gt_count, const int64_t* image_ids, int B, int T, int G, int num_classes,
                   const double* thresholds , int K, int protocol, int max_dets, float* rec_score,
                   int32_t* rec_class, int64_t* rec_key, uint16_t* rec_tp, uint16_t* rec_ign, int64_t rec_offset,
                   int32_t* npos, cvl_stream_t stream);

int cvl_eval_ap(const uint16_t* rec_tp, const uint16_t* rec_ign, const int64_t* seg_offsets, const int32_t* npos,
                int64_t n_records, int num_classes, int K, int mode, double* ap, int32_t* tp_total,
                cvl_stream_t stream);

#define CVL_EVAL_MAX_AREAS 4
#define CVL_EVAL_MAX_VIEWS 8

int cvl_eval_match_areas(const float* boxes, const float* scores, const float* classes, const int32_t* valid,
                         const float* gt_boxes, const int32_t* gt_labels, const uint8_t* gt_flags,
                         const int32_t* gt_count, const int64_t* image_ids, int B, int T, int G, int num_classes,
                         const double* thresholds , int K, int protocol, int max_dets,
                         const double* area_ranges , int A, const float* gt_area ,
                         const float* area_scale , float* rec_score, int32_t* rec_class,
                         int64_t* rec_key, uint16_t* rec_tp, uint16_t* rec_ign, uint16_t* rec_rank,
                         int64_t rec_offset, int32_t* npos, cvl_stream_t stream);

int cvl_eval_ap_views(const uint16_t* rec_tp, const uint16_t* rec_ign, const uint16_t* rec_rank,
                      const int64_t* seg_offsets, const int32_t* npos, int64_t n_records, int num_classes, int K,
                      int A, const int32_t* views , int R, double* ap, int32_t* tp_total,
                      cvl_stream_t stream);


int cvl_resize_pad_normalize(const void* src, int src_u8, int H, int W, int C, int flip, int out_h, int out_w,
                             int pad_h, int pad_w, float* out, cvl_stream_t stream);

size_t cvl_image_augment_workspace_size(int B, int N);
int cvl_image_augment(const float* img_src, float* img_dst, const float* tgt_src, float* tgt_dst,
                      const int32_t* ops, const float* params, int B, int N, int S, int T, void* workspace,
                      size_t workspace_bytes, cvl_stream_t stream);

enum { CVL_JPEG_UNSUPPORTED = 2, CVL_JPEG_CORRUPT = 3 };
#define CVL_JPEG_MAX_BATCH 4096

int cvl_jpeg_info(const uint8_t* data, size_t nbytes, int32_t* info );

int cvl_jpeg_entropy_decode(const uint8_t* data, size_t nbytes, int16_t* coef, size_t coef_cap,
                            uint16_t* qt );

int cvl_jpeg_batch_sizes(const int32_t* coef_counts, int n, size_t* staging_bytes, size_t* workspace_bytes);

int cvl_jpeg_decode_batch(const uint8_t* const* data, const size_t* nbytes, int n, uint8_t* const* out,
                          void* staging, size_t staging_bytes, void* workspace, size_t workspace_bytes,
                          int32_t* status, cvl_stream_t stream);

#ifdef __cplusplus
}
#endif
#endif
```

Baseline: 1454 images/s.

## Add LDS halo-tile mode to X32 conv kernel for 3x3 stride-1 convs

```diff
diff --git a/cv-lite-object-detection_amd/csrc/conv_common.h b/cv-lite-object-detection_amd/csrc/conv_common.h
--- a/cv-lite-object-detection_amd/csrc/conv_common.h
+++ b/cv-lite-object-detection_amd/csrc/conv_common.h
@@ -15,6 +15,7 @@
 
 extern thread_local int g_cvl_conv_last_kernel;
 extern thread_local int g_cvl_conv_last_ktile;
+extern thread_local int g_cvl_conv_last_halo;
 
 __device__ __forceinline__ int xcd_remap(int b, int nwg) {
   const int q = nwg / 8, r = nwg % 8, x = b % 8;
@@ -132,6 +133,7 @@
   bool dgrad;
   bool sw;
   bool wres;
+  bool halo;
   bool prio, acc, stamps;
   int stages;
   int bsum;
@@ -163,6 +165,7 @@
 
 bool cvl_conv_h_fits(const cvl_conv_desc* d, const ConvArgs& a, int* halo_px);
 constexpr int kConvHWresCb = 2;
+constexpr int kConvXHaloPx = 512;
 constexpr int kConvHStampWgs = 4096;
 constexpr unsigned kConvBufRecords = 0x7fffffffu;
 
diff --git a/cv-lite-object-detection_amd/csrc/conv_dispatch.hip b/cv-lite-object-detection_amd/csrc/conv_dispatch.hip
--- a/cv-lite-object-detection_amd/csrc/conv_dispatch.hip
+++ b/cv-lite-object-detection_amd/csrc/conv_dispatch.hip
@@ -1,4 +1,5 @@
 #include "conv_common.h"
+#include "conv_halo.h"
 
 namespace {
 
@@ -117,6 +118,15 @@
   return buffer_bounds_ok(a);
 }
 
+bool x32_halo_fits(const cvl_conv_desc* d, const ConvArgs& a) {
+  if (d->KH != 3 || d->KW != 3 || d->stride != 1 || d->pad_t != 1 || d->pad_l != 1 || a.Cin % 32) return false;
+  for (int i = 0; i < a.nseg; ++i) {
+    int px = 0;
+    if (!halo_seg_fits(a.seg[i], kConvXHaloPx, &px)) return false;
+  }
+  return true;
+}
+
 bool plan_x(const cvl_conv_desc* d, const ConvArgs& a, const ConvCallOpts& o, ConvPlan* p) {
   if (cvl_dispatch_flag("no_x") || !x32_fits(d, a)) return false;
   p->kernel = CVL_CK_X32;
@@ -126,6 +136,7 @@
   p->dbg = cvl_tune_int("CVL_X_ABLATE", 0);
   p->sw = !a.dst_f32 && !o.bn_stats && a.beta == 0.f && dst_chunks8(d) && !cvl_dispatch_flag("x_no_sw");
   p->ymask = p->sw && o.ymask && !a.relu_out && !cvl_dispatch_flag("no_relu_mask_fuse");
+  p->halo = !cvl_dispatch_flag("x_no_halo") && x32_halo_fits(d, a);
   return true;
 }
 
@@ -405,3 +416,15 @@
   *ktile = conv_plan_ktile(p);
   return CVL_OK;
 }
+
+extern "C" int cvl_conv_igemm_plan_halo(const cvl_conv_desc* d, int with_bn_stats, size_t workspace_bytes,
+                                        int32_t* halo) {
+  CVL_CHECK_ARG(d && halo);
+  *halo = 0;
+  if (d->prec == CVL_PREC_F32) return CVL_OK;
+  ConvPlan p;
+  const int st = conv_plan(d, ConvCallOpts{with_bn_stats != 0, CVL_BSUM_NONE, false, workspace_bytes}, &p);
+  if (st) return st;
+  *halo = p.kernel == CVL_CK_X32 && p.halo;
+  return CVL_OK;
+}
diff --git a/cv-lite-object-detection_amd/csrc/conv_halo.h b/cv-lite-object-detection_amd/csrc/conv_halo.h
--- /dev/null
+++ b/cv-lite-object-detection_amd/csrc/conv_halo.h
@@ -0,0 +1,70 @@
+#pragma once
+#include "conv_common.h"
+
+constexpr int kHaloBM = 256;
+
+struct HGeo {
+  int whole, mx, my, th, pitch, rows;
+};
+__host__ __device__ inline HGeo h_geo(int H, int W) {
+  HGeo g;
+  const int HW = H * W;
+  g.whole = HW < kHaloBM;
+  if (g.whole) {
+    const int n = kHaloBM / HW;
+    int lg = 0;
+    while ((1 << (lg + 1)) <= n) ++lg;
+    g.mx = 1 << ((lg + 1) / 2);
+    g.my = n / g.mx;
+    g.th = H;
+  } else {
+    g.mx = g.my = 1;
+    g.th = kHaloBM / W;
+  }
+  g.pitch = (g.mx * (W + 1) + 1 + 7) & ~7;
+  g.rows = g.my * (g.th + 1) + 1;
+  return g;
+}
+
+template <int NP>
+struct HaloPieces {
+  int rel[NP];
+  int yrow[NP];
+  unsigned valid;
+};
+
+template <int NP>
+__device__ __forceinline__ HaloPieces<NP> halo_pieces(const HGeo& G, int H, int W, int wave, int lane) {
+  HaloPieces<NP> P;
+  P.valid = 0;
+  const int hpx = G.rows * G.pitch;
+#pragma unroll
+  for (int j = 0; j < NP; ++j) {
+    const int hp = 16 * (wave + 8 * j) + (lane >> 2);
+    const int hy = hp / G.pitch, hx = hp - hy * G.pitch;
+    bool ok;
+    if (!G.whole) {
+      const int gx = hx - 1;
+      ok = gx >= 0 && gx < W;
+      P.rel[j] = (hy - 1) * W + gx;
+      P.yrow[j] = hy - 1;
+    } else {
+      const int ix = (hx - 1) / (W + 1), iy = (hy - 1) / (H + 1);
+      const int gx = hx - 1 - ix * (W + 1), gy = hy - 1 - iy * (H + 1);
+      ok = hx >= 1 && hy >= 1 && gx < W && gy < H && ix < G.mx && iy < G.my;
+      P.rel[j] = gy * W + gx;
+      P.yrow[j] = iy * G.mx + ix;
+    }
+    if (ok && hp < hpx) P.valid |= 1u << j;
+  }
+  return P;
+}
+
+static inline bool halo_seg_fits(const ConvSeg& q, int cap_px, int* halo_px) {
+  if (q.Hr != q.Hs || q.Wr != q.Ws) return false;
+  const int W = q.Wr, HW = q.Hr * q.Wr;
+  if (HW >= kHaloBM ? (kHaloBM % W || HW % kHaloBM) : (kHaloBM % HW)) return false;
+  const HGeo g = h_geo(q.Hr, W);
+  *halo_px = g.rows * g.pitch;
+  return g.mx * g.my * (g.whole ? HW : kHaloBM) == kHaloBM && *halo_px <= cap_px;
+}
diff --git a/cv-lite-object-detection_amd/csrc/conv_igemm.hip b/cv-lite-object-detection_amd/csrc/conv_igemm.hip
--- a/cv-lite-object-detection_amd/csrc/conv_igemm.hip
+++ b/cv-lite-object-detection_amd/csrc/conv_igemm.hip
@@ -492,9 +492,11 @@
 
 thread_local int g_cvl_conv_last_kernel = CVL_CK_NONE;
 thread_local int g_cvl_conv_last_ktile = 0;
+thread_local int g_cvl_conv_last_halo = 0;
 
 extern "C" int cvl_conv_igemm_last_kernel(void) { return g_cvl_conv_last_kernel; }
 extern "C" int cvl_conv_igemm_last_ktile(void) { return g_cvl_conv_last_ktile; }
+extern "C" int cvl_conv_igemm_last_halo(void) { return g_cvl_conv_last_halo; }
 
 int launch_base(const ConvPlan& p, const ConvArgs& a, hipStream_t s) {
   if (p.bn == 128) launch_bn<128>(p, a, s);
@@ -518,6 +520,7 @@
   }
   g_cvl_conv_last_kernel = p.kernel;
   g_cvl_conv_last_ktile = conv_plan_ktile(p);
+  g_cvl_conv_last_halo = p.kernel == CVL_CK_X32 && p.halo;
   if (st || p.splits <= 1) return st;
   return splitk_finish_launch(a, s);
 }
@@ -531,7 +534,7 @@
     case CVL_CK_L128: return "conv_igemm_l_kernel<128> (256x128)";
     case CVL_CK_L256: return "conv_igemm_l_kernel<256> (256x256)";
     case CVL_CK_X256: return "conv_igemm_x_kernel (256x256, 4 phases per 64-deep K-tile)";
-    case CVL_CK_X32: return "conv_igemm_x32_kernel (256x256, 5-slot ring of 32-deep K-tiles)";
+    case CVL_CK_X32: return "conv_igemm_x32_kernel (256x256, ring of 32-deep K-tiles: 5 A+B slots, or 6 B slots behind an LDS halo)";
     case CVL_CK_X32H: return "conv_igemm_x32h_kernel (256x256, 3x3 halo tile in LDS, 6-slot weight ring)";
     case CVL_CK_WG_SN: return "conv_wgrad_sn_kernel (Npad 32, taps on the dY side, chunk slabs)";
     case CVL_CK_WG_S: return "conv_wgrad_kernel (128-wide k tile)";
diff --git a/cv-lite-object-detection_amd/csrc/conv_igemm_h.hip b/cv-lite-object-detection_amd/csrc/conv_igemm_h.hip
--- a/cv-lite-object-detection_amd/csrc/conv_igemm_h.hip
+++ b/cv-lite-object-detection_amd/csrc/conv_igemm_h.hip
@@ -1,5 +1,6 @@
 #include "conv_common.h"
 #include "conv_epilogue.h"
+#include "conv_halo.h"
 
 namespace {
 
@@ -21,61 +22,6 @@
 __device__ __forceinline__ void dma16(__amdgpu_buffer_rsrc_t r, const cvl_bf16* lds_dst, unsigned voff) {
   __builtin_amdgcn_raw_ptr_buffer_load_lds(r, (__attribute__((address_space(3))) void*)lds_dst, 16, (int)voff, 0,
                                            0, 0);
-}
-
-struct HGeo {
-  int whole, mx, my, th, pitch, rows;
-};
-__host__ __device__ inline HGeo h_geo(int H, int W) {
-  HGeo g;
-  const int HW = H * W;
-  g.whole = HW < BM;
-  if (g.whole) {
-    const int n = BM / HW;
-    int lg = 0;
-    while ((1 << (lg + 1)) <= n) ++lg;
-    g.mx = 1 << ((lg + 1) / 2);
-    g.my = n / g.mx;
-    g.th = H;
-  } else {
-    g.mx = g.my = 1;
-    g.th = BM / W;
-  }
-  g.pitch = (g.mx * (W + 1) + 1 + 7) & ~7;
-  g.rows = g.my * (g.th + 1) + 1;
-  return g;
-}
-
-struct HaloPieces {
-  int rel[HPW];
-  int yrow[HPW];
-  unsigned valid;
-};
-
-__device__ __forceinline__ HaloPieces halo_pieces(const HGeo& G, int H, int W, int wave, int lane) {
-  HaloPieces P;
-  P.valid = 0;
-  const int hpx = G.rows * G.pitch;
-#pragma unroll
-  for (int j = 0; j < HPW; ++j) {
-    const int hp = 16 * (wave + 8 * j) + (lane >> 2);
-    const int hy = hp / G.pitch, hx = hp - hy * G.pitch;
-    bool ok;
-    if (!G.whole) {
-      const int gx = hx - 1;
-      ok = gx >= 0 && gx < W;
-      P.rel[j] = (hy - 1) * W + gx;
-      P.yrow[j] = hy - 1;
-    } else {
-      const int ix = (hx - 1) / (W + 1), iy = (hy - 1) / (H + 1);
-      const int gx = hx - 1 - ix * (W + 1), gy = hy - 1 - iy * (H + 1);
-      ok = hx >= 1 && hy >= 1 && gx < W && gy < H && ix < G.mx && iy < G.my;
-      P.rel[j] = gy * W + gx;
-      P.yrow[j] = iy * G.mx + ix;
-    }
-    if (ok && hp < hpx) P.valid |= 1u << j;
-  }
-  return P;
 }
 
 #ifdef CVL_MEASURE
@@ -147,7 +93,7 @@
   const int hch = lane & 3;
   int i_L = next_tile(t_lo), i_cb = cb0, i_sg = -1;
   unsigned hoff[HPW], woff[WJ + (WR ? 1 : 0)];
-  HaloPieces HP;
+  HaloPieces<HPW> HP;
   HP.valid = 0;
   auto cursor_tile = [&]() {
     int sg, mloc0, n0;
@@ -156,7 +102,7 @@
     const int W = S.Wr, H = S.Hr, HWr = H * W;
     const HGeo G = h_geo(H, W);
     if (sg != i_sg) {
-      HP = halo_pieces(G, H, W, wave, lane);
+      HP = halo_pieces<HPW>(G, H, W, wave, lane);
       i_sg = sg;
     }
     const int img0 = mloc0 / HWr;
@@ -618,12 +564,9 @@
   if (a.Npad == 32 && (d->mode != CVL_CONV_FWD || !d->dst_f32)) return false;
   for (int i = 0; i < a.nseg; ++i) {
     const ConvSeg& q = a.seg[i];
-    if (q.Hr != q.Hs || q.Wr != q.Ws) return false;
-    const int W = q.Wr, HW = q.Hr * q.Wr;
-    if (HW >= BM ? (BM % W || HW % BM) : (BM % HW)) return false;
-    const HGeo g = h_geo(q.Hr, W);
-    if (g.mx * g.my * (g.whole ? HW : BM) != BM || g.rows * g.pitch > HPX) return false;
-    if (g.rows * g.pitch > *halo_px) *halo_px = g.rows * g.pitch;
+    int px = 0;
+    if (!halo_seg_fits(q, HPX, &px)) return false;
+    if (px > *halo_px) *halo_px = px;
     const long src_bytes = (q.src_base + (long)a.B * q.src_img) * a.Cin * 2;
     if (src_bytes >= (long)kRecords - 65536) return false;
   }
diff --git a/cv-lite-object-detection_amd/csrc/conv_igemm_x.hip b/cv-lite-object-detection_amd/csrc/conv_igemm_x.hip
--- a/cv-lite-object-detection_amd/csrc/conv_igemm_x.hip
+++ b/cv-lite-object-detection_amd/csrc/conv_igemm_x.hip
@@ -1,5 +1,6 @@
 #include "conv_common.h"
 #include "conv_epilogue.h"
+#include "conv_halo.h"
 
 namespace {
 
@@ -21,11 +22,28 @@
 
 __device__ __forceinline__ int swz4(int r) { return (r >> 1) & 3; }
 
+constexpr int HPX32 = 512;
+constexpr int HPW32 = HPX32 / 16 / 8;
+constexpr int HALO32_EL = HPX32 * BK32;
+constexpr int BSLOT = 256 * BK32;
+constexpr int NBSLOT = 6;
+constexpr int BLEAD = NBSLOT - 2;
+static_assert(2 * HALO32_EL + NBSLOT * BSLOT <= LDS32_EL && HPX32 == kConvXHaloPx, "X32 halo form: LDS layout");
+static_assert(BLEAD >= 2 && HPW32 + BLEAD - 1 <= 8, "the halo of block cb + 1 is retired by the wait of phase (cb, 8)");
+constexpr int halo_pieces_in(int lo, int hi) {
+  int n = 0;
+  for (int p = lo; p <= hi; ++p) {
+    const int q = ((p % 9) + 9) % 9;
+    n += q >= 1 && q <= HPW32;
+  }
+  return n;
+}
+
 typedef __bf16 bf16x2 __attribute__((ext_vector_type(2)));
 typedef float f32x2 __attribute__((ext_vector_type(2)));
 typedef unsigned u32x4 __attribute__((ext_vector_type(4)));
 
-template <bool DGRAD, bool DBG, bool SW>
+template <bool DGRAD, bool DBG, bool SW, bool HALO>
 __device__ __forceinline__ void x32_body(const ConvArgs& a) {
   const int dbg = DBG ? a.dbg : 0;
   __shared__ __attribute__((aligned(16))) cvl_bf16 lds[LDS32_EL];
@@ -53,9 +71,9 @@
   const int nk = Kdim / BK32;
   const int x16 = wave * 16 + (lane >> 2), ch = lane & 3;
   const unsigned chs = (unsigned)((ch ^ swz4(x16)) * 16);
-  unsigned aoff[2], amask[2];
-#pragma unroll
-  for (int p = 0; p < 2; ++p) {
+  unsigned aoff[2] = {0u, 0u}, amask[2] = {0u, 0u};
+#pragma unroll
+  for (int p = 0; !HALO && p < 2; ++p) {
     const int ml = mloc0 + p * 128 + x16;
     const int img = ml / HWr, q = ml - img * HWr;
     const int oy = q / S.Wr, ox = q - (q / S.Wr) * S.Wr;
@@ -132,64 +150,201 @@
     asm volatile("" ::: "memory");
   };
 
-  issue();
-  issue();
-  issue();
-  wait_vm<8>();
-  __builtin_amdgcn_s_barrier();
-  asm volatile("" ::: "memory");
-  if (wm == 1) bar();
   unsigned long long clk0 = 0;
-  if (stamp) { stamp[1] = wall_clock64(); clk0 = __builtin_amdgcn_s_memtime(); }
-
-  int rslot = 0;
-  for (int kt = 0; kt < nk; ++kt) {
-    if (!(dbg & 16)) wait_vm<4>();
+  if constexpr (HALO) {
+    const HGeo G = h_geo(S.Hr, S.Wr);
+    const int ncb = Cin / BK32;
+    unsigned hoff[HPW32];
+    {
+      const int W = S.Wr, H = S.Hr;
+      const HaloPieces<HPW32> HP = halo_pieces<HPW32>(G, H, W, wave, lane);
+      const int img0 = mloc0 / HWr;
+      const int y0 = G.whole ? 0 : (mloc0 - img0 * HWr) / W;
+      const long base = S.src_base + (long)img0 * S.src_img + (long)y0 * W;
+#pragma unroll
+      for (int j = 0; j < HPW32; ++j) {
+        const int hp = 16 * (wave + 8 * j) + (lane >> 2);
+        bool ok = (HP.valid >> j) & 1u;
+        long pix;
+        if (!G.whole) {
+          ok = ok && (unsigned)(y0 + HP.yrow[j]) < (unsigned)H && img0 < a.B;
+          pix = base + HP.rel[j];
+        } else {
+          const int img = img0 + HP.yrow[j];
+          ok = ok && img < a.B;
+          pix = S.src_base + (long)img * S.src_img + HP.rel[j];
+        }
+        hoff[j] = ok ? (unsigned)(pix * Cin * 2) + (unsigned)((ch ^ swz4(hp)) * 16) : kOOB;
+      }
+    }
+    const int prow = G.pitch * BK32 * 2;
+    unsigned afr[TM][3];
+#pragma unroll
+    for (int i = 0; i < TM; ++i) {
+      const int r = wm * WM + i * 16 + lr;
+      const int ii = r / HWr, q = r - ii * HWr;
+      const int yy = q / S.Wr, xx = q - yy * S.Wr;
+      const int hy = 1 + (G.whole ? (ii / G.mx) * (S.Hr + 1) : 0) + yy;
+      const int hx = 1 + (G.whole ? (ii % G.mx) * (S.Wr + 1) : 0) + xx;
+      const int pc = hy * G.pitch + hx;
+#pragma unroll
+      for (int d = 0; d < 3; ++d) {
+        const int pp = pc + d - 1;
+        afr[i][d] = (unsigned)(pp * BK32 * 2 + ((lg ^ swz4(pp)) * 16));
+      }
+    }
+    cvl_bf16* const ring = lds + 2 * HALO32_EL;
+    int hkc = 0, htap = 0, hcb = 0, hslot = 0;
+    unsigned hbk = 0;
+    auto issue_b = [&]() {
+      if (!(dbg & 32)) {
+        const bool live = hkc < nk && !(dbg & 2);
+        cvl_bf16* Bb = ring + hslot * BSLOT + wave * 16 * BK32;
+#pragma unroll
+        for (int p = 0; p < 2; ++p)
+          dma16(rsB, Bb + p * 128 * BK32, live ? boff0 + (unsigned)(p * 128 * Kdim * 2) + hbk : kOOB);
+      }
+      ++hkc;
+      hslot = hslot == NBSLOT - 1 ? 0 : hslot + 1;
+      if (++htap == 9) { htap = 0; ++hcb; }
+      hbk = (unsigned)((htap * Cin + hcb * 32) * 2);
+    };
+    auto issue_h = [&](int cb, int j) {
+      if (dbg & 32) return;
+      const bool live = cb < ncb && !(dbg & 1);
+      dma16(rsA, lds + (cb & 1) * HALO32_EL + (wave + 8 * j) * 16 * BK32, live ? hoff[j] + (unsigned)(cb * 64) : kOOB);
+    };
+
+#pragma unroll
+    for (int j = 0; j < HPW32; ++j) issue_h(0, j);
+#pragma unroll
+    for (int i = 0; i < BLEAD; ++i) issue_b();
+    wait_vm<2 * (BLEAD - 1)>();
+    __builtin_amdgcn_s_barrier();
+    asm volatile("" ::: "memory");
+    if (wm == 1) bar();
+    if (stamp) { stamp[1] = wall_clock64(); clk0 = __builtin_amdgcn_s_memtime(); }
+
+    int rslot = 0;
+    auto phase = [&](int cb, auto TC) {
+      constexpr int t = decltype(TC)::value;
+      constexpr int fly = 2 * (BLEAD - 2) + halo_pieces_in(t - (BLEAD - 2), t - 1);
+      if (!(dbg & 16)) wait_vm<fly>();
+      if (t >= 1 && t <= HPW32) issue_h(cb + 1, t - 1);
+      issue_b();
+      const char* Hc = reinterpret_cast<const char*>(lds + (cb & 1) * HALO32_EL);
+      const cvl_bf16* Bc = ring + rslot * BSLOT;
+      s16x8 fa[TM], fb[TN];
+      if (dbg & 64) {
+#pragma unroll
+        for (int i = 0; i < TM; ++i) fa[i] = s16x8{(short)lr, 0, 0, 0, 0, 0, 0, (short)(cb + t)};
+#pragma unroll
+        for (int j = 0; j < TN; ++j) fb[j] = s16x8{(short)j, 0, 0, 0, 0, 0, 0, (short)lg};
+      } else {
+        constexpr int r = t / 3, sx = t % 3;
+        constexpr int d = DGRAD ? 2 - sx : sx;
+        const char* Hr = Hc + (DGRAD ? 1 - r : r - 1) * prow;
+#pragma unroll
+        for (int i = 0; i < TM; ++i) fa[i] = *reinterpret_cast<const s16x8*>(Hr + afr[i][d]);
+#pragma unroll
+        for (int j = 0; j < TN; ++j) {
+          const int rr = wn * WN + j * 16 + lr;
+          fb[j] = *reinterpret_cast<const s16x8*>(Bc + rr * BK32 + ((lg ^ swz4(rr)) * 8));
+        }
+      }
+      bar();
+      asm volatile("s_waitcnt lgkmcnt(0)" ::: "memory");
+      __builtin_amdgcn_sched_barrier(0);
+      __builtin_amdgcn_s_setprio(1);
+      if (dbg & 4) {
+        asm volatile("" ::"v"(fa[0]), "v"(fb[0]), "v"(fa[TM - 1]), "v"(fb[TN - 1]));
+      } else {
+#pragma unroll
+        for (int i = 0; i < TM; ++i) {
+#pragma unroll
+          for (int j = 0; j < TN; ++j)
+            acc[i][j] = SW ? __builtin_amdgcn_mfma_f32_16x16x32_bf16(__builtin_bit_cast(bf16x8, fb[j]),
+                                                                      __builtin_bit_cast(bf16x8, fa[i]), acc[i][j], 0, 0, 0)
+                           : __builtin_amdgcn_mfma_f32_16x16x32_bf16(__builtin_bit_cast(bf16x8, fa[i]),
+                                                                      __builtin_bit_cast(bf16x8, fb[j]), acc[i][j], 0, 0, 0);
+        }
+      }
+      __builtin_amdgcn_s_setprio(0);
+      __builtin_amdgcn_sched_barrier(0);
+      bar();
+      rslot = rslot == NBSLOT - 1 ? 0 : rslot + 1;
+    };
+    for (int cb = 0; cb < ncb; ++cb) {
+      phase(cb, std::integral_constant<int, 0>{});
+      phase(cb, std::integral_constant<int, 1>{});
+      phase(cb, std::integral_constant<int, 2>{});
+      phase(cb, std::integral_constant<int, 3>{});
+      phase(cb, std::integral_constant<int, 4>{});
+      phase(cb, std::integral_constant<int, 5>{});
+      phase(cb, std::integral_constant<int, 6>{});
+      phase(cb, std::integral_constant<int, 7>{});
+      phase(cb, std::integral_constant<int, 8>{});
+    }
+  } else {
     issue();
-    const cvl_bf16* Ac = lds + rslot * SLOT;
-    const cvl_bf16* Bc = Ac + 256 * BK32;
-    s16x8 fa[TM], fb[TN];
-    if (dbg & 64) {
-#pragma unroll
-      for (int i = 0; i < TM; ++i) fa[i] = s16x8{(short)lr, 0, 0, 0, 0, 0, 0, (short)kt};
-#pragma unroll
-      for (int j = 0; j < TN; ++j) fb[j] = s16x8{(short)j, 0, 0, 0, 0, 0, 0, (short)lg};
-    } else {
-#pragma unroll
-      for (int i = 0; i < TM; ++i) {
-        const int r = wm * WM + i * 16 + lr;
-        fa[i] = *reinterpret_cast<const s16x8*>(Ac + r * BK32 + ((lg ^ swz4(r)) * 8));
-      }
-#pragma unroll
-      for (int j = 0; j < TN; ++j) {
-        const int r = wn * WN + j * 16 + lr;
-        fb[j] = *reinterpret_cast<const s16x8*>(Bc + r * BK32 + ((lg ^ swz4(r)) * 8));
-      }
-    }
-    bar();
-    asm volatile("s_waitcnt lgkmcnt(0)" ::: "memory");
-    __builtin_amdgcn_sched_barrier(0);
-    __builtin_amdgcn_s_setprio(1);
-    if (dbg & 4) {
-      asm volatile("" ::"v"(fa[0]), "v"(fb[0]), "v"(fa[TM - 1]), "v"(fb[TN - 1]));
-    } else {
-#pragma unroll
-      for (int i = 0; i < TM; ++i) {
-#pragma unroll
-        for (int j = 0; j < TN; ++j)
-          acc[i][j] = SW ? __builtin_amdgcn_mfma_f32_16x16x32_bf16(__builtin_bit_cast(bf16x8, fb[j]),
-                                                                    __builtin_bit_cast(bf16x8, fa[i]), acc[i][j], 0, 0, 0)
-                         : __builtin_amdgcn_mfma_f32_16x16x32_bf16(__builtin_bit_cast(bf16x8, fa[i]),
-                                                                    __builtin_bit_cast(bf16x8, fb[j]), acc[i][j], 0, 0, 0);
-      }
-    }
-    __builtin_amdgcn_s_setprio(0);
-    __builtin_amdgcn_sched_barrier(0);
-    bar();
-    rslot = rslot == NSLOT - 1 ? 0 : rslot + 1;
+    issue();
+    issue();
+    wait_vm<8>();
+    __builtin_amdgcn_s_barrier();
+    asm volatile("" ::: "memory");
+    if (wm == 1) bar();
+    if (stamp) { stamp[1] = wall_clock64(); clk0 = __builtin_amdgcn_s_memtime(); }
+
+    int rslot = 0;
+    for (int kt = 0; kt < nk; ++kt) {
+      if (!(dbg & 16)) wait_vm<4>();
+      issue();
+      const cvl_bf16* Ac = lds + rslot * SLOT;
+      const cvl_bf16* Bc = Ac + 256 * BK32;
+      s16x8 fa[TM], fb[TN];
+      if (dbg & 64) {
+  #pragma unroll
+        for (int i = 0; i < TM; ++i) fa[i] = s16x8{(short)lr, 0, 0, 0, 0, 0, 0, (short)kt};
+  #pragma unroll
+        for (int j = 0; j < TN; ++j) fb[j] = s16x8{(short)j, 0, 0, 0, 0, 0, 0, (short)lg};
+      } else {
+  #pragma unroll
+        for (int i = 0; i < TM; ++i) {
+          const int r = wm * WM + i * 16 + lr;
+          fa[i] = *reinterpret_cast<const s16x8*>(Ac + r * BK32 + ((lg ^ swz4(r)) * 8));
+        }
+  #pragma unroll
+        for (int j = 0; j < TN; ++j) {
+          const int r = wn * WN + j * 16 + lr;
+          fb[j] = *reinterpret_cast<const s16x8*>(Bc + r * BK32 + ((lg ^ swz4(r)) * 8));
+        }
+      }
+      bar();
+      asm volatile("s_waitcnt lgkmcnt(0)" ::: "memory");
+      __builtin_amdgcn_sched_barrier(0);
+      __builtin_amdgcn_s_setprio(1);
+      if (dbg & 4) {
+        asm volatile("" ::"v"(fa[0]), "v"(fb[0]), "v"(fa[TM - 1]), "v"(fb[TN - 1]));
+      } else {
+  #pragma unroll
+        for (int i = 0; i < TM; ++i) {
+  #pragma unroll
+          for (int j = 0; j < TN; ++j)
+            acc[i][j] = SW ? __builtin_amdgcn_mfma_f32_16x16x32_bf16(__builtin_bit_cast(bf16x8, fb[j]),
+                                                                      __builtin_bit_cast(bf16x8, fa[i]), acc[i][j], 0, 0, 0)
+                           : __builtin_amdgcn_mfma_f32_16x16x32_bf16(__builtin_bit_cast(bf16x8, fa[i]),
+                                                                      __builtin_bit_cast(bf16x8, fb[j]), acc[i][j], 0, 0, 0);
+        }
+      }
+      __builtin_amdgcn_s_setprio(0);
+      __builtin_amdgcn_sched_barrier(0);
+      bar();
+      rslot = rslot == NSLOT - 1 ? 0 : rslot + 1;
+    }
   }
   if (wm == 0) bar();
   wait_vm<0>();
+  if constexpr (HALO && !SW) bar();
   if (stamp) { stamp[2] = wall_clock64(); stamp[3] = __builtin_amdgcn_s_memtime() - clk0; }
   if (dbg & 8) {
     if (acc[0][0][0] == 12345.f) reinterpret_cast<float*>(a.dst)[1] = 1.f;
@@ -251,10 +406,10 @@
   conv_l_epilogue<BN, WGM, TM, TN, NT>(a, S, acc, lds, tid, wm, wn, n0, mloc0, HWr, znone, BnSumPar{});
 }
 
-template <bool DGRAD, bool DBG = false, bool SW = false>
+template <bool DGRAD, bool DBG = false, bool SW = false, bool HALO = false>
 __global__ void __launch_bounds__(NT) conv_igemm_x32_kernel(ConvArgs a) {
   if (a.probe) probe_enter(a.probe);
-  x32_body<DGRAD, DBG, SW>(a);
+  x32_body<DGRAD, DBG, SW, HALO>(a);
   if (a.probe) probe_leave(a.probe);
 }
 
@@ -264,12 +419,15 @@
   const dim3 grid(p.grid);
   with_bool(p.dgrad, [&](auto DG) {
     with_bool(p.sw, [&](auto SW) {
+      with_bool(p.halo, [&](auto HL) {
+        constexpr bool dg = decltype(DG)::value, sw = decltype(SW)::value, hl = decltype(HL)::value;
 #ifdef CVL_MEASURE
-      if (p.dbg)
-        hipLaunchKernelGGL((conv_igemm_x32_kernel<decltype(DG)::value, true, decltype(SW)::value>), grid, dim3(NT), 0, s, a);
-      else
+        if (p.dbg)
+          hipLaunchKernelGGL((conv_igemm_x32_kernel<dg, true, sw, hl>), grid, dim3(NT), 0, s, a);
+        else
 #endif
-        hipLaunchKernelGGL((conv_igemm_x32_kernel<decltype(DG)::value, false, decltype(SW)::value>), grid, dim3(NT), 0, s, a);
+          hipLaunchKernelGGL((conv_igemm_x32_kernel<dg, false, sw, hl>), grid, dim3(NT), 0, s, a);
+      });
     });
   });
   return cvl_launch_status();
diff --git a/cv-lite-object-detection_amd/cvlite/_lib.py b/cv-lite-object-detection_amd/cvlite/_lib.py
--- a/cv-lite-object-detection_amd/cvlite/_lib.py
+++ b/cv-lite-object-detection_amd/cvlite/_lib.py
@@ -61,6 +61,8 @@
     "cvl_relu_": (c_int, [P, ctypes.c_long, P]),
     "cvl_conv_igemm_last_kernel": (c_int, []),
     "cvl_conv_igemm_last_ktile": (c_int, []),
+    "cvl_conv_igemm_last_halo": (c_int, []),
+    "cvl_conv_igemm_plan_halo": (c_int, [P, c_int, c_size_t, P]),
     "cvl_conv_igemm_plan": (c_int, [P, c_int, c_size_t, P, P]),
     "cvl_conv_igemm_plan_grid": (c_int, [P, c_int, c_int, c_size_t, P, P, P, P]),
     "cvl_conv_kernel_name": (ctypes.c_char_p, [c_int]),
@@ -253,7 +255,7 @@
 _lib = None
 
 
-NEWER = {"cvl_conv_igemm_last_ktile", "cvl_conv_igemm_plan", "cvl_conv_igemm_plan_bnsum", "cvl_conv_igemm_plan_grid",
+NEWER = {"cvl_conv_igemm_last_halo", "cvl_conv_igemm_plan_halo", "cvl_conv_igemm_last_ktile", "cvl_conv_igemm_plan", "cvl_conv_igemm_plan_bnsum", "cvl_conv_igemm_plan_grid",
          "cvl_conv_igemm_dgrad_bnsum_res_bits", "cvl_bn_finalize_apply_bits", "cvl_bn_finalize_apply_bnres_bits",
          "cvl_bn_backward_bits", "cvl_bn_backward_res_sums_bits", "cvl_bn_backward_res_sums_sc_bits",
          "cvl_bn_backward_sc_bits", "cvl_conv_wgrad_plan", "cvl_conv_wgrad_batch_plan", "cvl_conv_igemm_res_relu",
diff --git a/include/cvlite.h b/include/cvlite.h
--- a/include/cvlite.h
+++ b/include/cvlite.h
@@ -148,6 +148,8 @@
        CVL_CK_H64 = 14, CVL_CK_WG_H = 15, CVL_CK_P = 16 };
 int cvl_conv_igemm_last_kernel(void);
 int cvl_conv_igemm_last_ktile(void);
+int cvl_conv_igemm_last_halo(void);
+int cvl_conv_igemm_plan_halo(const cvl_conv_desc* d, int with_bn_stats, size_t workspace_bytes, int32_t* halo);
 int cvl_conv_igemm_plan(const cvl_conv_desc* d, int with_bn_stats, size_t workspace_bytes, int32_t* kernel,
                         int32_t* ktile);
 int cvl_conv_igemm_plan_grid(const cvl_conv_desc* d, int with_bn_stats, int bsum_offer, size_t workspace_bytes,
```

Result: no change. 1460 images/s, median of 6 (+0.4%).
